# cgmb/euler

Measured on AMD Instinct MI355X. Metric: cells*steps/sec of sim_step() (frames incl. the PCG pressure projection) + pressure-solve HBM GB/s vs roofline, higher is better.
Workload: dtype f64

## Files before the change

euler_amd/__init__.py:

```python
import ctypes as C
import os

import numpy as np

_HERE = os.path.dirname(os.path.abspath(__file__))
LIB_PATH = os.path.join(_HERE, "lib", "libeuler_hip.so")

DOT_AUTO, DOT_SEQUENTIAL, DOT_TREE = 0, 1, 2
PRECOND_IC0, PRECOND_JACOBI, PRECOND_IC0_TILE, PRECOND_IC0_TILE2, PRECOND_IC0_TILE_MG = 0, 1, 2, 3, 4
(OPT_P_STEPS, OPT_TILE_STORE_AS, OPT_TILE_REVERSE, OPT_RESIDENT_CAP, OPT_GRID4_MIN_CELLS, OPT_SLAB_FUSION, OPT_RCCL_SMALL, OPT_RCCL_NO_EXCHANGE, OPT_MARKERS_ROWMAJOR,
 OPT_SA_RUN, OPT_NO_INTERIOR, OPT_BUILD_GATHER, OPT_RESIDENT_FORCE_TIMEOUT, OPT_MG_SPLIT_LEVEL, OPT_MG_SPLIT_ACTIVE, OPT_MARKERS_TWO_PASS, OPT_BUILD_TWO_PASS,
 OPT_VELOCITY_TWO_PASS, OPT_NO_TILE_MAP, OPT_PROFILE_STRIDE, OPT_TILE_STORE_Z, OPT_ADVECT_RK2, OPT_ADVECT_MACCORMACK) = range(1, 24)
SWEEP_AUTO, SWEEP_BAND, SWEEP_SIMPLE = 0, 1, 2
PCG_F64, PCG_F32 = 0, 1
RESIDENT_AUTO, RESIDENT_OFF = 0, 1
IMAGE_COVERAGE, IMAGE_DYE, IMAGE_SPEED = 0, 1, 2
EDIT_SOLID, EDIT_CLEAR, EDIT_SINK, EDIT_SOURCE, EDIT_FILL, EDIT_DRAIN = range(6)
OVERVIEW_DTYPE = np.dtype({"names": ["cells", "solid", "sink", "water", "marks", "max_speed2", "dye"],
                           "formats": [np.uint32, np.uint32, np.uint32, np.uint32, np.uint32, np.float32, (np.uint64, 3)],
                           "offsets": [0, 4, 8, 12, 16, 20, 24], "itemsize": 48})
DIAG_CROWDED = 8
DIAG_DTYPE = np.dtype({"names": ["cells", "fluid", "markers", "crowded", "mass_x", "mass_y", "div_l1", "ke_hi", "ke_lo", "count_max", "nonfinite", "max_div", "max_speed2"],
                       "formats": [np.uint64] * 9 + [np.uint32, np.uint32, np.float32, np.float32],
                       "offsets": [0, 8, 16, 24, 32, 40, 48, 56, 64, 72, 76, 80, 84], "itemsize": 88})
FLOW_PRESSURE = 1
PAINT_VORTICITY, PAINT_PRESSURE, PAINT_SPEED = 0, 1, 2
FLOW_DTYPE = np.dtype({"names": ["cells", "water", "nodes", "nonfinite", "u_pos", "u_neg", "v_pos", "v_neg", "w_pos", "w_neg", "p_sum", "max_speed2", "max_abs_w", "max_p", "reserved"],
                       "formats": [np.uint32] * 4 + [np.uint64] * 7 + [np.float32] * 3 + [np.uint32],
                       "offsets": [0, 4, 8, 12, 16, 24, 32, 40, 48, 56, 64, 72, 76, 80, 84], "itemsize": 88})
DIAG_VALUES = ("mean_abs_div", "kinetic_energy", "com_x", "com_y", "markers_per_cell", "crowded_fraction")
(F_U, F_V, F_UTMP, F_VTMP, F_SOLID, F_SOURCE, F_SINK, F_COUNT, F_PREV_COUNT, F_MARKERS, F_PRECON,
 F_PRESSURE, F_PCG_B, F_PCG_R, F_PCG_Z, F_PCG_S, F_PCG_Q, F_CELLMASK,
 F_DYE_R, F_DYE_G, F_DYE_B, F_DYE_RTMP, F_DYE_GTMP, F_DYE_BTMP, F_MARKER_KEYS) = range(25)
(STAGE_ADVECT_MARKERS, STAGE_REFRESH_COUNTS, STAGE_SOURCES, STAGE_EXTRAPOLATE, STAGE_ADVECT_VELOCITY,
 STAGE_PROJECT) = range(6)
(OP_BUILD_SYSTEM, OP_PRECON_FACTOR, OP_FORWARD_SOLVE, OP_BACKWARD_SOLVE, OP_APPLY_A, OP_DOT_ZR, OP_DOT_ZS,
 OP_INF_NORM_R, OP_UPDATE_PR, OP_UPDATE_SEARCH) = range(10)

_FIELD_DTYPE = {
    F_U: np.float32, F_V: np.float32, F_UTMP: np.float32, F_VTMP: np.float32,
    F_SOLID: np.uint8, F_SOURCE: np.uint8, F_SINK: np.uint8, F_COUNT: np.uint8, F_PREV_COUNT: np.uint8,
    F_MARKERS: np.float32, F_PRECON: np.float64, F_PRESSURE: np.float64, F_PCG_B: np.float64,
    F_PCG_R: np.float64, F_PCG_Z: np.float64, F_PCG_S: np.float64, F_PCG_Q: np.float64, F_CELLMASK: np.uint8,
    F_DYE_R: np.float32, F_DYE_G: np.float32, F_DYE_B: np.float32,
    F_DYE_RTMP: np.float32, F_DYE_GTMP: np.float32, F_DYE_BTMP: np.float32, F_MARKER_KEYS: np.uint32,
}


class EulerError(RuntimeError):
    def __init__(self, code, msg):
        super().__init__("libeuler_hip error %d: %s" % (code, msg))
        self.code = code


class Config(C.Structure):
    _fields_ = [
        ("abi_version", C.c_int32), ("X", C.c_int32), ("Y", C.c_int32), ("device", C.c_int32),
        ("max_iterations", C.c_int32), ("tol", C.c_double), ("dot_mode", C.c_int32), ("precond", C.c_int32),
        ("sweep_mode", C.c_int32), ("max_substeps", C.c_int32), ("frame_time", C.c_float),
        ("viscosity", C.c_float), ("pcg_poll_interval", C.c_int32), ("rainbow", C.c_int32),
        ("precond_tile_records", C.c_int32), ("slab_rank", C.c_int32), ("slab_nranks", C.c_int32),
        ("slab_band_lo", C.c_int32), ("slab_band_hi", C.c_int32), ("pcg_precision", C.c_int32), ("resident", C.c_int32),
    ]


class Stats(C.Structure):
    _fields_ = [
        ("frames", C.c_uint64), ("total_substeps", C.c_uint64), ("total_pcg_iterations", C.c_uint64),
        ("last_substeps", C.c_int32), ("last_pcg_iterations", C.c_int32), ("last_residual", C.c_double),
        ("last_dt", C.c_float), ("n_markers", C.c_uint64), ("source_exhausted", C.c_int32),
        ("rng_state", C.c_uint64), ("marker_dt_events", C.c_uint64), ("marker_multi_events", C.c_uint64),
        ("fluid_cells", C.c_uint64),
    ]


_lib = None

EXPORTS = [
    "euler_config_default", "euler_create", "euler_destroy", "euler_last_error", "euler_abi_version",
    "euler_load_scenario_mem", "euler_load_scenario_file", "euler_load_half_tank", "euler_load_half_tanks", "euler_parse_scenario",
    "euler_seed_markers", "euler_step", "euler_timestep", "euler_substep", "euler_stage", "euler_pcg_op", "euler_set_precond", "euler_set_solver",
    "euler_get_field", "euler_set_field", "euler_set_markers", "euler_set_rng", "euler_get_stats",
    "euler_field_bytes", "euler_render", "euler_render_grids", "euler_render_grids_rgb", "euler_colorize", "euler_profile_enable",
    "euler_profile_class_count", "euler_profile_class_name", "euler_profile_get", "euler_profile_reset",
    "euler_measure_copy_bandwidth", "euler_measure_exchange", "euler_device_name", "euler_hbm_bytes", "euler_sweep_timeline", "euler_save_state", "euler_load_state", "euler_set_comm", "euler_set_stream", "euler_slab_info",
    "euler_rccl_unique_id", "euler_rccl_version", "euler_set_comm_rccl", "euler_comm_calls",
    "euler_p2p_export", "euler_p2p_connect", "euler_p2p_disconnect", "euler_p2p_calls", "euler_resident_info",
    "euler_set_option", "euler_get_option",
    "euler_overview", "euler_overview_text", "euler_overview_rgb", "euler_render_fit",
    "euler_diagnostics", "euler_diag_derive",
    "euler_overview_box", "euler_marker_raster", "euler_view_text", "euler_render_view",
    "euler_edit_box",
    "euler_flow_raster", "euler_flow_paint",
]

# ... 511 lines not shown
```

euler_amd/csrc/driver.hip:

```cpp
#include "euler_dev.h"
#include "k_mg.h"

#include <math.h>
#include <stdarg.h>
#include <stdlib.h>
#include <string.h>

#include <vector>

int eu_launch_build_system(euler_sim* S, float dt);
int eu_launch_velocity_update(euler_sim* S, float dt, int finish);
int eu_pressure_current(euler_sim* S);
int eu_unskew(euler_sim* S, const void* skew, void* rowmajor, int elem_bytes);
int eu_unskew_fluid(euler_sim* S, const double* skew, double* rowmajor);
double* eu_current_search_direction(euler_sim* S);
int eu_launch_tile_table(euler_sim* S);
int eu_skew(euler_sim* S, const void* rowmajor, void* skew, int elem_bytes);

static thread_local char g_err[512] = "";

void eu_set_error(const char* fmt, ...) {
  va_list ap;
  va_start(ap, fmt);
  vsnprintf(g_err, sizeof(g_err), fmt, ap);
// ... 40 lines not shown
    const int e = k / 2, cls = S->ev_cls[e];
    bool active = true;
    if (S->ev_iter[e] > -2) {
      const int q = S->ev_solve[e];
      const int iters = q == S->solve_seq ? cur_iters : (S->solve_seq - q < 256 ? S->solve_iters[q & 255] : 0);
      active = iters >= 0 && S->ev_iter[e] < iters;
      if (S->ev_iter[e] == -1) active = iters >= 0;
    }
    float ms = 0.f;
    if (hipEventElapsedTime(&ms, S->ev_pool[k], S->ev_pool[k + 1]) != hipSuccess) continue;
    if (active) { S->prof_ms[cls] += ms; S->prof_launches[cls] += 1; }
    else S->prof_idle[cls] += 1;
  }
  S->ev_used = 0;
  return EULER_OK;
}

extern "C" int euler_profile_class_count(void) { return KC__COUNT; }
extern "C" const char* euler_profile_class_name(int32_t c) { return (c >= 0 && c < KC__COUNT) ? k_class_names[c] : ""; }
extern "C" int euler_profile_enable(euler_sim* S, uint64_t mask) {
  if (!S) return EULER_EINVAL;
  int rc = eu_prof_flush(S);
  S->prof_mask = mask;
  S->prof_open = 0;
  return rc;
}
extern "C" int euler_profile_get(euler_sim* S, int32_t cls, double* ms, uint64_t* launches) {
  if (!S || cls < 0 || cls >= KC__COUNT) return EULER_EINVAL;
  int rc = eu_prof_flush(S);
  if (ms) *ms = S->prof_ms[cls];
  if (launches) *launches = S->prof_launches[cls];
  return rc;
}
extern "C" int euler_profile_reset(euler_sim* S) {
  if (!S) return EULER_EINVAL;
  int rc = eu_prof_flush(S);
  memset(S->prof_ms, 0, sizeof(S->prof_ms));
  memset(S->prof_launches, 0, sizeof(S->prof_launches));
  memset(S->prof_idle, 0, sizeof(S->prof_idle));
  return rc;
}

extern "C" int euler_config_default(euler_config* c) {
  if (!c) return EULER_EINVAL;
  memset(c, 0, sizeof(*c));
  c->abi_version = EULER_ABI_VERSION;
  c->X = 100; c->Y = 40;
  c->device = 0;
  c->max_iterations = 100;
  c->tol = (double)1e-6f;
  c->dot_mode = EULER_DOT_AUTO;
  c->precond = EULER_PRECOND_IC0;
  c->sweep_mode = EULER_SWEEP_AUTO;
  c->max_substeps = 8;
  c->frame_time = 0.1f;
  c->viscosity = 0.f;
  c->pcg_poll_interval = 8;
  return EULER_OK;
}

static int eu_set_tiles(euler_sim* S, int w) {
  if (w <= 0) w = 16;
  if (w != 8 && w != 16 && w != 32) { eu_set_error("precond_tile_records = %d: 8, 16 or 32 (0 = 16)", w); return EULER_EINVAL; }
  S->cfg.precond_tile_records = w;
  S->tile_w = w;
  return EULER_OK;
}

bool eu_resident_eligible(const euler_sim* S) {
  if (S->res_disabled || S->cfg.resident == EULER_RESIDENT_OFF) return false;
  if (S->cfg.precond != EULER_PRECOND_IC0_TILE || S->tile_w != 16 || S->cfg.sweep_mode == EULER_SWEEP_SIMPLE || S->cfg.dot_mode != EULER_DOT_TREE) return false;
  if (S->has_comm || S->slab_on || S->p2p_on) return false;
  const int cap = eu_resident_capacity(const_cast<euler_sim*>(S), S->cfg.pcg_precision == EULER_PCG_F32);
  if (S->cfg.pcg_precision == EULER_PCG_F32) return cap > 0 && S->geom.nbands * (S->geom.T / 16) <= 4 * cap;
  return cap > 0;
}
extern "C" int euler_resident_info(euler_sim* S, uint64_t out[3]) {
  if (!S || !out) return EULER_EINVAL;
  out[0] = eu_resident_eligible(S) ? 1 : 0; out[1] = S->res_solves; out[2] = S->res_fallbacks;
  return EULER_OK;
}

extern "C" int euler_set_option(euler_sim* S, int32_t key, int64_t value) {
  if (!S || key <= 0 || key >= EULER_OPT__COUNT) { eu_set_error("euler_set_option: unknown key %d", (int)key); return EULER_EINVAL; }
  bool ok = true;
  const char* when = nullptr;
  switch (key) {
    case EULER_OPT_P_STEPS: ok = value == 2 || value == 4 || value == 8; break;
    case EULER_OPT_SA_RUN: ok = value == 8 || value == 16 || value == 32;
      if (ok && value != 8 && (S->has_comm || eu_is_two_level(S))) when = "on a handle without a communicator, in the parity or the plain tile-local mode (the others run runs of 8)";
      break;
    case EULER_OPT_RCCL_SMALL: ok = value >= 0 && value <= 2; if (S->rccl) when = "before euler_set_comm_rccl"; break;
    case EULER_OPT_RCCL_NO_EXCHANGE: ok = value == 0 || value == 1; if (S->rccl) when = "before euler_set_comm_rccl"; break;
    case EULER_OPT_SLAB_FUSION: ok = value == 0 || value == 1; if (S->p2p_on) when = "before euler_p2p_connect"; break;
    case EULER_OPT_RESIDENT_CAP: case EULER_OPT_GRID4_MIN_CELLS: case EULER_OPT_RESIDENT_FORCE_TIMEOUT: ok = value >= 0; break;
    case EULER_OPT_MG_SPLIT_LEVEL: ok = value >= -1 && value < 12; break;
    case EULER_OPT_PROFILE_STRIDE: ok = value >= 1 && value <= 1024; break;
    case EULER_OPT_MG_SPLIT_ACTIVE: ok = false; break;
    case EULER_OPT_ADVECT_RK2: ok = value == 0 || value == 1;
      if (ok && value == 1 && S->slab_on) when = "on a whole-grid handle (row slabs: the midpoint samples reach one row beyond the ghost rows)";
      break;
    case EULER_OPT_ADVECT_MACCORMACK: ok = value == 0 || value == 1;
      if (ok && value == 1 && S->slab_on) when = "on a whole-grid handle (row slabs: the correction reads the forward result one row beyond the own rows)";
      break;
    default: ok = value == 0 || value == 1; break;
  }
  if (!ok) { eu_set_error("euler_set_option: key %d does not take the value %lld", (int)key, (long long)value); return EULER_EINVAL; }
  if (when) { eu_set_error("euler_set_option: key %d must be set %s", (int)key, when); return EULER_ESTATE; }
  HIPCHK(hipStreamSynchronize(S->stream));
  if (key == EULER_OPT_ADVECT_MACCORMACK && value == 1 && !S->mc_u) {
    float *a = nullptr, *b = nullptr;
    const size_t bytes = S->C * sizeof(float);
    if (hipMalloc((void**)&a, bytes) != hipSuccess || hipMalloc((void**)&b, bytes) != hipSuccess || hipMemset(a, 0, bytes) != hipSuccess ||
        hipMemset(b, 0, bytes) != hipSuccess) {
      if (a) (void)hipFree(a);
      if (b) (void)hipFree(b);
      (void)hipGetLastError();
      eu_set_error("euler_set_option: EULER_OPT_ADVECT_MACCORMACK needs %zu bytes of scratch", 2 * bytes);
      return EULER_ENOMEM;
    }
    S->mc_u = a; S->mc_v = b;
    S->hbm_bytes += 2 * bytes;
  }
  if (key == EULER_OPT_P_STEPS || key == EULER_OPT_SA_RUN) {
    int rcp = eu_pressure_current(S);
    if (rcp) return rcp;
  }
  S->opt[key] = value;
  if (key == EULER_OPT_P_STEPS || key == EULER_OPT_SA_RUN) S->s_ring_n = 0;
  if (key == EULER_OPT_MG_SPLIT_LEVEL) { eu_mg_split_release(S); S->opt[EULER_OPT_MG_SPLIT_ACTIVE] = 0; }
  return EULER_OK;
}
extern "C" int euler_get_option(euler_sim* S, int32_t key, int64_t* value) {
  if (!S || !value || key <= 0 || key >= EULER_OPT__COUNT) { eu_set_error("euler_get_option: unknown key %d", (int)key); return EULER_EINVAL; }
  *value = S->opt[key];
  return EULER_OK;
}

static const char* eu_precond_combination(const euler_sim* S, int precond, int tile_w, int has_comm, int slab_on, int p2p_on) {
  const bool coarse = precond == EULER_PRECOND_IC0_TILE2 || precond == EULER_PRECOND_IC0_TILE_MG;
  if (!coarse) return nullptr;
  if (tile_w != 16 || S->cfg.sweep_mode == EULER_SWEEP_SIMPLE) return "the coarse-correction preconditioners run on tiles of 16 records with the band schedule";
  if (precond == EULER_PRECOND_IC0_TILE2 && (has_comm || slab_on)) return "EULER_PRECOND_IC0_TILE2 runs on one GPU (row slabs: EULER_PRECOND_IC0_TILE_MG)";
  if (precond == EULER_PRECOND_IC0_TILE_MG && has_comm && (!slab_on || p2p_on)) return "EULER_PRECOND_IC0_TILE_MG with several ranks: row-slab handles without mailboxes only";
  return nullptr;
}

extern "C" int euler_set_precond(euler_sim* S, int32_t precond, int32_t tile_records) {
  if (!S || precond < EULER_PRECOND_IC0 || precond > EULER_PRECOND_IC0_TILE_MG) { eu_set_error("euler_set_precond: bad argument"); return EULER_EINVAL; }
  const int w = tile_records <= 0 ? 16 : tile_records;
  if (w != 8 && w != 16 && w != 32) { eu_set_error("precond_tile_records = %d: 8, 16 or 32 (0 = 16)", tile_records); return EULER_EINVAL; }
  if (const char* why = eu_precond_combination(S, precond, w, S->has_comm, S->slab_on, S->p2p_on)) { eu_set_error("euler_set_precond: %s", why); return EULER_EINVAL; }
  if (S->cfg.pcg_precision == EULER_PCG_F32 && (precond != EULER_PRECOND_IC0_TILE || w != 16)) { eu_set_error("euler_set_precond: an EULER_PCG_F32 handle runs EULER_PRECOND_IC0_TILE with tiles of 16 records only"); return EULER_EINVAL; }
  HIPCHK(hipStreamSynchronize(S->stream));
  const bool coarse = precond == EULER_PRECOND_IC0_TILE2 || precond == EULER_PRECOND_IC0_TILE_MG;
  if (coarse) { int rc = eu_coarse_alloc(S, precond == EULER_PRECOND_IC0_TILE_MG); if (rc) return rc; }
  (void)eu_set_tiles(S, w);
  S->cfg.dot_mode = coarse ? EULER_DOT_TREE : S->dot_mode_user;
  if (S->has_comm && S->cfg.dot_mode == EULER_DOT_SEQUENTIAL) S->cfg.dot_mode = EULER_DOT_TREE;
  S->cfg.precond = precond;
  S->lean_ok = 0;
  return EULER_OK;
}

extern "C" int euler_set_solver(euler_sim* S, int32_t max_iterations, double tol) {
  if (!S) return EULER_EINVAL;
  HIPCHK(hipStreamSynchronize(S->stream));
  if (max_iterations > 0) S->cfg.max_iterations = max_iterations;
  if (tol >= 0.0) S->cfg.tol = tol;
  return EULER_OK;
}

static thread_local size_t g_alloc_bytes = 0;
template <typename T>
static int dalloc(T** p, size_t n) {
  HIPCHK(hipMalloc((void**)p, n * sizeof(T)));
  g_alloc_bytes += n * sizeof(T);
  HIPCHK(hipMemset(*p, 0, n * sizeof(T)));
  return EULER_OK;
}
#define DALLOC(p, n) do { int _rc = dalloc(&(p), (n)); if (_rc) { euler_destroy(S); return _rc; } } while (0)

extern "C" void euler_destroy(euler_sim* S) {
  if (!S) return;
  if (S->stream) (void)hipStreamSynchronize(S->stream);
  eu_p2p_release(S);
  eu_rccl_release(S);
  eu_slab_release(S);
  eu_coarse_release(S);
  for (eu_devbuf* b : {&S->ov_buf, &S->diag_buf, &S->vr_buf, &S->flow_buf}) eu_devbuf_release(S, b);
  const size_t wo = S->shifted ? S->win_off : 0;
  for (float* f : {S->u, S->v, S->utmp, S->vtmp}) if (f) (void)hipFree(f + wo);
  for (uint8_t* g : {S->solid, S->source, S->sink, S->count, S->prev_count}) if (g) (void)hipFree(g + wo);
  if (S->count32) (void)hipFree(S->count32);
  if (S->blockedT) (void)hipFree(S->blockedT);
  if (S->tmap) (void)hipFree(S->tmap);
  if (S->uT) (void)hipFree(S->uT);
  if (S->vT) (void)hipFree(S->vT);
  if (S->countT) (void)hipFree(S->countT);
  if (S->solidT) (void)hipFree(S->solidT);
  if (S->sys_m) (void)hipFree(S->sys_m);
  if (S->sys_div) (void)hipFree(S->sys_div);
  void* dev[] = {S->markers[0], S->markers[1], S->keys[0], S->keys[1], S->ms, S->evmask, S->delmask, S->ev_theta, S->ev_delta, S->sel_idx, S->act_idx,
                 S->act_dt, S->cellmask64, S->draws, S->sel.block_sums, S->sc, S->partial, S->red_counter, S->granules, S->ticket, S->sweep_timeline, S->halo_buf, S->band_ranges, S->partial2, S->pair_buf, S->xrows, S->alpha_buf, S->rng_jump, S->chunk_flag, S->chunk_prev, S->chunk_part, S->tile_table, S->chunk_bits, S->chunk_list, S->zhalo, S->zrows,
                 S->rowmajor_tmp, S->mc_u, S->mc_v};
  for (void* p : dev) if (p) (void)hipFree(p);
  for (float* d : S->dye) if (d) (void)hipFree(d + wo);
  const size_t so = S->shifted ? S->skew_off : 0, sl = S->shifted ? (size_t)EU_SKEW_SLACK : 0;
  (void)so; (void)sl;
  for (void* d : S->s_ring_alloc) if (d) (void)hipFree(d);
  for (void* d : S->skew_alloc) if (d) (void)hipFree(d);
  const size_t fb_off = S->shifted ? (size_t)S->ab_lo * S->fb_stride * 64 : 0;
  if (S->fbits_fwd) (void)hipFree(S->fbits_fwd + fb_off);
  if (S->fbits_bwd) (void)hipFree(S->fbits_bwd + fb_off);
  if (S->ms_host) (void)hipHostFree(S->ms_host);
  if (S->sc_host) (void)hipHostFree(S->sc_host);
  if (S->poll_host) (void)hipHostFree(S->poll_host);
  if (S->res_err) (void)hipHostFree(S->res_err);
  if (S->res_gran) (void)hipFree(S->res_gran);
  for (hipEvent_t e : S->poll_event) if (e) (void)hipEventDestroy(e);
  if (S->ev_pool) { for (int k = 0; k < S->ev_cap; ++k) if (S->ev_pool[k]) (void)hipEventDestroy(S->ev_pool[k]); free(S->ev_pool); }
  free(S->ev_cls); free(S->ev_solve); free(S->ev_iter);
  if (S->stream && S->own_stream) (void)hipStreamDestroy(S->stream);
  free(S);
}

extern "C" int euler_create(const euler_config* cfg, euler_sim** out) {
  if (!cfg || !out) { eu_set_error("euler_create: null argument"); return EULER_EINVAL; }
  if (cfg->abi_version != EULER_ABI_VERSION) { eu_set_error("euler_create: ABI version %d != %d", cfg->abi_version, EULER_ABI_VERSION); return EULER_EINVAL; }
  if (cfg->X < 8 || cfg->Y < 8 || (size_t)cfg->X * cfg->Y > (size_t)1 << 30) { eu_set_error("euler_create: grid %dx%d out of range", cfg->X, cfg->Y); return EULER_EINVAL; }
  int ndev = 0;
  hipError_t e = hipGetDeviceCount(&ndev);
  if (e != hipSuccess || ndev == 0) {
    eu_set_error("euler_create: no HIP device (%s); libeuler_hip has no CPU path", e == hipSuccess ? "device count 0" : hipGetErrorString(e));
    return EULER_EHIP;
  }
  if (cfg->device < 0 || cfg->device >= ndev) { eu_set_error("euler_create: device %d of %d", cfg->device, ndev); return EULER_EINVAL; }
  HIPCHK(hipSetDevice(cfg->device));
  hipDeviceProp_t prop;
  HIPCHK(hipGetDeviceProperties(&prop, cfg->device));
  if (strncmp(prop.gcnArchName, "gfx950", 6) != 0) {
    eu_set_error("euler_create: device is %s; this library carries gfx950 code only", prop.gcnArchName);
    return EULER_EHIP;
  }

  euler_sim* S = (euler_sim*)calloc(1, sizeof(euler_sim));
  if (S) { S->opt[EULER_OPT_P_STEPS] = 8; S->opt[EULER_OPT_TILE_REVERSE] = 1; S->opt[EULER_OPT_GRID4_MIN_CELLS] = 1ll << 22; S->opt[EULER_OPT_SA_RUN] = 8; S->opt[EULER_OPT_PROFILE_STRIDE] = 1; }
  if (!S) return EULER_ENOMEM;
  g_alloc_bytes = 0;
  S->cfg = *cfg;
  if (S->cfg.max_iterations <= 0) S->cfg.max_iterations = 100;
  if (S->cfg.max_substeps <= 0) S->cfg.max_substeps = 8;
  if (S->cfg.frame_time <= 0.f) S->cfg.frame_time = 0.1f;
  S->X = cfg->X; S->Y = cfg->Y;
  const size_t C = S->C = (size_t)cfg->X * cfg->Y;
  if (S->cfg.dot_mode == EULER_DOT_AUTO) S->cfg.dot_mode = C <= 65536 ? EULER_DOT_SEQUENTIAL : EULER_DOT_TREE;
  S->dot_mode_user = S->cfg.dot_mode;
  if (S->cfg.sweep_mode == EULER_SWEEP_AUTO) S->cfg.sweep_mode = EULER_SWEEP_BAND;
  S->geom.X = S->X; S->geom.Y = S->Y;
  S->geom.nbands = (S->Y + 63) / 64;
  S->geom.T = (S->X + 63 + 95) / 96 * 96;
  S->geom.TS = (S->geom.T + 31) / 32 * 32 + 64;
  S->geom.S = (size_t)S->geom.nbands * S->geom.TS * 64;
  const int nbands = S->geom.nbands;
  S->slab_on = cfg->slab_nranks >= 1;
  if (S->slab_on) {
    if (cfg->slab_rank < 0 || cfg->slab_rank >= cfg->slab_nranks || cfg->slab_nranks > nbands) {
      eu_set_error("euler_create: slab rank %d of %d for %d bands of 64 rows", cfg->slab_rank, cfg->slab_nranks, nbands);
      free(S); return EULER_EINVAL;
    }
    if (S->cfg.sweep_mode == EULER_SWEEP_SIMPLE) {
      eu_set_error("euler_create: row slabs do not run EULER_SWEEP_SIMPLE");
      free(S); return EULER_EINVAL;
    }
    S->band_lo = (int)((int64_t)nbands * cfg->slab_rank / cfg->slab_nranks);
    S->band_hi = (int)((int64_t)nbands * (cfg->slab_rank + 1) / cfg->slab_nranks);
    if (cfg->slab_band_hi > cfg->slab_band_lo || cfg->slab_band_lo != 0) {
      const int lo = cfg->slab_band_lo, hi = cfg->slab_band_hi;
      const bool first = cfg->slab_rank == 0, last = cfg->slab_rank + 1 == cfg->slab_nranks;
      if (lo < 0 || hi <= lo || hi > nbands || (first && lo != 0) || (last && hi != nbands) || (!first && lo < cfg->slab_rank) ||
          (!last && nbands - hi < cfg->slab_nranks - 1 - cfg->slab_rank)) {
        eu_set_error("euler_create: slab rank %d of %d cannot own bands [%d, %d) of %d (every rank needs a band; the ranges tile the grid in rank order)",
                     cfg->slab_rank, cfg->slab_nranks, lo, hi, nbands);
        free(S); return EULER_EINVAL;
      }
      S->band_lo = lo; S->band_hi = hi;
    }
    if (S->cfg.dot_mode == EULER_DOT_SEQUENTIAL) S->cfg.dot_mode = EULER_DOT_TREE;
  } else { S->band_lo = 0; S->band_hi = nbands; }
  S->row_lo = 64 * S->band_lo; S->row_hi = 64 * S->band_hi < S->Y ? 64 * S->band_hi : S->Y;
  S->win_lo = S->row_lo - EU_GHOST_LO > 0 ? S->row_lo - EU_GHOST_LO : 0;
  S->win_hi = S->row_hi + EU_GHOST_HI < S->Y ? S->row_hi + EU_GHOST_HI : S->Y;
  S->win_off = (size_t)S->win_lo * S->X;
  S->Cw = (size_t)(S->win_hi - S->win_lo) * S->X;
  S->ab_lo = S->band_lo > 0 ? S->band_lo - 1 : 0; S->ab_hi = S->band_hi < nbands ? S->band_hi + 1 : nbands;
  S->skew_off = (size_t)S->ab_lo * S->geom.TS * 64;
  S->Sw = (size_t)(S->ab_hi - S->ab_lo) * S->geom.TS * 64;
  S->e_lo = (size_t)S->band_lo * S->geom.TS * 64; S->e_cnt = (size_t)(S->band_hi - S->band_lo) * S->geom.TS * 64;
  const size_t SS = S->Sw;
  const size_t Cw = S->Cw;
  if (C > ((size_t)1 << 29) || Cw > ((size_t)1 << 28) || (SS + EU_SKEW_SLACK) * 8 >= ((size_t)1 << 32)) {
    eu_set_error("grid %d x %d is larger than the supported maximum (2^28 cells per GPU, 2^29 in all)", cfg->X, cfg->Y);
    free(S);
    return EULER_EINVAL;
  }
#define CREATECHK(call) do { hipError_t _e = (call); if (_e != hipSuccess) { int _rc = eu_hip_fail(_e, #call, __FILE__, __LINE__); euler_destroy(S); return _rc; } } while (0)
  CREATECHK(hipStreamCreateWithFlags(&S->stream, hipStreamNonBlocking));
  S->own_stream = 1;

  DALLOC(S->u, Cw); DALLOC(S->v, Cw); DALLOC(S->utmp, Cw); DALLOC(S->vtmp, Cw);
  DALLOC(S->solid, Cw); DALLOC(S->source, Cw); DALLOC(S->sink, Cw); DALLOC(S->count, Cw); DALLOC(S->prev_count, Cw);
  DALLOC(S->count32, Cw);
  if (!S->slab_on) { DALLOC(S->blockedT, Cw); DALLOC(S->uT, Cw); DALLOC(S->vT, Cw); DALLOC(S->countT, Cw); DALLOC(S->solidT, Cw); }
  eu_state_replaced(S);
  DALLOC(S->sys_m, Cw); DALLOC(S->sys_div, Cw);
  if (S->cfg.rainbow) for (float*& d : S->dye) DALLOC(d, Cw);
  S->max_markers = 4 * C;
  if (S->slab_on) { const size_t cap = 6 * (size_t)(S->row_hi - S->row_lo) * S->X + 65536; if (cap < S->max_markers) S->max_markers = cap; }
  DALLOC(S->markers[0], S->max_markers); DALLOC(S->markers[1], S->max_markers);
  if (S->slab_on) { DALLOC(S->keys[0], S->max_markers); DALLOC(S->keys[1], S->max_markers); }
  DALLOC(S->ms, 1);
  const size_t mwords = (S->max_markers + 63) / 64;
  DALLOC(S->evmask, mwords);
  if (!S->slab_on) DALLOC(S->delmask, mwords);
  if (!S->slab_on) {
    S->tmap_nx = (S->X + 63) / 64 + 1; S->tmap_n = S->tmap_nx * ((S->Y + 63) / 64 + 2);
    DALLOC(S->tmap, 3 * (size_t)S->tmap_n);
  }
  DALLOC(S->ev_theta, S->max_markers); DALLOC(S->ev_delta, S->max_markers);
  S->sel_cap = S->max_markers;
  DALLOC(S->sel_idx, S->sel_cap);
  DALLOC(S->act_idx, S->max_markers); DALLOC(S->act_dt, S->max_markers);
  DALLOC(S->cellmask64, (Cw + 63) / 64 + 1);
  S->sel.capacity_blocks = (mwords + 2047) / 2048 + 1;
  DALLOC(S->sel.block_sums, S->sel.capacity_blocks);
  {
    const size_t stagger = (size_t)EU_ARRAY_STAGGER / 8 * 8;
    int k = 0;
    for (double** d : {&S->b, &S->p, &S->r, &S->z, &S->s, &S->s2, &S->q, &S->precon}) {
      DALLOC(*d, SS + EU_SKEW_SLACK + 8 * stagger / 8);
      S->skew_alloc[k] = *d;
      *d += (size_t)k * stagger / 8;
      ++k;
    }
    DALLOC(S->cellmask, SS + EU_SKEW_SLACK);
    S->skew_alloc[8] = S->cellmask;
  }
  S->fb_stride = 12 * (((S->geom.T + 7) / 8 + 11) / 12) + 4;
  DALLOC(S->fbits_fwd, (size_t)(S->ab_hi - S->ab_lo) * S->fb_stride * 64);
  DALLOC(S->fbits_bwd, (size_t)(S->ab_hi - S->ab_lo) * S->fb_stride * 64);
  DALLOC(S->sc, 1);
  DALLOC(S->band_ranges, (size_t)S->geom.nbands);
  { int rc = eu_set_tiles(S, S->cfg.precond_tile_records); if (rc) { euler_destroy(S); return rc; } }
  S->red_blocks = (int)eu_blocks(S->e_cnt, EU_RED_ELEMS, 2048);
  DALLOC(S->partial, (size_t)S->red_blocks > 2048 ? (size_t)S->red_blocks : 2048);
  DALLOC(S->partial2, 2048);
  DALLOC(S->pair_buf, 2 * 64);
  DALLOC(S->alpha_buf, 64);
  S->xrow_len = ((size_t)S->X + 15) / 16 * 16 + 64;
  DALLOC(S->xrows, 8 * S->xrow_len);
  S->chunk_cap = (size_t)(S->band_hi - S->band_lo) * (S->geom.T / 16);
  S->chunk_words = (S->chunk_cap + 63) / 64;
  DALLOC(S->chunk_flag, S->chunk_cap + 64);
  DALLOC(S->chunk_prev, S->chunk_cap + 64);
  DALLOC(S->chunk_part, S->chunk_cap + 64);
  DALLOC(S->tile_table, 8 * 64 * 2);
  DALLOC(S->chunk_bits, S->chunk_words + 1);
  DALLOC(S->chunk_list, S->chunk_cap + 64);
  {
    RngJump* J = (RngJump*)malloc(sizeof(RngJump));
    if (!J) { euler_destroy(S); return EULER_ENOMEM; }
    auto step = [](unsigned long long st) { st ^= st >> 12; st ^= st << 25; st ^= st >> 27; return st; };
    for (int b = 0; b < 64; ++b) J->col[0][b] = step(1ull << b);
    for (int i = 1; i < EU_RNG_JUMPS; ++i)
      for (int b = 0; b < 64; ++b) {
        unsigned long long x = J->col[i - 1][b], y = 0;
        for (int k = 0; k < 64; ++k) if ((x >> k) & 1) y ^= J->col[i - 1][k];
        J->col[i][b] = y;
      }
    int rc = dalloc(&S->rng_jump, 1);
    if (!rc && hipMemcpy(S->rng_jump, J, sizeof(RngJump), hipMemcpyHostToDevice) != hipSuccess) rc = EULER_EHIP;
    free(J);
    if (rc) { euler_destroy(S); return rc; }
  }
  DALLOC(S->red_counter, 1);
  DALLOC(S->halo_buf, (size_t)8 * S->X);
  S->gran_stride = (S->geom.T - 63 + 7) / 8 * 8;
  DALLOC(S->granules, (size_t)S->geom.nbands * S->gran_stride * 2);
  DALLOC(S->ticket, 1);
  DALLOC(S->sweep_timeline, (size_t)S->geom.nbands * 8);
  S->ticket_base = 0; S->epoch = 0;
  for (float** f : {&S->u, &S->v, &S->utmp, &S->vtmp}) *f -= S->win_off;
  for (float*& d : S->dye) if (d) d -= S->win_off;
  for (uint8_t** g : {&S->solid, &S->source, &S->sink, &S->count, &S->prev_count}) *g -= S->win_off;
  for (double** d : {&S->b, &S->p, &S->r, &S->z, &S->s, &S->s2, &S->q, &S->precon}) *d += EU_SKEW_SLACK - S->skew_off;
  S->cellmask += EU_SKEW_SLACK - S->skew_off;
  S->fbits_fwd -= (size_t)S->ab_lo * S->fb_stride * 64; S->fbits_bwd -= (size_t)S->ab_lo * S->fb_stride * 64;
  S->shifted = 1;
  CREATECHK(hipHostMalloc((void**)&S->ms_host, sizeof(MarkerState), hipHostMallocDefault));
  CREATECHK(hipHostMalloc((void**)&S->sc_host, sizeof(PcgScalars), hipHostMallocDefault));
  CREATECHK(hipHostMalloc((void**)&S->poll_host, 2 * sizeof(PcgScalars), hipHostMallocDefault));
  CREATECHK(hipHostMalloc((void**)&S->res_err, sizeof(int), hipHostMallocDefault));
  *S->res_err = 0;
  DALLOC(S->res_gran, 2 * 2 * (2 * 768) * 2);
  S->res_tag = 1;
  memset(S->poll_host, 0, 2 * sizeof(PcgScalars));
  for (hipEvent_t& e : S->poll_event) CREATECHK(hipEventCreateWithFlags(&e, hipEventDisableTiming));
  memset(S->ms_host, 0, sizeof(MarkerState)); memset(S->sc_host, 0, sizeof(PcgScalars));

  S->interp_lim[0] = nextafterf((float)(S->X - 2), 0.f);
  S->interp_lim[1] = nextafterf((float)(S->Y - 1), 0.f);
  S->interp_lim[2] = nextafterf((float)(S->X - 1), 0.f);
  S->interp_lim[3] = nextafterf((float)(S->Y - 2), 0.f);

  S->ev_cap = 16384;
  S->ev_pool = (hipEvent_t*)calloc((size_t)S->ev_cap, sizeof(hipEvent_t));
  S->ev_cls = (int*)calloc((size_t)S->ev_cap / 2, sizeof(int));
  S->ev_solve = (int*)calloc((size_t)S->ev_cap / 2, sizeof(int));
  S->ev_iter = (int*)calloc((size_t)S->ev_cap / 2, sizeof(int));
  S->prof_iter = -2;
  if (!S->ev_pool || !S->ev_cls || !S->ev_solve || !S->ev_iter) { euler_destroy(S); return EULER_ENOMEM; }
  for (int k = 0; k < S->ev_cap; ++k) CREATECHK(hipEventCreate(&S->ev_pool[k]));
  if (S->slab_on) { int rc = eu_slab_alloc(S); if (rc) { euler_destroy(S); return rc; } }
  if (S->cfg.precond == EULER_PRECOND_IC0_TILE2 || S->cfg.precond == EULER_PRECOND_IC0_TILE_MG) {
    if ((S->slab_on && S->cfg.precond != EULER_PRECOND_IC0_TILE_MG) || S->tile_w != 16 || S->cfg.sweep_mode == EULER_SWEEP_SIMPLE) {
      eu_set_error("EULER_PRECOND_IC0_TILE2: one GPU; _MG: one GPU or row slabs; both: tiles of 16 records, the band schedule"); euler_destroy(S); return EULER_EINVAL;
    }
    S->cfg.dot_mode = EULER_DOT_TREE;
    int rc = eu_coarse_alloc(S, S->cfg.precond == EULER_PRECOND_IC0_TILE_MG);
    if (rc) { euler_destroy(S); return rc; }
  }
  S->hbm_bytes = g_alloc_bytes + (S->slab_on ? eu_slab_bytes(S) : 0);
  eu_launch_tile_table(S);
  if (S->cfg.pcg_precision != EULER_PCG_F64 && S->cfg.pcg_precision != EULER_PCG_F32) { eu_set_error("euler_create: pcg_precision %d", S->cfg.pcg_precision); euler_destroy(S); return EULER_EINVAL; }
  if (S->cfg.pcg_precision == EULER_PCG_F32 && !eu_resident_eligible(S)) {
    eu_set_error("euler_create: EULER_PCG_F32 runs in the resident solver: one GPU, EULER_PRECOND_IC0_TILE with tiles of 16 records, EULER_DOT_TREE, "
                 "EULER_RESIDENT_AUTO, and a grid of at most %d 16-record chunks (this one: %d)", 4 * eu_resident_capacity(S, 1), S->geom.nbands * (S->geom.T / 16));
    euler_destroy(S); return EULER_EINVAL;
  }
  CREATECHK(hipStreamSynchronize(S->stream));
#undef CREATECHK
  *out = S;
  return EULER_OK;
}

static int upload_scenario(euler_sim* S, const uint8_t* solid, const uint8_t* source, const uint8_t* sink,
                           const uint8_t* fluid) {
  const size_t C = S->C;
  if (S->slab_on && !S->has_comm) { eu_set_error("row-slab handle: install the communicator (euler_set_comm / euler_set_comm_rccl) before loading a scenario"); return EULER_ESTATE; }
  std::vector<float> mk;
  std::vector<unsigned int> keys;
  uint64_t rng = EULER_RNG_SEED, n = 0, n_loc = 0;
  int rc;
  if (S->slab_on) {
    uint64_t cells = 0;
    for (int y = S->row_lo > 0 ? S->row_lo - 1 : 0; y < S->row_hi; ++y)
      for (int x = 0; x < S->X; ++x) cells += fluid[(size_t)y * S->X + x] != 0;
    const uint64_t room = 4 * cells;
    if (room > S->max_markers) { eu_set_error("row slab %d holds up to %llu markers, more than its capacity %zu", S->cfg.slab_rank, (unsigned long long)room, S->max_markers); return EULER_ENOMEM; }
    try { mk.resize(2 * (size_t)room + 2); keys.resize((size_t)room + 1); } catch (...) { return EULER_ENOMEM; }
    rc = euler_seed_markers_rows(fluid, S->X, S->Y, S->row_lo, S->row_hi, &rng, mk.data(), keys.data(), room, &n, &n_loc);
  } else {
    try { mk.resize(2 * 4 * C); } catch (...) { return EULER_ENOMEM; }
    rc = euler_seed_markers(fluid, S->X, S->Y, &rng, mk.data(), &n);
    n_loc = n;
  }
  if (rc) return rc;
  size_t nsrc = 0;
  for (size_t i = (size_t)S->row_lo * S->X; i < (size_t)S->row_hi * S->X; ++i) nsrc += source[i] != 0;
  S->n_source_cells = nsrc;
  if (S->draws) { (void)hipFree(S->draws); S->draws = nullptr; }
  if (nsrc) HIPCHK(hipMalloc((void**)&S->draws, 2 * nsrc * sizeof(float)));

  hipStream_t st = S->stream;
  const size_t wo = S->win_off, Cw = S->Cw;
  HIPCHK(hipMemcpyAsync(S->solid + wo, solid + wo, Cw, hipMemcpyHostToDevice, st));
  HIPCHK(hipMemcpyAsync(S->source + wo, source + wo, Cw, hipMemcpyHostToDevice, st));
  HIPCHK(hipMemcpyAsync(S->sink + wo, sink + wo, Cw, hipMemcpyHostToDevice, st));
  eu_state_replaced(S);
  for (float* f : {S->u, S->v, S->utmp, S->vtmp}) HIPCHK(hipMemsetAsync(f + wo, 0, Cw * sizeof(float), st));
  for (double* d : {S->b, S->p, S->r, S->z, S->s, S->s2, S->q, S->precon}) HIPCHK(hipMemsetAsync(d + S->skew_off, 0, S->Sw * sizeof(double), st));
  for (float* d : S->dye) if (d) HIPCHK(hipMemsetAsync(d + wo, 0, Cw * sizeof(float), st));
  HIPCHK(hipMemsetAsync(S->count + wo, 0, Cw, st));
  HIPCHK(hipMemsetAsync(S->prev_count + wo, 0, Cw, st));
// ... 114 lines not shown
  if (!ops->allreduce || !ops->halo || !ops->chain || !ops->allgather || ops->rank < 0 || ops->rank >= ops->nranks) {
    eu_set_error("euler_set_comm: incomplete communicator"); return EULER_EINVAL;
  }
  const int nb = S->geom.nbands;
  if (ops->nranks > nb) { eu_set_error("euler_set_comm: %d ranks for %d bands (64 rows each)", ops->nranks, nb); return EULER_EINVAL; }
  if (S->cfg.sweep_mode == EULER_SWEEP_SIMPLE) { eu_set_error("euler_set_comm: EULER_SWEEP_SIMPLE is single-rank only"); return EULER_EINVAL; }
  S->comm = *ops; S->bulk = *ops;
  S->has_comm = 1;
  S->couple = coupling == EULER_SLAB_EXACT;
  S->band_lo = (int)((int64_t)nb * ops->rank / ops->nranks);
  S->band_hi = (int)((int64_t)nb * (ops->rank + 1) / ops->nranks);
  S->e_lo = (size_t)S->band_lo * S->geom.TS * 64;
  S->e_cnt = (size_t)(S->band_hi - S->band_lo) * S->geom.TS * 64;
  if (S->cfg.dot_mode == EULER_DOT_SEQUENTIAL) S->cfg.dot_mode = EULER_DOT_TREE;
  return eu_set_comm_slot(S);
}

extern "C" int euler_set_comm(euler_sim* S, const euler_comm_ops* ops, int32_t coupling) {
  if (!S) return EULER_EINVAL;
  HIPCHK(hipStreamSynchronize(S->stream));
  eu_p2p_release(S);
  eu_rccl_release(S);
  return eu_install_comm(S, ops, coupling, 0);
}

extern "C" int euler_slab_info(euler_sim* S, int32_t* lo, int32_t* hi, int32_t* nb) {
  if (!S) return EULER_EINVAL;
  if (lo) *lo = S->band_lo;
  if (hi) *hi = S->band_hi;
  if (nb) *nb = S->geom.nbands;
  return EULER_OK;
}

int eu_sync_marker_state(euler_sim* S) {
  HIPCHK(hipMemcpyAsync(S->ms_host, S->ms, sizeof(MarkerState), hipMemcpyDeviceToHost, S->stream));
  HIPCHK(hipStreamSynchronize(S->stream));
  S->n_markers_host = S->slab_on ? S->ms_host->n_loc : S->ms_host->n;
  if (S->ms_host->error) {
    if (S->ms_host->error >= 16) { eu_set_error("row slabs (seen on rank %d): exchange buffer overflow on some rank (code %d: 16 dt-chain candidates, 17 migration, 18 deletions, 19 marker capacity)", S->cfg.slab_rank, S->ms_host->error); return EULER_ESTATE; }
    eu_set_error("device-side bounded wait expired (band pipeline), error=%d", S->ms_host->error);
    return EULER_ETIMEOUT;
  }
  return EULER_OK;
}

extern "C" int euler_timestep(euler_sim* S, float frame_time_left, float* dt) {
  if (!S || !S->loaded) { eu_set_error("euler_timestep: no scenario loaded"); return EULER_ESTATE; }
  int rc = eu_launch_timestep(S, frame_time_left);
  if (rc) return rc;
  rc = eu_sync_marker_state(S);
  if (rc) return rc;
  if (dt) *dt = S->ms_host->dt;
  return EULER_OK;
}

static int run_stage(euler_sim* S, int stage, float dt) {
  if (stage != EULER_STAGE_REFRESH_COUNTS) S->prebin_valid = 0;
  if (stage == EULER_STAGE_EXTRAPOLATE && S->maxsq_state == 2) S->maxsq_state = 1;
  if (stage == EULER_STAGE_REFRESH_COUNTS) { S->uv_clean = S->uv_clean == 1 ? 2 : 0; S->uv_zb = 0; }
  if (stage == EULER_STAGE_REFRESH_COUNTS) { S->utmp_clean = S->utmp_clean == 1 ? 2 : 0; S->countT_clean = S->countT_clean == 1 ? 2 : 0; }
  if (stage == EULER_STAGE_SOURCES) S->uv_zb = 0;
  switch (stage) {
    case EULER_STAGE_ADVECT_MARKERS: return eu_launch_advect_markers(S, dt);
    case EULER_STAGE_REFRESH_COUNTS: return eu_launch_refresh_counts(S);
    case EULER_STAGE_SOURCES: {
      int rc = eu_launch_dye_extrapolate(S);
      if (!rc) rc = eu_launch_sources(S);
      if (!rc) rc = eu_launch_dye_sources(S);
      return rc;
    }
    case EULER_STAGE_EXTRAPOLATE: return eu_launch_extrapolate(S);
    case EULER_STAGE_ADVECT_VELOCITY: {
      int rc = eu_launch_dye_advect(S, dt);
      if (!rc) rc = eu_launch_advect_velocity(S, dt);
      return rc;
    }
    case EULER_STAGE_PROJECT: return eu_launch_project(S, dt);
    default: eu_set_error("unknown stage %d", stage); return EULER_EINVAL;
  }
}

extern "C" int euler_stage(euler_sim* S, int32_t stage, float dt) {
  if (!S || !S->loaded) { eu_set_error("euler_stage: no scenario loaded"); return EULER_ESTATE; }
  int rc = S->slab_on ? eu_slab_stage(S, stage, dt) : run_stage(S, stage, dt);
  if (rc) return rc;
  if (S->slab_on && (rc = eu_slab_error_sync(S))) return rc;
  rc = eu_sync_marker_state(S);
  if (!rc && stage == EULER_STAGE_PROJECT) {
    S->stats.last_pcg_iterations = S->sc_host->nonzero ? S->sc_host->iters : 0;
    S->stats.last_residual = S->sc_host->rnorm;
  }
  return rc;
}

static int substep_async(euler_sim* S, float dt) {
  if (S->slab_on) return eu_slab_substep(S, dt);
  for (int st = 0; st < EULER_STAGE__COUNT; ++st) {
    int rc = run_stage(S, st, dt);
    if (rc) return rc;
  }
  return EULER_OK;
}

static void account_substep(euler_sim* S, float dt) {
  S->stats.total_substeps += 1;
  S->stats.last_dt = dt;
}

extern "C" int euler_substep(euler_sim* S, float dt) {
  if (!S || !S->loaded) { eu_set_error("euler_substep: no scenario loaded"); return EULER_ESTATE; }
  int rc = substep_async(S, dt);
  if (rc) return rc;
  if (S->slab_on && (rc = eu_slab_error_sync(S))) return rc;
  rc = eu_sync_marker_state(S);
  if (rc) return rc;
  account_substep(S, dt);
  S->stats.total_pcg_iterations += (uint64_t)S->sc_host->iters;
  S->stats.last_pcg_iterations = S->sc_host->iters;
  S->stats.last_residual = S->sc_host->rnorm;
  return EULER_OK;
}

extern "C" int euler_step(euler_sim* S) {
  if (!S || !S->loaded) { eu_set_error("euler_step: no scenario loaded"); return EULER_ESTATE; }
  float frame_time = S->cfg.frame_time;
  int nsub = 0, iters = 0;
  for (int step = 0; frame_time > 0.f && step < S->cfg.max_substeps; ++step) {
    float dt = 0.f;
    int rc = euler_timestep(S, frame_time, &dt);
    if (rc) return rc;
    if (step > 0) { iters += S->sc_host->iters; S->stats.last_residual = S->sc_host->rnorm; }
    frame_time -= dt;
    rc = substep_async(S, dt);
    if (rc) return rc;
    account_substep(S, dt);
    ++nsub;
  }
  int rc = S->slab_on ? eu_slab_error_sync(S) : EULER_OK;
  if (rc) return rc;
  rc = eu_sync_marker_state(S);
  if (rc) return rc;
  if (nsub) { iters += S->sc_host->iters; S->stats.last_residual = S->sc_host->rnorm; }
  S->stats.total_pcg_iterations += (uint64_t)iters;
  S->stats.last_pcg_iterations = iters;
  S->stats.last_substeps = nsub;
  S->stats.frames += 1;
  return EULER_OK;
}

extern "C" int euler_pcg_op(euler_sim* S, int32_t op, float dt, double a, double* out) {
  if (!S || !S->loaded) { eu_set_error("euler_pcg_op: no scenario loaded"); return EULER_ESTATE; }
  if (S->slab_on) { eu_set_error("euler_pcg_op: single PCG operations are not exposed on a row-slab handle"); return EULER_ESTATE; }
  S->pcg_fields_resident = 0;
  int rcp = eu_pressure_current(S);
  if (rcp) return rcp;
  return eu_launch_pcg_op(S, op, dt, a, out);
}

static int field_ptr(euler_sim* S, int f, void** p, size_t* bytes) {
  const size_t C = (size_t)(S->row_hi - S->row_lo) * S->X, o = (size_t)S->row_lo * S->X;
  switch (f) {
    case EULER_F_U: *p = S->u + o; *bytes = C * 4; break;
    case EULER_F_V: *p = S->v + o; *bytes = C * 4; break;
    case EULER_F_UTMP: *p = S->utmp + o; *bytes = C * 4; break;
    case EULER_F_VTMP: *p = S->vtmp + o; *bytes = C * 4; break;
    case EULER_F_SOLID: *p = S->solid + o; *bytes = C; break;
    case EULER_F_SOURCE: *p = S->source + o; *bytes = C; break;
    case EULER_F_SINK: *p = S->sink + o; *bytes = C; break;
    case EULER_F_COUNT: *p = S->count + o; *bytes = C; break;
    case EULER_F_PREV_COUNT: *p = S->prev_count + o; *bytes = C; break;
    case EULER_F_MARKERS: *p = S->markers[S->cur]; *bytes = (size_t)S->n_markers_host * 8; break;
    case EULER_F_MARKER_KEYS:
      if (!S->slab_on) { eu_set_error("EULER_F_MARKER_KEYS: row-slab handles only (elsewhere a marker's key is its index)"); return EULER_ESTATE; }
      *p = S->keys[S->cur]; *bytes = (size_t)S->n_markers_host * 4; break;
    case EULER_F_PRECON: *p = S->precon; *bytes = C * 8; break;
    case EULER_F_PRESSURE: *p = S->p; *bytes = C * 8; break;
    case EULER_F_PCG_B: *p = S->b; *bytes = C * 8; break;
    case EULER_F_PCG_R: *p = S->r; *bytes = C * 8; break;
    case EULER_F_PCG_Z: *p = S->z; *bytes = C * 8; break;
    case EULER_F_PCG_S: *p = eu_current_search_direction(S); *bytes = C * 8; break;
    case EULER_F_PCG_Q: *p = S->q; *bytes = C * 8; break;
    case EULER_F_CELLMASK: *p = S->cellmask; *bytes = C; break;
    case EULER_F_DYE_R: case EULER_F_DYE_G: case EULER_F_DYE_B: case EULER_F_DYE_RTMP: case EULER_F_DYE_GTMP: case EULER_F_DYE_BTMP:
      if (!S->dye[0]) { eu_set_error("field %d needs euler_config.rainbow", f); return EULER_ESTATE; }
      *p = S->dye[f - EULER_F_DYE_R] + o; *bytes = C * 4; break;
    default: eu_set_error("unknown field %d", f); return EULER_EINVAL;
  }
  return EULER_OK;
}

extern "C" size_t euler_field_bytes(const euler_sim* S, int32_t f) {
  void* p; size_t b = 0;
  if (!S || field_ptr((euler_sim*)S, f, &p, &b)) return 0;
  return b;
}

static bool field_is_skewed(int f) {
  return f == EULER_F_PRECON || f == EULER_F_PRESSURE || (f >= EULER_F_PCG_B && f <= EULER_F_PCG_Q) || f == EULER_F_CELLMASK;
}
static int ensure_rowmajor_tmp(euler_sim* S) {
  if (!S->rowmajor_tmp) HIPCHK(hipMalloc((void**)&S->rowmajor_tmp, (size_t)(S->row_hi - S->row_lo) * S->X * sizeof(double)));
  return EULER_OK;
}

extern "C" int euler_get_field(euler_sim* S, int32_t f, void* dst, size_t dst_bytes) {
  if (!S || !dst) return EULER_EINVAL;
  void* p; size_t b;
  int rc = field_ptr(S, f, &p, &b);
  if (rc) return rc;
  if (dst_bytes < b) { eu_set_error("euler_get_field(%d): buffer %zu < %zu bytes", f, dst_bytes, b); return EULER_EINVAL; }
  if (b == 0) return EULER_OK;
  if ((f == EULER_F_PCG_Z || f == EULER_F_PCG_S || f == EULER_F_PCG_Q) && S->pcg_fields_resident) {
    eu_set_error("euler_get_field(%d): the last solve ran in the resident kernel, which keeps z, s and A s in registers (euler_config.resident = EULER_RESIDENT_OFF shows them)", f);
    return EULER_ESTATE;
  }
  if (f == EULER_F_PRESSURE && (rc = eu_pressure_current(S))) return rc;
  if (field_is_skewed(f)) {
    rc = ensure_rowmajor_tmp(S);
    if (rc) return rc;
    if (f == EULER_F_PCG_S && S->s_none) HIPCHK(hipMemsetAsync(S->rowmajor_tmp, 0, b, S->stream));
    else if (f == EULER_F_PCG_S && S->s_stale) eu_unskew_fluid(S, (const double*)p, (double*)S->rowmajor_tmp);
    else eu_unskew(S, p, S->rowmajor_tmp, f == EULER_F_CELLMASK ? 1 : 8);
    p = S->rowmajor_tmp;
  }
  HIPCHK(hipMemcpyAsync(dst, p, b, hipMemcpyDeviceToHost, S->stream));
  HIPCHK(hipStreamSynchronize(S->stream));
  return EULER_OK;
}

int eu_set_source_count(euler_sim* S, size_t nsrc) {
  S->n_source_cells = nsrc;
  if (S->draws) { (void)hipFree(S->draws); S->draws = nullptr; }
  if (nsrc) HIPCHK(hipMalloc((void**)&S->draws, 2 * nsrc * sizeof(float)));
  return EULER_OK;
}

extern "C" int euler_set_field(euler_sim* S, int32_t f, const void* src, size_t src_bytes) {
  if (!S || !src) return EULER_EINVAL;
  if (field_is_skewed(f)) { int rcp = eu_pressure_current(S); if (rcp) return rcp; }
  eu_state_edited(S);
  if (S->slab_on && (f == EULER_F_MARKERS || f == EULER_F_MARKER_KEYS || f == EULER_F_COUNT || f == EULER_F_PREV_COUNT ||
                     f == EULER_F_SOLID || f == EULER_F_SOURCE)) {
    eu_set_error("euler_set_field(%d): a row-slab handle takes its markers, counts, solid and source cells from euler_load_scenario_* / euler_load_state only", f); return EULER_ESTATE;
  }
  if (f == EULER_F_MARKERS) return euler_set_markers(S, (const float*)src, src_bytes / 8);
  void* p; size_t b;
  int rc = field_ptr(S, f, &p, &b);
  if (rc) return rc;
  if (src_bytes != b) { eu_set_error("euler_set_field(%d): %zu bytes given, %zu expected", f, src_bytes, b); return EULER_EINVAL; }
  if (field_is_skewed(f)) {
    S->lean_ok = 0;
    if (f == EULER_F_PCG_S) { S->s_stale = 0; S->s_launched = 0; S->s_none = 0; }
    rc = ensure_rowmajor_tmp(S);
    if (rc) return rc;
    HIPCHK(hipMemcpyAsync(S->rowmajor_tmp, src, b, hipMemcpyHostToDevice, S->stream));
    eu_skew(S, S->rowmajor_tmp, p, f == EULER_F_CELLMASK ? 1 : 8);
  } else {
    HIPCHK(hipMemcpyAsync(p, src, b, hipMemcpyHostToDevice, S->stream));
  }
  HIPCHK(hipStreamSynchronize(S->stream));
  if (S->slab_on && (f == EULER_F_U || f == EULER_F_V)) {
    rc = eu_slab_exchange_uv(S);
    if (rc) return rc;
    HIPCHK(hipStreamSynchronize(S->stream));
  }
  if (f == EULER_F_SOLID || f == EULER_F_SINK) { S->blocked_dirty = 1; S->solidT_dirty = 1; }
  if (f == EULER_F_SOURCE) {
    const uint8_t* s = (const uint8_t*)src;
    size_t nsrc = 0;
    for (size_t i = 0; i < (size_t)(S->row_hi - S->row_lo) * S->X; ++i) nsrc += s[i] != 0;
    if ((rc = eu_set_source_count(S, nsrc))) return rc;
  }
  S->loaded = 1;
  return EULER_OK;
}

__global__ void k_set_marker_state(MarkerState* ms, unsigned long long n, unsigned long long maxm, int set_n,
                                   unsigned long long rng, int exhausted, int set_rng) {
  if (set_n) { ms->n = n; ms->max_markers = maxm; }
  if (set_rng) { ms->rng_state = rng; ms->exhausted = exhausted; }
}

extern "C" int euler_set_markers(euler_sim* S, const float* xy, uint64_t n) {
  if (!S || (!xy && n) || n > S->max_markers) return EULER_EINVAL;
  if (S->slab_on) { eu_set_error("euler_set_markers: not on a row-slab handle"); return EULER_ESTATE; }
  eu_state_edited(S);
  if (n) HIPCHK(hipMemcpyAsync(S->markers[S->cur], xy, n * 8, hipMemcpyHostToDevice, S->stream));
  hipLaunchKernelGGL(k_set_marker_state, dim3(1), dim3(1), 0, S->stream, S->ms, (unsigned long long)n,
                     (unsigned long long)S->max_markers, 1, 0ull, 0, 0);
  S->loaded = 1;
  return eu_sync_marker_state(S);
}

extern "C" int euler_set_rng(euler_sim* S, uint64_t rng, int32_t exhausted) {
  if (!S) return EULER_EINVAL;
  hipLaunchKernelGGL(k_set_marker_state, dim3(1), dim3(1), 0, S->stream, S->ms, 0ull, 0ull, 0, (unsigned long long)rng,
                     (int)exhausted, 1);
  return eu_sync_marker_state(S);
}

__global__ __launch_bounds__(256) void k_count_fluid(const uint8_t* __restrict__ count, size_t C, unsigned long long* out) {
  unsigned int c = 0;
  for (size_t i = (size_t)blockIdx.x * blockDim.x + threadIdx.x; i < C; i += (size_t)gridDim.x * blockDim.x) c += count[i] != 0;
  c = (unsigned int)eu_wave_sum((double)c);
  if ((threadIdx.x & 63) == 0 && c) atomicAdd(out, (unsigned long long)c);
}

extern "C" int euler_get_stats(euler_sim* S, euler_stats* out) {
  if (!S || !out) return EULER_EINVAL;
  int rc = eu_sync_marker_state(S);
  if (rc) return rc;
  unsigned long long* scratch = (unsigned long long*)S->partial;
  HIPCHK(hipMemsetAsync(scratch, 0, 8, S->stream));
  hipLaunchKernelGGL(k_count_fluid, dim3(eu_blocks((size_t)(S->row_hi - S->row_lo) * S->X, 256 * 8, 1024)), dim3(256), 0, S->stream,
                     S->count + (size_t)S->row_lo * S->X, (size_t)(S->row_hi - S->row_lo) * S->X, scratch);
  unsigned long long nf = 0;
  HIPCHK(hipMemcpyAsync(&nf, scratch, 8, hipMemcpyDeviceToHost, S->stream));
  HIPCHK(hipStreamSynchronize(S->stream));
  S->stats.n_markers = S->ms_host->n;
  S->stats.source_exhausted = S->ms_host->exhausted;
  S->stats.rng_state = S->ms_host->rng_state;
  S->stats.marker_dt_events = S->ms_host->total_dt_events;
// ... 136 lines not shown
```

euler_amd/csrc/euler_dev.h:

```cpp
#pragma once

#include <hip/hip_runtime.h>
#include <stdint.h>
#include <stdio.h>

#include "euler.h"
#include "euler_host.h"

#define EU_H 1.0f
#define EU_RHO 1.0f
#define EU_G (-10.0f)

#define CM_FLUID 0x01
#define CM_RIGHT 0x02
#define CM_UP    0x04
#define CM_LEFT  0x08
#define CM_DOWN  0x10
#define CM_DIAG_SHIFT 5
#define CM_INTERIOR 0x9F
#define EU_CHUNK_INTERIOR 0x80000000u

enum {
  KC_TIMESTEP = 0, KC_MARKER_ADVECT, KC_MARKER_EVENTS, KC_MARKER_BIN, KC_MARKER_COMPACT, KC_SOURCES,
  KC_SELECT, KC_EXTRAPOLATE, KC_ADVECT_VELOCITY, KC_BUILD_SYSTEM, KC_PRECON_FACTOR,
// ... 97 lines not shown
  unsigned long long* delmask;
  uint8_t* tmap;
  int tmap_nx, tmap_n;
  int tmap_valid;
  int utmp_clean;
  int countT_clean;
  uint8_t* blockedT;
  int blocked_dirty;
  float *uT, *vT; uint8_t *countT, *solidT;
  int solidT_dirty;
  float* dye[6];
  eu_devbuf ov_buf, diag_buf, vr_buf, flow_buf;
  float *mc_u, *mc_v;
  float2* markers[2];
  int cur;
  size_t max_markers;
  unsigned long long n_markers_host;
  size_t n_source_cells;
  MarkerState* ms;
  MarkerState* ms_host;
  unsigned long long* evmask;
  float* ev_theta;
  float* ev_delta;
  unsigned int* sel_idx;
  size_t sel_cap;
  unsigned int* act_idx; float* act_dt;
  unsigned long long* cellmask64;
  float* draws;
  SelectScratch sel;

  SkewGeom geom;
  double *b, *p, *r, *z, *s, *q, *precon;
  double* s2;
  void* skew_alloc[9];
  uint8_t* cellmask;
  uint8_t* sys_m; float* sys_div;
  unsigned int* fbits_fwd; unsigned int* fbits_bwd;
  int fb_stride;
  int4* band_ranges;
  int coarse_m, coarse_shift, coarse_nx, coarse_ny, coarse_n;
  int *cc_diag, *cc_right, *cc_up;
  int* cc_pinned;
  double* cc_sten;
  int cc_n;
  double* cc_fac;
  double* cc_inv;
  double* cc_part;
  double* cc_y;
  double* cc_null;
  int mg_levels, mg_nx[12], mg_ny[12];
  size_t mg_off[12], mg_cells;
  double* mg_a;
  unsigned long long* mg_a0i;
  double *mg_rhs, *mg_x;
  double* mg_wd;
  uint8_t* mg_inner0; double mg_ic[9];
  double* mg_part;
  double* mg_dot;
  double* mg_null0;
  double* mg_m0;
  void* mg_split;
  double* mg_xbuf; int mg_xslot;
  unsigned long long* res_gran;
  unsigned long long res_tag;
  int* res_err;
  int res_disabled;
  unsigned int res_last_chunks;
  int res_have_last, res_skip_once;
  unsigned long long res_solves, res_fallbacks;
  int pcg_fields_resident;
  int tile_w;
  double* s_ring[8];
  void* s_ring_alloc[8];
  double* s_base[2];
  int s_ring_n;
  int s_launched;
  int s_none;
  int s_stale;
  const double* tile_as_override;
  double* partial2;
  struct RngJump* rng_jump;
  uint8_t* chunk_flag;
  uint8_t* chunk_prev;
  uint8_t* chunk_part;
  size_t hbm_bytes;
  int lean_ok;
  double* zhalo;
  double* zrows;
  int z_halo_last;
  double* tile_table;
  unsigned long long* chunk_bits;
  unsigned int* chunk_list;
  size_t chunk_words, chunk_cap;
  double* xrows;
  size_t xrow_len;
  int gs_cur;
  double* alpha_buf;
  double* pair_buf;
  double* rowmajor_tmp;
  PcgScalars* sc;
  PcgScalars* sc_host;
  PcgScalars* poll_host;
  hipEvent_t poll_event[2];
  double* partial;
  unsigned int* red_counter;
  int red_blocks;
  unsigned long long* granules;
  int gran_stride;
  unsigned int* ticket;
  unsigned int ticket_base;
  unsigned int epoch;
  unsigned long long* sweep_timeline;

  float interp_lim[4];

  euler_stats stats;

  euler_comm_ops comm;
  int has_comm, couple;
  int band_lo, band_hi;
  size_t e_lo, e_cnt;
  double* halo_buf;
  int own_stream;
  int slab_on, shifted;
  int row_lo, row_hi, win_lo, win_hi;
  size_t win_off, Cw, skew_off, Sw;
  int ab_lo, ab_hi;
  unsigned int* keys[2];
  euler_comm_ops bulk;
  struct SlabScratch* slab;
  int part_lo[64], part_hi[64];
  void* rccl;
  void* p2p;
  int p2p_on;

  uint64_t prof_mask;
  uint64_t prof_open;
  unsigned int prof_seq[32];
  double prof_ms[KC__COUNT];
  uint64_t prof_launches[KC__COUNT];
  uint64_t prof_idle[KC__COUNT];
  hipEvent_t* ev_pool; int* ev_cls; int* ev_solve; int* ev_iter; int ev_used, ev_cap;
  int solve_seq;
  int prof_iter;
  int solve_iters[256];
};

void eu_set_error(const char* fmt, ...);
int eu_hip_fail(hipError_t e, const char* what, const char* file, int line);
#define HIPCHK(call) do { hipError_t _e = (call); if (_e != hipSuccess) return eu_hip_fail(_e, #call, __FILE__, __LINE__); } while (0)

void eu_prof_begin(euler_sim* S, int cls);
void eu_prof_end(euler_sim* S, int cls);
int  eu_prof_flush(euler_sim* S);

#define LAUNCH(S, CLS, KERNEL, GRID, BLOCK, ...)                                   \
  do {                                                                             \
    eu_prof_begin((S), (CLS));                                                     \
    hipLaunchKernelGGL(KERNEL, GRID, BLOCK, 0, (S)->stream, __VA_ARGS__);          \
    eu_prof_end((S), (CLS));                                                       \
  } while (0)

static inline unsigned eu_blocks(size_t n, unsigned per_block, unsigned cap = 0x7fffffffu) {
  size_t b = (n + per_block - 1) / per_block;
  if (b < 1) b = 1;
  if (b > cap) b = cap;
  return (unsigned)b;
}

__device__ __forceinline__ size_t eu_xcd_block() {
  const unsigned int b = blockIdx.x, full = gridDim.x & ~7u;
  return b < full ? (size_t)(b & 7) * (full >> 3) + (b >> 3) : (size_t)b;
}

#define EU_GHOST_LO 1
#define EU_GHOST_HI 2
int  eu_slab_alloc(euler_sim* S);
size_t eu_slab_bytes(const euler_sim* S);
void eu_slab_release(euler_sim* S);
int  eu_slab_substep(euler_sim* S, float dt);
int  eu_slab_stage(euler_sim* S, int stage, float dt);
int  eu_slab_timestep(euler_sim* S, float frame_time_left);
int  eu_slab_after_load(euler_sim* S);
int  eu_slab_check_partition(euler_sim* S);
int  eu_slab_exchange_uv(euler_sim* S);
int  eu_slab_exchange_dye(euler_sim* S);
int  eu_slab_render(euler_sim* S, int wx, int wy, char* out, int cap, int* len);
int  eu_slab_after_restore(euler_sim* S);
int  eu_slab_error_sync(euler_sim* S);
int  eu_slab_same_everywhere(euler_sim* S, const double* vals, int n, int* same);
int  eu_slab_status_sync(euler_sim* S, int local_rc, int* worst);
static inline void eu_state_replaced(euler_sim* S) {
  S->blocked_dirty = 1; S->solidT_dirty = 1;
  S->prebin_valid = 0;
  if (S->maxsq_state == 2) S->maxsq_state = 1;
  S->p_pending = 0;
  S->uv_clean = 0; S->uv_zb = 0;
  S->tmap_valid = 0; S->utmp_clean = 0; S->countT_clean = 0;
}
static inline void eu_state_edited(euler_sim* S) {
  S->prebin_valid = 0;
  if (S->maxsq_state == 2) S->maxsq_state = 1;
  S->uv_clean = 0; S->uv_zb = 0; S->tmap_valid = 0; S->utmp_clean = 0; S->countT_clean = 0;
}
static inline bool eu_tile_map_on(const euler_sim* S) { return S->tmap && S->tmap_valid && !S->slab_on && S->opt[EULER_OPT_NO_TILE_MAP] == 0; }
int eu_launch_timestep(euler_sim* S, float frame_time_left);
int eu_launch_advect_markers(euler_sim* S, float dt);
int eu_launch_refresh_counts(euler_sim* S);
int eu_launch_sources(euler_sim* S);
int eu_launch_extrapolate(euler_sim* S);
int eu_launch_advect_velocity(euler_sim* S, float dt);
int eu_launch_diffuse(euler_sim* S, float dt);
int eu_launch_project(euler_sim* S, float dt);
int eu_resident_capacity(euler_sim* S, int f32);
int eu_launch_resident(euler_sim* S, unsigned int n_chunks);
bool eu_resident_eligible(const euler_sim* S);
int eu_launch_colorize(euler_sim* S);
int eu_launch_dye_extrapolate(euler_sim* S);
int eu_launch_dye_sources(euler_sim* S);
int eu_launch_dye_advect(euler_sim* S, float dt);
int eu_launch_pcg_op(euler_sim* S, int op, float dt, double a, double* out);
int eu_ordered_select(euler_sim* S, const unsigned long long* mask, size_t nwords, unsigned int* out_idx,
                      unsigned int* out_total);
int eu_sync_marker_state(euler_sim* S);
int eu_marker_compact(euler_sim* S, const unsigned long long* delmask);
int eu_observe_enter(const euler_sim* S, const char* who, const char* slab_reason, const void* out, int x0, int y0, int x1, int y1);
int eu_devbuf_reserve(euler_sim* S, const char* who, const char* what, eu_devbuf* b, size_t bytes);
void eu_devbuf_release(euler_sim* S, eu_devbuf* b);
int eu_observe_readback(euler_sim* S, void* out, const eu_devbuf* b, size_t bytes);
int eu_overview_entered(euler_sim* S, const char* who, int x0, int y0, int x1, int y1, int W, int H, euler_overview_px* out, size_t out_bytes);
void eu_rccl_release(euler_sim* S);
void eu_p2p_release(euler_sim* S);
int eu_p2p_halo_skewed(euler_sim* S, double* s_skewed);
void eu_p2p_xgran(euler_sim* S, int backward, const unsigned long long** in, unsigned long long** out);
int  eu_p2p_has_neighbour_arrays(const euler_sim* S);
void eu_p2p_neighbour_arrays(euler_sim* S, const double** z_dn, const double** s_dn, const double** z_up, const double** s_up);
int eu_install_comm(euler_sim* S, const euler_comm_ops* ops, int32_t coupling, int allow_single);
static inline bool eu_is_tile(const euler_sim* S) { return S->cfg.precond == EULER_PRECOND_IC0_TILE || S->cfg.precond == EULER_PRECOND_IC0_TILE2 || S->cfg.precond == EULER_PRECOND_IC0_TILE_MG; }
static inline bool eu_is_two_level(const euler_sim* S) { return S->cfg.precond == EULER_PRECOND_IC0_TILE2 || S->cfg.precond == EULER_PRECOND_IC0_TILE_MG; }
static inline bool eu_is_mg(const euler_sim* S) { return S->cfg.precond == EULER_PRECOND_IC0_TILE_MG; }
int  eu_coarse_alloc(euler_sim* S, bool mg);
void eu_coarse_release(euler_sim* S);
int  eu_launch_coarse_setup(euler_sim* S);
int  eu_launch_coarse_consistent(euler_sim* S);
int  eu_launch_coarse_solve(euler_sim* S, int fin_op, int force);
int  eu_launch_coarse_search_init(euler_sim* S);
int  eu_coarse_comm_slots(euler_sim* S);
int  eu_launch_coarse_pre(euler_sim* S, int force);
int  eu_launch_coarse_scatter(euler_sim* S);
int  eu_launch_coarse_add_row(euler_sim* S, double* row, int yrow);

#ifdef __HIPCC__

#define EU_WAVE 64

struct GridRef {
  int X, Y;
  const uint8_t* count;
  float ux_lim, uy_lim, vx_lim, vy_lim;
};

__device__ __forceinline__ bool eu_prop_p(const uint8_t* g, size_t i) { return g[i] != 0; }
__device__ __forceinline__ bool eu_tiles_idle(const uint8_t* __restrict__ tmap, int tnx, int tn, int ty, int tx0, int ntx) {
  unsigned int a = 0;
  for (int k = 0; k <= ntx; ++k) {
    const int tx = tx0 + k < tnx ? tx0 + k : tnx - 1;
    const int t = ty * tnx + tx;
    a |= (unsigned int)tmap[t] | tmap[t + tnx] | tmap[tn + t] | tmap[tn + t + tnx];
  }
  return a == 0;
}
__device__ __forceinline__ bool eu_tiles_idle_cur(const uint8_t* __restrict__ tmap, int tnx, int ty, int tx0, int tx1, bool up) {
  unsigned int a = 0;
  for (int tx = tx0; tx <= tx1 + 1; ++tx) {
    const int t = ty * tnx + (tx < tnx ? tx : tnx - 1);
    a |= (unsigned int)tmap[t] | (up ? (unsigned int)tmap[t + tnx] : 0u);
  }
  return a == 0;
}
__device__ __forceinline__ bool eu_prop_u(const uint8_t* g, size_t i) { return (g[i] != 0) | (g[i + 1] != 0); }
__device__ __forceinline__ bool eu_prop_v(const uint8_t* g, size_t i, int X) { return (g[i] != 0) | (g[i + X] != 0); }

__device__ __forceinline__ float eu_lerp(float x0, float x1, float f) { return (1.f - f) * x0 + f * x1; }
__device__ __forceinline__ float eu_frac(float f, bool start_ok, bool end_ok) {
  return !start_ok ? 1.f : (!end_ok ? 0.f : f);
}
__device__ __forceinline__ float eu_clampf(float lo, float x, float hi) { return x < lo ? lo : (x > hi ? hi : x); }

template <int TYPE, bool TR = false, bool PROPS = TR>
__device__ __forceinline__ float eu_interp(const GridRef& g, const float* __restrict__ q, float ix, float iy) {
  ix = eu_clampf(0.f, ix, TYPE == 1 ? g.ux_lim : g.vx_lim);
  iy = eu_clampf(0.f, iy, TYPE == 2 ? g.vy_lim : g.uy_lim);
  float wx, wy;
  const float fx = modff(ix, &wx), fy = modff(iy, &wy);
  const int bx = (int)wx, by = (int)wy;
  const size_t sx = TR ? (size_t)g.Y : (size_t)1, sy = TR ? (size_t)1 : (size_t)g.X;
  const size_t i00 = (size_t)by * sy + (size_t)bx * sx;
  const float r00 = q[i00], r01 = q[i00 + sx], r10 = q[i00 + sy], r11 = q[i00 + sy + sx];
// ... 207 lines not shown
```

euler_amd/csrc/k_pcg.h:

```cpp
#pragma once

#include "euler_dev.h"
#include "k_mg.h"

#define COMM_CALL(expr) do { if ((expr) != 0) { eu_set_error("communicator callback failed: %s", #expr); return EULER_ECOMM; } } while (0)
#define LOC(ptr) ((ptr) + S->e_lo)
enum { SW_FACTOR = 0, SW_FORWARD = 1, SW_BACKWARD = 2 };

int eu_launch_build_system(euler_sim* S, float dt);
int eu_launch_velocity_update(euler_sim* S, float dt, int finish);
int eu_launch_band_ranges(euler_sim* S);
int eu_launch_sweep(euler_sim* S, int op, int cls, int force, int fin_qq = -1);
int eu_launch_factor_tile(euler_sim* S, int force);
int eu_launch_precond_tile(euler_sim* S, int rupd, int sweeps, int fin_dot, int force, double alpha, bool r_only = false, int zform = -1);
int eu_launch_search_apply(euler_sim* S, int it);
int eu_launch_finish_p(euler_sim* S);
int eu_launch_dot(euler_sim* S, const double* a, const double* b, int fin_op, int force);
int eu_comm_exchange(euler_sim* S, double* send_lo, double* send_hi, double* recv_lo, double* recv_hi, int count, double* small, int nsmall);
int eu_comm_finish(euler_sim* S, int fin_op, int is_max, int force);
int eu_comm_halo_two(euler_sim* S, double* a, double* b);
bool tile_recompute(const euler_sim* S);
int p_steps(const euler_sim* S);

enum { FIN_SIGMA_INIT = 0, FIN_ALPHA, FIN_RNORM, FIN_BETA, FIN_STORE_ONLY, FIN_TO_COMM };
#define FIN_VIA_P2P 0x100

static inline bool tile_fused(const euler_sim* S) { return eu_is_tile(S) && S->cfg.sweep_mode != EULER_SWEEP_SIMPLE; }
static inline bool ghost_mode(const euler_sim* S) { return S->has_comm && !S->p2p_on && tile_fused(S); }
enum { XR_ZSEND_LO = 0, XR_ZSEND_HI, XR_ZRECV_LO, XR_ZRECV_HI, XR_GS_LO0, XR_GS_LO1, XR_GS_HI0, XR_GS_HI1 };
static inline double* xrow(const euler_sim* S, int k) { return S->xrows + (size_t)k * S->xrow_len; }
static inline int sa_run(const euler_sim* S) {
  if (S->opt[EULER_OPT_SA_RUN] != 8 && !S->has_comm && !eu_is_two_level(S)) return (int)S->opt[EULER_OPT_SA_RUN];
  return 8;
}
static inline bool tile_z_recompute(const euler_sim* S) {
  return tile_recompute(S) && tile_fused(S) && !eu_is_two_level(S) && S->tile_w == 16 && !S->has_comm && !S->slab_on && S->band_lo == 0 &&
         S->opt[EULER_OPT_TILE_STORE_Z] == 0 && S->chunk_list && S->tile_table;
}
static inline int fin_or_comm(const euler_sim* S, int fin_op) {
  return S->has_comm ? (S->p2p_on ? (fin_op | FIN_VIA_P2P) : (int)FIN_TO_COMM) : fin_op;
}

#ifdef __HIPCC__
#define RED_THREADS 1024
typedef double sw_d2 __attribute__((ext_vector_type(2)));

__device__ __forceinline__ bool pcg_idle(const PcgScalars* sc) { return sc->done || !sc->nonzero; }

#define DPP_WAVE_SHL1 0x130
#define DPP_WAVE_SHR1 0x138

template <int CTRL>
__device__ __forceinline__ double wave_shift_inject(double v, double edge) {
  const int lo = __builtin_amdgcn_update_dpp(__double2loint(edge), __double2loint(v), CTRL, 0xf, 0xf, false);
  const int hi = __builtin_amdgcn_update_dpp(__double2hiint(edge), __double2hiint(v), CTRL, 0xf, 0xf, false);
  return __hiloint2double(hi, lo);
}


__device__ __forceinline__ void pcg_scalar_step(PcgScalars* sc, int op, double v) {
  switch (op) {
    case FIN_SIGMA_INIT: sc->sigma = v; break;
    case FIN_ALPHA: sc->zs = v; sc->alpha_prev = sc->alpha; sc->alpha = sc->sigma / v; sc->alpha_hist[sc->iters & 7] = sc->alpha; sc->iters += 1; break;
    case FIN_RNORM: sc->rnorm = v; if (v <= sc->tol) sc->done = 1; break;
    case FIN_BETA: sc->sigma_new = v; sc->beta = v / sc->sigma; sc->sigma = v; break;
    case FIN_TO_COMM: sc->comm_val = v; if (sc->comm_slot) *sc->comm_slot = v; break;
    default: sc->sigma_new = v; break;
  }
}

template <int NT = RED_THREADS>
__device__ __forceinline__ double block_sum(double v) {
  __shared__ double sw[NT / 64];
  v = eu_wave_sum(v);
  __syncthreads();
  if ((threadIdx.x & 63) == 0) sw[threadIdx.x >> 6] = v;
  __syncthreads();
  double t = 0.0;
  if (threadIdx.x == 0) for (int k = 0; k < NT / 64; ++k) t += sw[k];
  return t;
}
template <int NT = RED_THREADS>
__device__ __forceinline__ double block_max(double v) {
  __shared__ double sm[NT / 64];
  v = eu_wave_max(v);
  __syncthreads();
  if ((threadIdx.x & 63) == 0) sm[threadIdx.x >> 6] = v;
  __syncthreads();
  double t = 0.0;
  if (threadIdx.x == 0) for (int k = 0; k < NT / 64; ++k) t = sm[k] > t ? sm[k] : t;
  return t;
}

template <bool IS_MAX, int NT = RED_THREADS>
__device__ __forceinline__ void block_finish(double v_block, double* partial, unsigned int* counter, PcgScalars* sc, int op) {
  __shared__ int am_last;
  if (threadIdx.x == 0) {
    __hip_atomic_store(reinterpret_cast<unsigned long long*>(&partial[blockIdx.x]),
                       (unsigned long long)__double_as_longlong(v_block), __ATOMIC_RELAXED, __HIP_MEMORY_SCOPE_AGENT);
    asm volatile("s_waitcnt vmcnt(0)" ::: "memory");
    const unsigned int t = __hip_atomic_fetch_add(counter, 1u, __ATOMIC_RELAXED, __HIP_MEMORY_SCOPE_AGENT);
    am_last = t == gridDim.x - 1;
  }
  __syncthreads();
  if (!am_last) return;
  double v = 0.0;
  for (unsigned int i = threadIdx.x; i < gridDim.x; i += NT) {
    const double w = __longlong_as_double((long long)__hip_atomic_load(
        reinterpret_cast<unsigned long long*>(&partial[i]), __ATOMIC_RELAXED, __HIP_MEMORY_SCOPE_AGENT));
    if (IS_MAX) v = w > v ? w : v; else v += w;
  }
  v = IS_MAX ? block_max<NT>(v) : block_sum<NT>(v);
  if (op & FIN_VIA_P2P) { v = p2p_allreduce_block<IS_MAX>(sc, v); op &= 0xff; }
  if (threadIdx.x == 0) {
    pcg_scalar_step(sc, op, v);
    __hip_atomic_store(counter, 0u, __ATOMIC_RELAXED, __HIP_MEMORY_SCOPE_AGENT);
  }
}

__device__ __forceinline__ void st_system(const double* p, double v) {
  asm volatile("global_store_dwordx2 %0, %1, off sc0 sc1" :: "v"(p), "v"(v) : "memory");
// ... 29 lines not shown
    const double res = (cm & CM_FLUID) ? qv : 0.0;
    const double carry = -1.0 * cpre * res;
    own = carry; out = carry;
    if (j & 1) zz[j >> 1].y = res; else zz[j >> 1].x = res;
  }
  own = 0.0; out = 0.0;
#pragma unroll
  for (int j = W - 1; j >= 0; --j) {
    const int cm = (int)((mm[j >> 1] >> ((j & 1) * 8)) & 0xff);
    const double cin = (j & 1) ? zz[j >> 1].y : zz[j >> 1].x, cpre = (j & 1) ? pp[j >> 1].y : pp[j >> 1].x;
    const double nbv = wave_shift_inject<DPP_WAVE_SHL1>(out, 0.0);
    const double kr = ((cm & CM_RIGHT) ? -1.0 : 0.0) * cpre, ku = ((cm & CM_UP) ? -1.0 : 0.0) * cpre;
    const double t = cin - kr * own - ku * nbv;
    const double zv = t * cpre;
    const double res = (cm & CM_FLUID) ? zv : 0.0;
    own = res; out = res;
    if (DOT && (cm & CM_FLUID)) dsum += res * ((j & 1) ? rr[j >> 1].y : rr[j >> 1].x);
    if (j & 1) zz[j >> 1].y = res; else zz[j >> 1].x = res;
  }
}
struct ZrArgs { const double* r; const double* pre; const double* table; const double* halo; const double* rows; int X; };
struct CoarseRef { const double* y; int shift, nx, ny, band0; };
struct SaHist { const double* s[6]; };

struct SweepArgs {
  SkewGeom g;
  const uint8_t* mask;
  const unsigned int* fbits_fwd;
  const unsigned int* fbits_bwd;
  int fb_stride;
  double* pre;
  const double* in;
  double* out;
  unsigned long long* granules;
  int gran_stride;
  const unsigned long long* xg_in;
  unsigned long long* xg_out;
  const int4* ranges;
  int band_lo, nb_local;
  int couple;
  unsigned int* ticket;
  unsigned int ticket_base;
  unsigned int epoch;
  const PcgScalars* sc;
  int force;
  int* error;
  unsigned long long* timeline;
  int tile_w;
  int fin_qq;
  double* qq_partial;
  unsigned int* qq_counter;
  PcgScalars* sc_w;
};

struct TileArgs {
  SkewGeom g;
  const uint8_t* mask;
  double* pre;
  double* r;
  const double* as;
  double* z;
  int band_lo, nb_local;
  int rupd;
  int sweeps;
  int fin_dot;
  int via;
  double* part_max; double* part_dot;
  unsigned int* counter;
  const unsigned int* list;
  const double* table;
  PcgScalars* sc;
  int force;
  double alpha_arg;
  double* pair_slot;
  double *zsend_lo, *zsend_hi;
  int edge_lo, edge_hi;
  int reverse;
  double* cpart;
  int cshift;
  int cmode, cnx, cny;
  const double *gs_lo, *gs_hi;
  int zform;
  double *zhalo, *zrows;
};

__device__ __forceinline__ double factor_step(double aa, double own, double nbv) {
  const double cl = -1.0 * own, cb = -1.0 * nbv;
  double e = aa - cl * cl - cb * cb;
  if (e < 0.25 * aa) e = (aa != 0.0) ? aa : 1.0;
  return 1.0 / sqrt(e);
}

template <int CTRL>
__device__ __forceinline__ double dpp_move(double v) {
  const int lo = __builtin_amdgcn_update_dpp(0, __double2loint(v), CTRL, 0xf, 0xf, true);
  const int hi = __builtin_amdgcn_update_dpp(0, __double2hiint(v), CTRL, 0xf, 0xf, true);
  return __hiloint2double(hi, lo);
}
__device__ __forceinline__ double group_sum(double v) {
  v = v + dpp_move<0xB1>(v);
  v = v + dpp_move<0x4E>(v);
  if (MG_LG == 8) v = v + dpp_move<0x141>(v);
  return v;
}
#endif
```

euler_amd/csrc/k_pcg.hip:

```cpp
#include "k_pcg.h"

#include <cmath>
#include <vector>

template <bool IS_MAX>
__global__ __launch_bounds__(RED_THREADS) void k_reduce_final(const double* __restrict__ partial, int n, PcgScalars* sc,
                                                              int op, int force) {
  if (!force && pcg_idle(sc)) return;
  double v = 0.0;
  for (int i = threadIdx.x; i < n; i += RED_THREADS) {
    const double w = partial[i];
    if (IS_MAX) v = w > v ? w : v; else v += w;
  }
  v = IS_MAX ? block_max(v) : block_sum(v);
  if (threadIdx.x == 0) pcg_scalar_step(sc, op, v);
}

template <bool EDGES>
__global__ __launch_bounds__(RED_THREADS) void k_dot_partial(const double* __restrict__ a, const double* __restrict__ b,
                                                             const uint8_t* __restrict__ mask, size_t S,
                                                             double* __restrict__ partial, PcgScalars* sc, int force,
                                                             unsigned int* counter, int fin_op, int TS, int nb_local, int edges) {
  if (!force && pcg_idle(sc)) return;
  const size_t chunk = (((S + gridDim.x - 1) / gridDim.x) + 1) & ~(size_t)1;
  const size_t lo = (size_t)blockIdx.x * chunk, hi = lo + chunk < S ? lo + chunk : S;
  double t = 0.0;
  for (size_t i = lo + 2 * (size_t)threadIdx.x; i < hi; i += 2 * RED_THREADS) {
    const unsigned int mm = *reinterpret_cast<const unsigned short*>(mask + i);
    if (!((mm | (mm >> 8)) & CM_FLUID)) continue;
    const sw_d2 av = *reinterpret_cast<const sw_d2*>(a + i), bv = *reinterpret_cast<const sw_d2*>(b + i);
    if (mm & CM_FLUID) t += av.x * bv.x;
    if ((mm >> 8) & CM_FLUID) t += av.y * bv.y;
    if (EDGES && slab_edge_row(i, (int)((i & 127) >> 1), TS, nb_local, edges)) {
      if (mm & CM_FLUID) st_system(a + i, av.x);
      if ((mm >> 8) & CM_FLUID) st_system(a + i + 1, av.y);
    }
  }
  if (EDGES) asm volatile("s_waitcnt vmcnt(0)" ::: "memory");
  t = block_sum(t);
  block_finish<false>(t, partial, counter, sc, fin_op);
}

#define SEQ_TILE 4096
__global__ __launch_bounds__(256) void k_dot_sequential(const double* __restrict__ a, const double* __restrict__ b,
                                                        const uint8_t* __restrict__ mask, SkewGeom g, PcgScalars* sc,
                                                        int op, int force) {
  if (!force && pcg_idle(sc)) return;
  __shared__ double prod[2][SEQ_TILE];
  __shared__ unsigned long long any[2][SEQ_TILE / 64];
  const size_t C = (size_t)g.X * g.Y;
  const int ntiles = (int)((C + SEQ_TILE - 1) / SEQ_TILE);
  const int wave = threadIdx.x >> 6, lane = threadIdx.x & 63;
  double total = 0.0;
  for (int tile = -1; tile < ntiles; ++tile) {
    if (wave > 0 && tile + 1 < ntiles) {
      const int buf = (tile + 1) & 1;
      const size_t base = (size_t)(tile + 1) * SEQ_TILE;
      for (int grp = wave - 1; grp < SEQ_TILE / 64; grp += 3) {
        const size_t c = base + (size_t)grp * 64 + lane;
        bool f = false;
        double pr = 0.0;
        if (c < C) {
          const size_t i = skew_index(g, (int)(c % g.X), (int)(c / g.X));
          f = (mask[i] & CM_FLUID) != 0;
          if (f) pr = a[i] * b[i];
        }
        prod[buf][grp * 64 + lane] = pr;
        const unsigned long long bal = __ballot(f);
        if (lane == 0) any[buf][grp] = bal;
      }
    }
    if (threadIdx.x == 0 && tile >= 0) {
      const int buf = tile & 1;
      for (int grp = 0; grp < SEQ_TILE / 64; ++grp) {
        if (any[buf][grp] == 0ull) continue;
        const double* pp = &prod[buf][grp * 64];
        double v[64];
#pragma unroll
        for (int k = 0; k < 64; ++k) v[k] = pp[k];
#pragma unroll
        for (int k = 0; k < 64; ++k) total += v[k];
      }
    }
    __syncthreads();
  }
  if (threadIdx.x == 0) pcg_scalar_step(sc, op, total);
}

__global__ __launch_bounds__(RED_THREADS) void k_apply_a(const double* __restrict__ s, double* __restrict__ z,
                                                         const uint8_t* __restrict__ mask, SkewGeom g,
                                                         double* __restrict__ partial, PcgScalars* sc, int force,
                                                         unsigned int* counter, int fin_op) {
  if (!force && pcg_idle(sc)) return;
  const size_t S = g.S;
  const size_t chunk = (((S + gridDim.x - 1) / gridDim.x) + 127) & ~(size_t)127;
  const size_t lo = (size_t)blockIdx.x * chunk, hi = lo + chunk < S ? lo + chunk : S;
  double t = 0.0;
  for (size_t i = lo + 2 * (size_t)threadIdx.x; i < hi; i += 2 * RED_THREADS) {
    const unsigned int mm = *reinterpret_cast<const unsigned short*>(mask + i);
    const unsigned int m0 = mm & 0xff, m1 = mm >> 8;
    if (!((m0 | m1) & CM_FLUID)) continue;
    const sw_d2 c = *reinterpret_cast<const sw_d2*>(s + i);
    const int l = (int)((i & 127) >> 1);
    sw_d2 o = {0.0, 0.0};
    if (m0 & CM_FLUID) {
      double v = (double)(int)(m0 >> CM_DIAG_SHIFT) * c.x;
      v = v - ((m0 & CM_RIGHT) ? c.y : 0.0);
      if (m0 & CM_UP) {
        size_t up = i + 3;
        if (l == 63) { int band, tt, ll; skew_decode(g, i, band, tt, ll); up = skew_index(g, tt - 63, 64 * (band + 1)); }
        v = v - s[up];
      } else {
        v = v - 0.0;
      }
      v = v - ((m0 & CM_LEFT) ? s[i - 127] : 0.0);
      if (m0 & CM_DOWN) {
        size_t dn = i - 129;
        if (l == 0) { int band, tt, ll; skew_decode(g, i, band, tt, ll); dn = skew_index(g, tt, 64 * band - 1); }
        v = v - s[dn];
      } else {
        v = v - 0.0;
      }
      o.x = v;
      t += v * c.x;
    }
    if (m1 & CM_FLUID) {
      double v = (double)(int)(m1 >> CM_DIAG_SHIFT) * c.y;
      v = v - ((m1 & CM_RIGHT) ? s[i + 128] : 0.0);
      if (m1 & CM_UP) {
        size_t up = i + 130;
        if (l == 63) { int band, tt, ll; skew_decode(g, i + 1, band, tt, ll); up = skew_index(g, tt - 63, 64 * (band + 1)); }
        v = v - s[up];
      } else {
        v = v - 0.0;
      }
      v = v - ((m1 & CM_LEFT) ? c.x : 0.0);
      if (m1 & CM_DOWN) {
        size_t dn = i - 2;
        if (l == 0) { int band, tt, ll; skew_decode(g, i + 1, band, tt, ll); dn = skew_index(g, tt, 64 * band - 1); }
        v = v - s[dn];
      } else {
        v = v - 0.0;
      }
      o.y = v;
      t += v * c.y;
    }
    if ((m0 & m1) & CM_FLUID) *reinterpret_cast<sw_d2*>(z + i) = o;
    else if (m0 & CM_FLUID) z[i] = o.x;
    else z[i + 1] = o.y;
  }
  t = block_sum(t);
  if (fin_op >= 0) block_finish<false>(t, partial, counter, sc, fin_op);
}

__global__ __launch_bounds__(RED_THREADS) void k_update_pr(double* __restrict__ p, double* __restrict__ r,
                                                           const double* __restrict__ s, const double* __restrict__ z,
                                                           const uint8_t* __restrict__ mask, size_t S,
                                                           double* __restrict__ partial, PcgScalars* sc, int force,
                                                           double alpha_arg, unsigned int* counter, int fin_op) {
  if (!force && pcg_idle(sc)) return;
  const double alpha = force ? alpha_arg : sc->alpha;
  const double nalpha = -alpha;
  const size_t chunk = (((S + gridDim.x - 1) / gridDim.x) + 1) & ~(size_t)1;
  const size_t lo = (size_t)blockIdx.x * chunk, hi = lo + chunk < S ? lo + chunk : S;
  double mx = 0.0;
  for (size_t i = lo + 2 * (size_t)threadIdx.x; i < hi; i += 2 * RED_THREADS) {
    const unsigned int mm = *reinterpret_cast<const unsigned short*>(mask + i);
    const bool f0 = (mm & CM_FLUID) != 0, f1 = ((mm >> 8) & CM_FLUID) != 0;
    if (!(f0 | f1)) continue;
    const sw_d2 sv = *reinterpret_cast<const sw_d2*>(s + i), zv = *reinterpret_cast<const sw_d2*>(z + i);
    sw_d2 pv = *reinterpret_cast<const sw_d2*>(p + i), rv = *reinterpret_cast<const sw_d2*>(r + i);
    if (f0) { pv.x = pv.x + sv.x * alpha; rv.x = rv.x + zv.x * nalpha; const double a = fabs(rv.x); if (a > mx) mx = a; }
    if (f1) { pv.y = pv.y + sv.y * alpha; rv.y = rv.y + zv.y * nalpha; const double a = fabs(rv.y); if (a > mx) mx = a; }
    *reinterpret_cast<sw_d2*>(p + i) = pv;
    *reinterpret_cast<sw_d2*>(r + i) = rv;
  }
  mx = block_max(mx);
  if (fin_op >= 0) block_finish<true>(mx, partial, counter, sc, fin_op);
}

__global__ __launch_bounds__(RED_THREADS) void k_inf_norm(const double* __restrict__ r, const uint8_t* __restrict__ mask,
                                                          size_t S, double* __restrict__ partial) {
  const size_t chunk = (S + gridDim.x - 1) / gridDim.x;
  const size_t lo = (size_t)blockIdx.x * chunk, hi = lo + chunk < S ? lo + chunk : S;
  double mx = 0.0;
  for (size_t i = lo + threadIdx.x; i < hi; i += RED_THREADS)
    if (mask[i] & CM_FLUID) { const double a = fabs(r[i]); if (a > mx) mx = a; }
  mx = block_max(mx);
  if (threadIdx.x == 0) partial[blockIdx.x] = mx;
}

template <bool COPY>
__global__ __launch_bounds__(256) void k_update_search(double* __restrict__ s, const double* __restrict__ z,
                                                       const uint8_t* __restrict__ mask, size_t S, const PcgScalars* sc,
                                                       int force, double beta_arg) {
  if (!force && pcg_idle(sc)) return;
  const double beta = force ? beta_arg : sc->beta;
  for (size_t i = 2 * ((size_t)blockIdx.x * blockDim.x + threadIdx.x); i < S; i += 2 * (size_t)gridDim.x * blockDim.x) {
    const sw_d2 zv = *reinterpret_cast<const sw_d2*>(z + i);
    if (COPY) { *reinterpret_cast<sw_d2*>(s + i) = zv; continue; }
    const unsigned int mm = *reinterpret_cast<const unsigned short*>(mask + i);
    const bool f0 = (mm & CM_FLUID) != 0, f1 = ((mm >> 8) & CM_FLUID) != 0;
    if (!(f0 | f1)) continue;
    sw_d2 sv = *reinterpret_cast<const sw_d2*>(s + i);
    if (f0) sv.x = zv.x + beta * sv.x;
    if (f1) sv.y = zv.y + beta * sv.y;
    *reinterpret_cast<sw_d2*>(s + i) = sv;
  }
}

__global__ __launch_bounds__(256) void k_publish_edge_rows(double* arr, SkewGeom g, int y0, int y1, const PcgScalars* sc) {
  if (pcg_idle(sc)) return;
  const int x = blockIdx.x * 256 + threadIdx.x;
  if (x >= g.X) return;
  const int y = blockIdx.y == 0 ? y0 : y1;
  if (y < 0) return;
  double* p = arr + skew_index(g, x, y);
  st_system(p, *p);
}

__global__ __launch_bounds__(256) void k_jacobi(const double* __restrict__ r, double* __restrict__ z,
                                                const uint8_t* __restrict__ mask, size_t S, const PcgScalars* sc, int force) {
  if (!force && pcg_idle(sc)) return;
  for (size_t i = (size_t)blockIdx.x * blockDim.x + threadIdx.x; i < S; i += (size_t)gridDim.x * blockDim.x) {
    const uint8_t m = mask[i];
    const int d = m >> CM_DIAG_SHIFT;
// ... 207 lines not shown
  const int n = p_steps(S);
  if (!S->s_base[0]) { S->s_base[0] = S->s; S->s_base[1] = S->s2; }
  if (n > 2) { S->s = S->s_base[0]; S->s2 = S->s_base[1]; }
  else if (S->s != S->s_base[0] && S->s != S->s_base[1]) { S->s = S->s_base[0]; S->s2 = S->s_base[1]; }
  else if (S->s2 != S->s_base[0] && S->s2 != S->s_base[1]) S->s2 = S->s == S->s_base[0] ? S->s_base[1] : S->s_base[0];
  S->s_ring[0] = S->s; S->s_ring[1] = S->s2;
  for (int k = 2; k < n; ++k) {
    if (!S->s_ring_alloc[k]) {
      const size_t elems = S->Sw + EU_SKEW_SLACK;
      if (hipMalloc(&S->s_ring_alloc[k], elems * sizeof(double)) != hipSuccess) {
        (void)hipGetLastError();
        S->s_ring_alloc[k] = nullptr;
        for (int j = 2; j < k; ++j) if (S->s_ring_alloc[j]) { (void)hipFree(S->s_ring_alloc[j]); S->s_ring_alloc[j] = nullptr; S->hbm_bytes -= elems * sizeof(double); }
        S->opt[EULER_OPT_P_STEPS] = 2;
        return ring_begin(S);
      }
      S->hbm_bytes += elems * sizeof(double);
      HIPCHK(hipMemsetAsync(S->s_ring_alloc[k], 0, elems * sizeof(double), S->stream));
    }
    S->s_ring[k] = static_cast<double*>(S->s_ring_alloc[k]) + EU_SKEW_SLACK - S->skew_off;
  }
  S->s_ring_n = n;
  S->s_launched = 0;
  return EULER_OK;
}
double* eu_current_search_direction(euler_sim* S) {
  if (S->s_ring_n < 2 || S->s_launched <= 0) return S->s;
  (void)hipStreamSynchronize(S->stream);
  const int ran = S->sc_host->nonzero ? S->sc_host->iters : 0;
  if (ran <= 0 || ran > S->s_launched) return S->s;
  return S->s_ring[(ran - 1) % S->s_ring_n];
}

__global__ void k_pcg_reset(PcgScalars* sc, double tol, int max_iters) {
  sc->sigma = sc->zs = sc->sigma_new = sc->alpha = sc->alpha_prev = sc->beta = sc->rnorm = 0.0;
  sc->tol = tol; sc->nonzero = 0; sc->done = 0; sc->iters = 0; sc->max_iters = max_iters; sc->zfix = 0;
}

static inline bool first_direction_folded(const euler_sim* S) { return tile_fused(S) && eu_is_mg(S) && !S->has_comm && S->cfg.dot_mode != EULER_DOT_SEQUENTIAL && sa_run(S) == 8; }
struct Solve {
  PcgScalars prev;
  int pred_iters;
  bool drain_poll;
  bool zr, zr_ran;
  bool solved;
};

static int project_begin(euler_sim* S, float dt, Solve& v) {
  S->s_launched = 0;
  S->z_halo_last = 0;
  S->p_pending = 0;
  S->pcg_fields_resident = 0;
  v.prev = *S->sc_host;
  S->solve_iters[S->solve_seq & 255] = S->sc_host->nonzero ? S->sc_host->iters : -1;
  if (S->solve_seq > 0) { S->res_last_chunks = S->sc_host->n_chunks; S->res_have_last = 1; }
  S->solve_seq += 1;
  v.pred_iters = (S->sc_host->nonzero && S->sc_host->done && S->sc_host->iters < S->cfg.max_iterations) ? S->sc_host->iters : 0;
  v.drain_poll = S->p2p_on && !(S->sc_host->nonzero && !S->sc_host->done && S->sc_host->iters >= S->cfg.max_iterations);
  S->prof_iter = -1;
  LAUNCH(S, KC_MISC, k_pcg_reset, dim3(1), dim3(1), S->sc, S->cfg.tol, S->cfg.max_iterations);
  eu_launch_build_system(S, dt);
  if (S->has_comm) {
    hipLaunchKernelGGL(k_nonzero_to_comm, dim3(1), dim3(1), 0, S->stream, S->sc);
    COMM_CALL(S->comm.allreduce(S->comm.ctx, &S->sc->comm_val, 1, 1));
    hipLaunchKernelGGL(k_nonzero_from_comm, dim3(1), dim3(1), 0, S->stream, S->sc);
  }
  return EULER_OK;
}

static int project_resident(euler_sim* S, float dt, Solve& v) {
  const bool res_skip = S->res_skip_once != 0;
  S->res_skip_once = 0;
  if (!res_skip && eu_resident_eligible(S)) {
    const unsigned int cap_chunks = 4u * (unsigned int)eu_resident_capacity(S, S->cfg.pcg_precision == EULER_PCG_F32);
    unsigned int guess = S->res_last_chunks;
    if (!S->res_have_last) {
      HIPCHK(hipMemcpyAsync(S->sc_host, S->sc, sizeof(PcgScalars), hipMemcpyDeviceToHost, S->stream));
      HIPCHK(hipStreamSynchronize(S->stream));
      guess = S->sc_host->n_chunks;
    }
    if (guess + guess / 16 + 8 <= cap_chunks || S->cfg.pcg_precision == EULER_PCG_F32) {
      v.solved = true;
      S->prof_iter = -2;
      if (int rc = eu_launch_resident(S, cap_chunks)) return rc;
      HIPCHK(hipMemcpyAsync(S->sc_host, S->sc, sizeof(PcgScalars), hipMemcpyDeviceToHost, S->stream));
      HIPCHK(hipStreamSynchronize(S->stream));
      S->res_last_chunks = S->sc_host->n_chunks; S->res_have_last = 1;
      const int err = *S->res_err;
      if (err == 0) {
        if (S->sc_host->nonzero) { S->res_solves += 1; S->pcg_fields_resident = 1; }
        return eu_launch_velocity_update(S, dt, 0);
      }
      *S->res_err = 0;
      if (S->cfg.pcg_precision == EULER_PCG_F32 && err == 2) { eu_set_error("EULER_PCG_F32: the solve's active chunks do not fit the resident solver"); return EULER_EHIP; }
      if (err != 2) { S->res_fallbacks += 1; S->res_disabled = 1; }
      S->solve_seq -= 1;
      S->lean_ok = 0;
      S->res_skip_once = 1;
      *S->sc_host = v.prev;
      return eu_launch_project(S, dt);
    }
  }
  return EULER_OK;
}

static int project_first_direction(euler_sim* S, Solve& v) {
  int rc;
  const bool tile = tile_fused(S), two_level = tile && eu_is_two_level(S);
  if (two_level && S->has_comm && !(eu_is_mg(S) && ghost_mode(S) && S->slab_on)) {
    eu_set_error("coarse-correction preconditioners with several ranks: EULER_PRECOND_IC0_TILE_MG on row slabs without mailboxes only");
    return EULER_EINVAL;
  }
  if (two_level && (rc = eu_launch_coarse_setup(S))) return rc;
  if (two_level && (rc = eu_launch_coarse_consistent(S))) return rc;
  v.zr = tile && tile_z_begin(S);
  if (tile) {
    if ((rc = eu_launch_factor_tile(S, 0))) return rc;
    if ((rc = eu_launch_precond_tile(S, 0, 1, FIN_SIGMA_INIT, 0, 0.0))) return rc;
  } else {
  if (S->cfg.precond != EULER_PRECOND_JACOBI && (rc = eu_launch_sweep(S, SW_FACTOR, KC_PRECON_FACTOR, 0))) return rc;
  if ((rc = launch_precondition(S, 0, FIN_SIGMA_INIT))) return rc;
  }
  if ((rc = ring_begin(S))) return rc;
  if (first_direction_folded(S)) {
    const PcgScalars& ps = v.prev;
    if (ps.nonzero && !(std::isfinite(ps.alpha) && std::isfinite(ps.beta) && std::isfinite(ps.rnorm) && std::isfinite(ps.sigma) && std::isfinite(ps.zs)))
      for (int k = 0; k < S->s_ring_n; ++k) HIPCHK(hipMemsetAsync(S->s_ring[k] + S->skew_off, 0, S->Sw * sizeof(double), S->stream));
  }
  else if (two_level) { if ((rc = eu_launch_coarse_search_init(S))) return rc; }
  else
  LAUNCH(S, KC_UPDATE_SEARCH, k_update_search<true>, dim3(eu_blocks(S->e_cnt, 256 * 4, 4096)), dim3(256), LOC(S->s), LOC(S->z),
         LOC(S->cellmask), S->e_cnt, S->sc, 0, 0.0);
  if (S->has_comm && eu_p2p_has_neighbour_arrays(S)) {
    const int y0 = S->band_lo > 0 ? 64 * S->band_lo : -1, y1 = S->band_hi < S->geom.nbands ? 64 * S->band_hi - 1 : -1;
    LAUNCH(S, KC_UPDATE_SEARCH, k_publish_edge_rows, dim3((S->X + 255) / 256, 2), dim3(256), S->s, S->geom, y0, y1, S->sc);
  }
  if (S->s_ring_n == 2) HIPCHK(hipMemsetAsync(LOC(S->s2), 0, S->e_cnt * sizeof(double), S->stream));
  S->s_stale = 1;
  return EULER_OK;
}

static int project_iterate(euler_sim* S, Solve& v) {
  int rc;
  HIPCHK(hipMemcpyAsync(S->sc_host, S->sc, sizeof(PcgScalars), hipMemcpyDeviceToHost, S->stream));
  HIPCHK(hipStreamSynchronize(S->stream));
  const int poll = S->cfg.pcg_poll_interval > 0 ? S->cfg.pcg_poll_interval : 8;
  const int max_it = S->cfg.max_iterations;
  const bool tile = tile_fused(S), fold0 = first_direction_folded(S);
  int it = 0, chunk = 0;
  bool stop = !S->sc_host->nonzero;
  S->s_none = stop ? 1 : 0;
  while (it < max_it && !stop) {
    int chunk_end = it + poll;
    if (!v.drain_poll && v.pred_iters > 0 && it < v.pred_iters + poll && chunk_end > v.pred_iters - 2) {
      const int lo = v.pred_iters - 2 < chunk_end ? v.pred_iters - 2 : chunk_end;
      chunk_end = lo > it + 2 ? lo : it + 2;
    }
    if (chunk_end > max_it) chunk_end = max_it;
    for (; it < chunk_end; ++it) {
      S->prof_iter = it;
      const bool fused = it > 0 || fold0;
      if (it == 0 && fold0) { S->s = S->s_ring[S->s_ring_n - 1]; S->s2 = S->s_ring[0]; }
      if ((rc = fused ? eu_launch_search_apply(S, it) : launch_apply_a_and_alpha(S, 0))) return rc;
      if (tile) {
        S->prof_iter = it;
        const int nx = it + 1, steps = S->s_ring_n;
        const bool next_odd = !(nx >= steps && nx % steps == 0);
        const int zform = v.zr && it + 1 < max_it ? (it + 2 < max_it && next_odd ? 1 : 0) : -1;
        if ((rc = eu_launch_precond_tile(S, 1, it + 1 < max_it, FIN_BETA, 0, 0.0, false, zform))) return rc;
        S->z_halo_last = zform == 1;
        v.zr_ran = v.zr_ran || zform == 1;
        continue;
      }
      S->tile_as_override = fused ? S->q : S->z;
      rc = eu_launch_precond_tile(S, 1, 0, -1, 0, 0.0, true);
      S->tile_as_override = nullptr;
      if (rc) return rc;
      if (it + 1 < max_it) {
        S->prof_iter = it + 1;
        if ((rc = launch_precondition(S, 0, FIN_BETA))) return rc;
      }
    }
    if (it < max_it && v.drain_poll) {
      HIPCHK(hipMemcpyAsync(S->sc_host, S->sc, sizeof(PcgScalars), hipMemcpyDeviceToHost, S->stream));
      HIPCHK(hipStreamSynchronize(S->stream));
      stop = S->sc_host->done != 0;
    } else
    if (it < max_it) {
      const int slot = chunk & 1;
      if (chunk > 0) {
        HIPCHK(hipEventSynchronize(S->poll_event[slot ^ 1]));
        stop = S->poll_host[slot ^ 1].done != 0;
      }
      HIPCHK(hipMemcpyAsync(&S->poll_host[slot], S->sc, sizeof(PcgScalars), hipMemcpyDeviceToHost, S->stream));
      HIPCHK(hipEventRecord(S->poll_event[slot], S->stream));
      ++chunk;
    }
  }
  return EULER_OK;
}

static int project_finish(euler_sim* S, float dt, const Solve& v) {
  int rc;
  S->prof_iter = -2;
  S->z_halo_last = 0;
  if (v.zr_ran && (rc = eu_launch_precond_tile(S, 0, 1, -1, 0, 0.0, false, 2))) return rc;
  const bool finish_in_update = !S->has_comm && !S->slab_on && S->opt[EULER_OPT_VELOCITY_TWO_PASS] == 0;
  if (!finish_in_update) { if ((rc = eu_launch_finish_p(S))) return rc; }
  if (S->s_ring_n > 2) { S->s = S->s_base[0]; S->s2 = S->s_base[1]; }
  if (S->has_comm && S->slab_on) {
    const int X = S->X, nbk = (X + 255) / 256;
    double *send_lo = S->halo_buf, *send_hi = S->halo_buf + X, *recv_lo = S->halo_buf + 2 * X, *recv_hi = S->halo_buf + 3 * X;
    if (S->band_lo > 0) hipLaunchKernelGGL(k_pack_row, dim3(nbk), dim3(256), 0, S->stream, S->p, send_lo, S->geom, S->band_lo, 0);
    COMM_CALL(S->bulk.halo(S->bulk.ctx, send_lo, send_hi, recv_lo, recv_hi, X));
    if (S->band_hi < S->geom.nbands) hipLaunchKernelGGL(k_unpack_row, dim3(nbk), dim3(256), 0, S->stream, S->p, recv_hi, S->geom, S->band_hi, 0);
  } else if (S->has_comm) {
    const int n = S->comm.nranks, nb = S->geom.nbands;
    std::vector<int64_t> off(n), cnt(n);
    for (int k = 0; k < n; ++k) {
      const int64_t lo = (int64_t)nb * k / n, hi = (int64_t)nb * (k + 1) / n;
      off[k] = lo * S->geom.TS * 64 * 8;
      cnt[k] = (hi - lo) * S->geom.TS * 64 * 8;
    }
    COMM_CALL(S->comm.allgather(S->comm.ctx, S->p, off.data(), cnt.data()));
  }
  if ((rc = eu_launch_velocity_update(S, dt, finish_in_update ? 1 : 0))) return rc;
  HIPCHK(hipMemcpyAsync(S->sc_host, S->sc, sizeof(PcgScalars), hipMemcpyDeviceToHost, S->stream));
  return EULER_OK;
}

int eu_launch_project(euler_sim* S, float dt) {
  Solve v = {};
  int rc;
  if ((rc = project_begin(S, dt, v))) return rc;
  if ((rc = project_resident(S, dt, v)) || v.solved) return rc;
  if ((rc = project_first_direction(S, v))) return rc;
  if ((rc = project_iterate(S, v))) return rc;
  return project_finish(S, dt, v);
}

int eu_launch_pcg_op(euler_sim* S, int op, float dt, double a, double* out) {
  S->s_none = 0;
  S->s_launched = 0;
  const bool want_scalar = op == EULER_OP_DOT_ZR || op == EULER_OP_DOT_ZS || op == EULER_OP_INF_NORM_R;
  const size_t SS = S->geom.S;
  if (eu_is_two_level(S) && (op == EULER_OP_PRECON_FACTOR || op == EULER_OP_FORWARD_SOLVE || op == EULER_OP_BACKWARD_SOLVE)) {
    eu_set_error("euler_pcg_op: the preconditioner of EULER_PRECOND_IC0_TILE2 / _MG is not available as a single operation (select EULER_PRECOND_IC0_TILE for its tile level)");
    return EULER_EINVAL;
  }
  switch (op) {
    case EULER_OP_BUILD_SYSTEM:
      LAUNCH(S, KC_MISC, k_pcg_reset, dim3(1), dim3(1), S->sc, S->cfg.tol, S->cfg.max_iterations);
      eu_launch_build_system(S, dt);
      break;
    case EULER_OP_PRECON_FACTOR: if (tile_fused(S)) eu_launch_factor_tile(S, 1); else eu_launch_sweep(S, SW_FACTOR, KC_PRECON_FACTOR, 1); break;
    case EULER_OP_FORWARD_SOLVE: if (!tile_fused(S)) eu_launch_sweep(S, SW_FORWARD, KC_FORWARD_SOLVE, 1); break;
    case EULER_OP_BACKWARD_SOLVE:
      if (tile_fused(S)) eu_launch_precond_tile(S, 0, 1, FIN_STORE_ONLY, 1, 0.0); else eu_launch_sweep(S, SW_BACKWARD, KC_BACKWARD_SOLVE, 1);
      break;
    case EULER_OP_APPLY_A:
      LAUNCH(S, KC_APPLY_A, k_apply_a, dim3(S->red_blocks), dim3(RED_THREADS), S->s, S->z, S->cellmask, S->geom,
             S->partial, S->sc, 1, S->red_counter, -1);
      break;
    case EULER_OP_DOT_ZR: eu_launch_dot(S, S->z, S->r, FIN_STORE_ONLY, 1); break;
    case EULER_OP_DOT_ZS: eu_launch_dot(S, S->z, S->s, FIN_STORE_ONLY, 1); break;
    case EULER_OP_INF_NORM_R:
      LAUNCH(S, KC_UPDATE_PR, k_inf_norm, dim3(S->red_blocks), dim3(RED_THREADS), S->r, S->cellmask, SS, S->partial);
      LAUNCH(S, KC_REDUCE_FINAL, k_reduce_final<true>, dim3(1), dim3(RED_THREADS), S->partial, S->red_blocks, S->sc,
             (int)FIN_STORE_ONLY, 1);
      break;
    case EULER_OP_UPDATE_PR:
      LAUNCH(S, KC_UPDATE_PR, k_update_pr, dim3(S->red_blocks), dim3(RED_THREADS), S->p, S->r, S->s, S->z, S->cellmask,
             SS, S->partial, S->sc, 1, a, S->red_counter, -1);
      break;
    case EULER_OP_UPDATE_SEARCH:
      LAUNCH(S, KC_UPDATE_SEARCH, k_update_search<false>, dim3(eu_blocks(SS, 256 * 4, 4096)), dim3(256), S->s, S->z,
             S->cellmask, SS, S->sc, 1, a);
// ... 9 lines not shown
```

euler_amd/csrc/k_sweep.hip:

```cpp
#include "k_pcg.h"

#include <type_traits>


__device__ __forceinline__ void sweep_qq_arrive(const SweepArgs& a, int ord, double lane_sum) {
  const int lane = threadIdx.x & 63;
  const double v = eu_wave_sum(lane_sum);
  int last = 0;
  if (lane == 0) {
    __hip_atomic_store(reinterpret_cast<unsigned long long*>(&a.qq_partial[ord]), (unsigned long long)__double_as_longlong(v), __ATOMIC_RELAXED, __HIP_MEMORY_SCOPE_AGENT);
    asm volatile("s_waitcnt vmcnt(0)" ::: "memory");
    last = __hip_atomic_fetch_add(a.qq_counter, 1u, __ATOMIC_RELAXED, __HIP_MEMORY_SCOPE_AGENT) == (unsigned int)a.nb_local - 1;
  }
  last = __builtin_amdgcn_readfirstlane(last);
  if (!last) return;
  double t = 0.0;
  for (int k = lane; k < a.nb_local; k += 64)
    t += __longlong_as_double((long long)__hip_atomic_load(reinterpret_cast<unsigned long long*>(&a.qq_partial[k]), __ATOMIC_RELAXED, __HIP_MEMORY_SCOPE_AGENT));
  t = eu_wave_sum(t);
  if (lane == 0) {
    pcg_scalar_step(a.sc_w, a.fin_qq, t);
    __hip_atomic_store(a.qq_counter, 0u, __ATOMIC_RELAXED, __HIP_MEMORY_SCOPE_AGENT);
  }
}
// ... 387 lines not shown
  a.mask = S->cellmask; a.fbits_fwd = S->fbits_fwd; a.fbits_bwd = S->fbits_bwd; a.fb_stride = S->fb_stride; a.pre = S->precon;
  a.in = op == SW_FORWARD ? S->r : S->q;
  a.out = op == SW_FORWARD ? S->q : S->z;
  a.granules = S->granules; a.gran_stride = S->gran_stride; a.ticket = S->ticket;
  a.xg_in = nullptr; a.xg_out = nullptr;
  a.ranges = S->band_ranges;
  a.band_lo = S->band_lo; a.nb_local = S->band_hi - S->band_lo; a.couple = S->has_comm && S->couple;
  a.ticket_base = S->ticket_base; a.epoch = S->epoch;
  a.sc = S->sc; a.force = force; a.error = &S->ms->error;
  a.timeline = S->sweep_timeline;
  a.tile_w = eu_is_tile(S) ? S->tile_w : 0;
  a.fin_qq = -1; a.qq_partial = S->partial; a.qq_counter = S->red_counter; a.sc_w = S->sc;
  return a;
}

__global__ __launch_bounds__(1024) void k_band_ranges(const uint8_t* __restrict__ count, int X, int Y, int T, int4* __restrict__ ranges, int band0) {
  __shared__ int s_lo, s_hi;
  const int band = band0 + blockIdx.x;
  if (threadIdx.x == 0) { s_lo = 0x7fffffff; s_hi = -1; }
  __syncthreads();
  int lo = 0x7fffffff, hi = -1;
  const int rows = Y - band * 64 < 64 ? Y - band * 64 : 64;
  for (int x = threadIdx.x; x < X; x += 1024) {
    for (int l0 = 0; l0 < rows; l0 += 8) {
      uint8_t c[8];
#pragma unroll
      for (int k = 0; k < 8; ++k) c[k] = l0 + k < rows ? count[(size_t)(band * 64 + l0 + k) * X + x] : (uint8_t)0;
#pragma unroll
      for (int k = 0; k < 8; ++k)
        if (c[k]) { const int t = x + l0 + k; lo = t < lo ? t : lo; hi = t > hi ? t : hi; }
    }
  }
  if (hi >= 0) { atomicMin(&s_lo, lo); atomicMax(&s_hi, hi); }
  __syncthreads();
  if (threadIdx.x == 0) {
    int4 r = make_int4(0, 0, 0, 0);
    if (s_hi >= 0) {
      const int f0 = s_lo / 32 * 32, f1 = (s_hi + 2 + 31) / 32 * 32;
      const int b0 = (T - 1 - s_hi) / 32 * 32, b1 = (T - 1 - s_lo + 2 + 31) / 32 * 32;
      r = make_int4(f0 / 8, f1 / 8, b0 / 8, b1 / 8);
    }
    ranges[band] = r;
  }
}
__global__ __launch_bounds__(256) void k_pack_fbits(const uint8_t* __restrict__ cellmask, SkewGeom g, unsigned int* __restrict__ fwd,
                                                    unsigned int* __restrict__ bwd, int fb_stride, int band_lo, int nb_local) {
  const size_t i = (size_t)blockIdx.x * 256 + threadIdx.x;
  if (i >= (size_t)nb_local * fb_stride * 64) return;
  const int lane = (int)(i & 63);
  const int gi = (int)((i >> 6) % fb_stride), band = band_lo + (int)((i >> 6) / fb_stride);
  const uint8_t* base = cellmask + (size_t)band * g.TS * 64 + 2 * lane;
  unsigned int wf = 0, wb = 0;
#pragma unroll
  for (int j = 0; j < 8; ++j) {
    const int tf = 8 * gi + j, tb = g.T - 1 - 8 * gi - j;
    if (tf < g.T && (base[(size_t)(tf & ~1) * 64 + (tf & 1)] & CM_FLUID)) wf |= 1u << j;
    if (tb >= 0) {
      const unsigned int m = base[(size_t)(tb & ~1) * 64 + (tb & 1)];
      if (m & CM_FLUID) wb |= 1u << j;
      if (m & CM_RIGHT) wb |= 1u << (8 + j);
      if (m & CM_UP) wb |= 1u << (16 + j);
    }
  }
  const size_t o = ((size_t)band * fb_stride + gi) * 64 + lane;
  fwd[o] = wf; bwd[o] = wb;
}
int eu_launch_band_ranges(euler_sim* S) {
  if (eu_is_tile(S)) return EULER_OK;
  const bool nbrs = S->has_comm && S->couple && !S->slab_on;
  const int b0 = nbrs && S->band_lo > 0 ? S->band_lo - 1 : S->band_lo, b1 = nbrs && S->band_hi < S->geom.nbands ? S->band_hi + 1 : S->band_hi;
  LAUNCH(S, KC_BUILD_SYSTEM, k_band_ranges, dim3(b1 - b0), dim3(1024), S->count, S->X, S->Y, S->geom.T, S->band_ranges, b0);
  const int nbl = S->band_hi - S->band_lo;
  const size_t n = (size_t)nbl * S->fb_stride * 64;
  LAUNCH(S, KC_BUILD_SYSTEM, k_pack_fbits, dim3((unsigned)((n + 255) / 256)), dim3(256), S->cellmask, S->geom, S->fbits_fwd, S->fbits_bwd,
         S->fb_stride, S->band_lo, nbl);
  return EULER_OK;
}

int eu_launch_sweep(euler_sim* S, int op, int cls, int force, int fin_qq) {
  typedef void (*Kernel)(SweepArgs);
  static const Kernel simple[3] = {k_sweep_simple<SW_FACTOR>, k_sweep_simple<SW_FORWARD>, k_sweep_simple<SW_BACKWARD>};
  static const Kernel skew[3] = {k_sweep_skew<SW_FACTOR>, k_sweep_skew<SW_FORWARD>, k_sweep_skew<SW_BACKWARD>};
  static const Kernel skew_xg[3] = {k_sweep_skew<SW_FACTOR, true>, k_sweep_skew<SW_FORWARD, true>, k_sweep_skew<SW_BACKWARD, true>};
  if (S->cfg.sweep_mode == EULER_SWEEP_SIMPLE) {
    LAUNCH(S, cls, simple[op], dim3(1), dim3(1024), make_sweep_args(S, op, force));
    return EULER_OK;
  }
  const bool BWD = op == SW_BACKWARD;
  const int nb = S->geom.nbands, nbl = S->band_hi - S->band_lo;
  const bool chain = S->has_comm && S->couple;
  const int64_t row_bytes = (int64_t)S->gran_stride * 2 * 8;
  const int g_first = BWD ? nb - S->band_hi : S->band_lo, g_last = g_first + nbl - 1;
  const int r = S->comm.rank, prev_rank = BWD ? r + 1 : r - 1, next_rank = BWD ? r - 1 : r + 1;
  S->epoch += 1;
  if (chain && S->p2p_on) {
    SweepArgs a = make_sweep_args(S, op, force);
    eu_p2p_xgran(S, BWD ? 1 : 0, &a.xg_in, &a.xg_out);
    LAUNCH(S, cls, skew_xg[op], dim3(nbl), dim3(192), a);
    S->ticket_base += (unsigned)nbl;
    return EULER_OK;
  }
  if (chain && g_first > 0)
    COMM_CALL(S->comm.chain(S->comm.ctx, S->granules + (size_t)(g_first - 1) * S->gran_stride * 2, row_bytes, prev_rank, r));
  SweepArgs a = make_sweep_args(S, op, force);
  a.fin_qq = fin_qq;
  LAUNCH(S, cls, skew[op], dim3(nbl), dim3(192), a);
  S->ticket_base += (unsigned)nbl;
  if (chain && g_last + 1 < nb)
    COMM_CALL(S->comm.chain(S->comm.ctx, S->granules + (size_t)g_last * S->gran_stride * 2, row_bytes, r, next_rank));
  return EULER_OK;
}
```

euler_amd/csrc/k_tile.hip:

```cpp
#include "k_pcg.h"

#include <type_traits>

#define PT_THREADS 256
__device__ __forceinline__ void tile_block_reduce(double& mx, double& sm) {
  __shared__ double s_mx[PT_THREADS / 64], s_sm[PT_THREADS / 64];
  mx = eu_wave_max(mx);
  sm = eu_wave_sum(sm);
  __syncthreads();
  if ((threadIdx.x & 63) == 0) { s_mx[threadIdx.x >> 6] = mx; s_sm[threadIdx.x >> 6] = sm; }
  __syncthreads();
  if (threadIdx.x == 0) {
    mx = s_mx[0]; sm = s_sm[0];
    for (int k = 1; k < PT_THREADS / 64; ++k) { mx = s_mx[k] > mx ? s_mx[k] : mx; sm += s_sm[k]; }
  }
}

__global__ __launch_bounds__(64) void k_tile_table(double* __restrict__ tab) {
  const int lane = threadIdx.x & 63;
  double own = 0.0, out = 0.0;
  sw_d2 pp[8];
#pragma unroll
  for (int j = 0; j < 16; ++j) {
    const double nbv = wave_shift_inject<DPP_WAVE_SHR1>(out, 0.0);
    const double res = factor_step(4.0, own, nbv);
    own = res; out = res;
    if (j & 1) pp[j >> 1].y = res; else pp[j >> 1].x = res;
  }
#pragma unroll
  for (int P = 0; P < 8; ++P) reinterpret_cast<sw_d2*>(tab)[P * 64 + lane] = pp[P];
}
int eu_launch_tile_table(euler_sim* S) {
  hipLaunchKernelGGL(k_tile_table, dim3(1), dim3(64), 0, S->stream, S->tile_table);
  return EULER_OK;
}

template <int W>
__global__ __launch_bounds__(PT_THREADS) void k_factor_tile(TileArgs a) {
  if (!a.force && pcg_idle(a.sc)) return;
  const int lane = threadIdx.x & 63;
  const int ntb = a.g.T / W, total = a.nb_local * ntb;
  const int n_waves = gridDim.x * (PT_THREADS / 64);
  for (int tile = blockIdx.x * (PT_THREADS / 64) + (threadIdx.x >> 6); tile < total; tile += n_waves) {
    const int band = a.band_lo + tile / ntb, k = tile % ntb;
    const size_t base = ((size_t)band * a.g.TS + (size_t)k * W) * 64 + 2 * lane;
    unsigned int mm[W / 2];
    unsigned int any = 0;
#pragma unroll
    for (int P = 0; P < W / 2; ++P) { mm[P] = *reinterpret_cast<const unsigned short*>(a.mask + base + P * 128); any |= mm[P]; }
    if (!__ballot(((any | (any >> 8)) & CM_FLUID) != 0)) continue;
    sw_d2 pp[W / 2];
#pragma unroll
    for (int P = 0; P < W / 2; ++P) pp[P] = *reinterpret_cast<const sw_d2*>(a.pre + base + P * 128);
    double own = 0.0, out = 0.0;
#pragma unroll
    for (int j = 0; j < W; ++j) {
      const int cm = (int)((mm[j >> 1] >> ((j & 1) * 8)) & 0xff);
      const double cpre = (j & 1) ? pp[j >> 1].y : pp[j >> 1].x;
      const double nbv = wave_shift_inject<DPP_WAVE_SHR1>(out, 0.0);
      const double aa = (double)(cm >> CM_DIAG_SHIFT);
      const double res = (cm & CM_FLUID) ? factor_step(aa, own, nbv) : cpre;
      own = res; out = res;
      if (j & 1) pp[j >> 1].y = res; else pp[j >> 1].x = res;
    }
#pragma unroll
    for (int P = 0; P < W / 2; ++P) *reinterpret_cast<sw_d2*>(a.pre + base + P * 128) = pp[P];
  }
}

#ifndef PT_RECOMP_BLOCKS
#define PT_RECOMP_BLOCKS 1
#endif
template <int W, bool RECOMP = false, int CMODE = 0>
__global__ __launch_bounds__(PT_THREADS, RECOMP ? PT_RECOMP_BLOCKS : 1) void k_precond_tile(TileArgs a) {
  if (!a.force && (a.zform == 2 ? a.sc->zfix == 0 : pcg_idle(a.sc))) return;
  const int lane = threadIdx.x & 63;
  const int ntb = a.g.T / W, total = a.nb_local * ntb;
  const int n_waves = gridDim.x * (PT_THREADS / 64);
  const double nalpha = -(a.force ? a.alpha_arg : a.sc->alpha);
  double mx = 0.0, dsum = 0.0;
  const bool listed = W == 16 && a.list != nullptr;
  const int todo = listed ? (int)a.sc->n_chunks : total;
  constexpr int TABP = W == 16 ? 8 : 1;
  __shared__ sw_d2 s_tab[TABP][64];
  __shared__ double s_cpart[CMODE == 2 ? PT_THREADS / 64 : 1][CMODE == 2 ? 16 * 2 * MG_NSLOT : 1];
  (void)s_cpart;
  const bool have_tab = W == 16 && listed && a.table != nullptr;
  if (have_tab) {
    for (int k = threadIdx.x; k < TABP * 64; k += PT_THREADS) (&s_tab[0][0])[k] = reinterpret_cast<const sw_d2*>(a.table)[k];
    __syncthreads();
  }
  typedef std::integral_constant<bool, true> yes_t;
  typedef std::integral_constant<bool, false> no_t;
  for (int i = blockIdx.x * (PT_THREADS / 64) + (threadIdx.x >> 6); i < todo; i += n_waves) {
    const int ii = a.reverse ? todo - 1 - i : i;
    const unsigned int ent = listed ? a.list[ii] : (unsigned int)ii;
    const bool interior = have_tab && (ent & EU_CHUNK_INTERIOR) != 0;
    const int tile = (int)(listed ? ent & ~EU_CHUNK_INTERIOR : ent);
    const int band = a.band_lo + tile / ntb, k = tile % ntb;
    const size_t base = ((size_t)band * a.g.TS + (size_t)k * W) * 64 + 2 * lane;
    auto run = [&](auto full_tag) {
      constexpr bool FULL = decltype(full_tag)::value;
      unsigned int mm[W / 2];
      unsigned int any = 0;
#pragma unroll
      for (int P = 0; P < W / 2; ++P) {
        mm[P] = FULL ? (unsigned int)(CM_INTERIOR | (CM_INTERIOR << 8)) : (unsigned int)*reinterpret_cast<const unsigned short*>(a.mask + base + P * 128);
        any |= mm[P];
      }
      if (!FULL && !listed && !__ballot(((any | (any >> 8)) & CM_FLUID) != 0)) return;
      sw_d2 rr[W / 2], qq[W / 2], pp[W / 2];
#pragma unroll
      for (int P = 0; P < W / 2; ++P) {
        rr[P] = *reinterpret_cast<const sw_d2*>(a.r + base + P * 128);
        if (RECOMP && a.rupd) continue;
        if (!a.sweeps) pp[P] = sw_d2{0.0, 0.0};
        else if (FULL) pp[P] = s_tab[P < TABP ? P : 0][lane];
        else pp[P] = *reinterpret_cast<const sw_d2*>(a.pre + base + P * 128);
        if (!RECOMP && a.rupd) qq[P] = *reinterpret_cast<const sw_d2*>(a.as + base + P * 128);
      }
      if (RECOMP && a.rupd) {
        const int npairs = a.g.TS / 2, P0 = k * (W / 2);
        sw_d2 ss[W / 2 + 2];
#pragma unroll
        for (int P = -1; P <= W / 2; ++P)
          ss[P + 1] = (P0 + P >= 0 && P0 + P < npairs) ? *reinterpret_cast<const sw_d2*>(a.as + base + (long long)P * 128) : sw_d2{0.0, 0.0};
        double ev = 0.0;
        if (lane < 16) {
          const int x = k * W + lane;
          if (x < a.g.X) {
            if (a.gs_lo && band == a.band_lo) ev = a.gs_lo[x];
            else if (band > 0) ev = a.as[skew_index(a.g, x, 64 * band - 1)];
          }
        } else if (lane >= 48) {
          const int x = k * W + lane - 48 - 63;
          if (x >= 0 && x < a.g.X) {
            if (a.gs_hi && band == a.band_lo + a.nb_local - 1) ev = a.gs_hi[x];
            else if (band + 1 < a.g.nbands) ev = a.as[skew_index(a.g, x, 64 * (band + 1))];
          }
        }
        const int ev_lo = __double2loint(ev), ev_hi = __double2hiint(ev);
#pragma unroll
        for (int P = 0; P < W / 2; ++P) {
          const unsigned int m0 = mm[P] & 0xff, m1 = mm[P] >> 8;
          const sw_d2 cc = ss[P + 1];
          const double prev_y = ss[P].y, nxt_x = ss[P + 2].x;
          const double d0 = __hiloint2double(__builtin_amdgcn_readlane(ev_hi, 2 * P), __builtin_amdgcn_readlane(ev_lo, 2 * P));
          const double d1 = __hiloint2double(__builtin_amdgcn_readlane(ev_hi, 2 * P + 1), __builtin_amdgcn_readlane(ev_lo, 2 * P + 1));
          const double u0 = __hiloint2double(__builtin_amdgcn_readlane(ev_hi, 48 + 2 * P), __builtin_amdgcn_readlane(ev_lo, 48 + 2 * P));
// ... 37 lines not shown
        for (int m = 0; m < MG_NSEG; ++m) { sg_s[m] = 0.0; sg_t[m] = 0.0; }
#pragma unroll
        for (int j = 0; j < W; ++j) {
          const int cm = (int)((mm[j >> 1] >> ((j & 1) * 8)) & 0xff);
          const double rv = (cm & CM_FLUID) ? ((j & 1) ? rr[j >> 1].y : rr[j >> 1].x) : 0.0;
          const double jv = rv * (double)j;
#pragma unroll
          for (int m = 0; m < MG_NSEG; ++m) {
            const bool in = (m == 0 || j >= tbase + MG_G0 * m) && (m == MG_NSEG - 1 || j < tbase + MG_G0 * (m + 1));
            sg_s[m] += in ? rv : 0.0; sg_t[m] += in ? jv : 0.0;
          }
        }
        double cn[MG_NSEG + 1];
#pragma unroll
        for (int m = 0; m <= MG_NSEG; ++m) cn[m] = 0.0;
#pragma unroll
        for (int m = 0; m < MG_NSEG; ++m) {
          double u1 = sg_t[m] + (double)(-tbase - MG_G0 * m) * sg_s[m], u0 = (double)MG_G0 * sg_s[m] - u1;
          if (Jb + m < 0) { u0 = 0.0; u1 = (double)MG_G0 * sg_s[m]; }
          if (Jb + m >= a.cnx - 1) { u0 = (double)MG_G0 * sg_s[m]; u1 = 0.0; }
          cn[m] += u0; cn[m + 1] += u1;
        }
        const bool shifted = Jb != Jq;
        wy0 *= 1.0 / (MG_G0 * MG_G0); wy1 *= 1.0 / (MG_G0 * MG_G0);
        double* sp = s_cpart[threadIdx.x >> 6];
#pragma unroll
        for (int q = 0; q < MG_NSLOT; ++q) {
          const double lo = cn[q], hi = q >= 1 ? cn[q - 1] : 0.0;
          const double cs = shifted ? hi : lo;
          const double p0 = group_sum(wy0 * cs), p1 = group_sum(wy1 * cs);
          if ((lane & 3) == 0) { sp[quad * 2 * MG_NSLOT + q] = p0; sp[quad * 2 * MG_NSLOT + MG_NSLOT + q] = p1; }
        }
        __builtin_amdgcn_fence(__ATOMIC_RELEASE, "wavefront");
        __builtin_amdgcn_wave_barrier();
        {
          double* cp = a.cpart + ((size_t)(tile / ntb) * MG_NGRP * ntb + (size_t)k) * (2 * MG_NSLOT);
#pragma unroll
          for (int u = 0; u < (MG_PART + 63) / 64; ++u) {
            const int e = lane + 64 * u;
            if (e < MG_PART) {
              const int g = e / (2 * MG_NSLOT), w = e % (2 * MG_NSLOT);
              const double va = g > 0 ? sp[(2 * g - 1) * 2 * MG_NSLOT + w] : 0.0, vb = g < 8 ? sp[(2 * g) * 2 * MG_NSLOT + w] : 0.0;
              cp[((size_t)g * ntb) * (2 * MG_NSLOT) + w] = va + vb;
            }
          }
        }
        __builtin_amdgcn_fence(__ATOMIC_ACQUIRE, "wavefront");
        __builtin_amdgcn_wave_barrier();
      } else if (W == 16 && CMODE == 1) {
        const int xl = k * W - 63, J0 = (xl > 0 ? xl : 0) >> a.cshift;
        double c0 = 0.0, c1 = 0.0, c2 = 0.0;
#pragma unroll
        for (int j = 0; j < W; ++j) {
          const int cm = (int)((mm[j >> 1] >> ((j & 1) * 8)) & 0xff);
          const double rv = (cm & CM_FLUID) ? ((j & 1) ? rr[j >> 1].y : rr[j >> 1].x) : 0.0;
          const int x = k * W + j - lane;
          const int b = ((x > 0 ? x : 0) >> a.cshift) - J0;
          c0 += b == 0 ? rv : 0.0; c1 += b == 1 ? rv : 0.0; c2 += b == 2 ? rv : 0.0;
        }
        c0 = eu_wave_sum(c0); c1 = eu_wave_sum(c1); c2 = eu_wave_sum(c2);
        if (lane == 0) { double* cp = a.cpart + (size_t)tile * 3; cp[0] = c0; cp[1] = c1; cp[2] = c2; }
      }
      if (RECOMP && a.rupd) {
        asm volatile("" ::: "memory");
#pragma unroll
        for (int P = 0; P < W / 2; ++P) pp[P] = FULL ? s_tab[P < TABP ? P : 0][lane] : *reinterpret_cast<const sw_d2*>(a.pre + base + P * 128);
      }
      tile_solve<W, true>(mm, rr, pp, qq, dsum);
      if (W == 16 && a.zform == 1) {
        double* h = a.zhalo + ((size_t)band * ntb + k) * 128;
        h[lane] = qq[0].x;
        h[64 + lane] = qq[W / 2 - 1].y;
        if (lane == 0 || lane == 63) {
          double* row = a.zrows + ((size_t)band * 2 + (lane == 63 ? 1 : 0)) * a.g.X;
#pragma unroll
          for (int j = 0; j < W; ++j) {
            const int x = k * W + j - lane;
            if (x >= 0 && x < a.g.X) row[x] = (j & 1) ? qq[j >> 1].y : qq[j >> 1].x;
          }
        }
      } else {
#pragma unroll
        for (int P = 0; P < W / 2; ++P) *reinterpret_cast<sw_d2*>(a.z + base + P * 128) = qq[P];
      }
      if (band == a.edge_lo || band == a.edge_hi) {
        const bool lo = band == a.edge_lo && lane == 0, hi = band == a.edge_hi && lane == 63;
#pragma unroll
        for (int j = 0; j < W; ++j) {
          const double zv = (j & 1) ? qq[j >> 1].y : qq[j >> 1].x;
          const int x_lo = k * W + j, x_hi = k * W + j - 63;
          if (lo && x_lo < a.g.X) a.zsend_lo[x_lo] = zv;
          if (hi && x_hi >= 0 && x_hi < a.g.X) a.zsend_hi[x_hi] = zv;
        }
      }
    };
    if (W == 16 && interior) run(yes_t()); else run(no_t());
  }
  tile_block_reduce(mx, dsum);
  __shared__ int am_last;
  if (threadIdx.x == 0) {
    __hip_atomic_store(reinterpret_cast<unsigned long long*>(&a.part_max[blockIdx.x]), (unsigned long long)__double_as_longlong(mx), __ATOMIC_RELAXED, __HIP_MEMORY_SCOPE_AGENT);
    __hip_atomic_store(reinterpret_cast<unsigned long long*>(&a.part_dot[blockIdx.x]), (unsigned long long)__double_as_longlong(dsum), __ATOMIC_RELAXED, __HIP_MEMORY_SCOPE_AGENT);
    asm volatile("s_waitcnt vmcnt(0)" ::: "memory");
    const unsigned int t = __hip_atomic_fetch_add(a.counter, 1u, __ATOMIC_RELAXED, __HIP_MEMORY_SCOPE_AGENT);
    am_last = t == gridDim.x - 1;
  }
  __syncthreads();
  if (!am_last) return;
  double vmax = 0.0, vsum = 0.0;
  for (unsigned int i = threadIdx.x; i < gridDim.x; i += PT_THREADS) {
    const double m = __longlong_as_double((long long)__hip_atomic_load(reinterpret_cast<unsigned long long*>(&a.part_max[i]), __ATOMIC_RELAXED, __HIP_MEMORY_SCOPE_AGENT));
    const double d = __longlong_as_double((long long)__hip_atomic_load(reinterpret_cast<unsigned long long*>(&a.part_dot[i]), __ATOMIC_RELAXED, __HIP_MEMORY_SCOPE_AGENT));
    vmax = m > vmax ? m : vmax; vsum += d;
  }
  tile_block_reduce(vmax, vsum);
  if (a.via == FIN_VIA_P2P) {
    if (a.rupd) vmax = p2p_allreduce_block<true>(a.sc, vmax);
    if (a.fin_dot >= 0) vsum = p2p_allreduce_block<false>(a.sc, vsum);
  }
  if (threadIdx.x == 0) {
    if (a.via == FIN_TO_COMM) { a.pair_slot[0] = vmax; a.pair_slot[1] = vsum; }
    else {
      if (a.rupd) pcg_scalar_step(a.sc, FIN_RNORM, vmax);
      if (a.fin_dot >= 0 && !(a.rupd && a.sc->done)) pcg_scalar_step(a.sc, a.fin_dot, vsum);
    }
    if (a.zform >= 0) a.sc->zfix = a.zform == 1 ? 1u : 0u;
    __hip_atomic_store(a.counter, 0u, __ATOMIC_RELAXED, __HIP_MEMORY_SCOPE_AGENT);
  }
}

__global__ void k_pair_fold(PcgScalars* sc, const double* __restrict__ pairs, int stride, int R, int rupd, int fin_dot, int force) {
  if (!force && pcg_idle(sc)) return;
  double vmax = 0.0, vsum = 0.0;
  for (int r = 0; r < R; ++r) { vmax = pairs[(size_t)stride * r] > vmax ? pairs[(size_t)stride * r] : vmax; vsum += pairs[(size_t)stride * r + 1]; }
  if (rupd) pcg_scalar_step(sc, FIN_RNORM, vmax);
  if (fin_dot >= 0 && !(rupd && sc->done)) pcg_scalar_step(sc, fin_dot, vsum);
}
static TileArgs make_tile_args(euler_sim* S, int force) {
  TileArgs a;
  a.g = S->geom; a.mask = S->cellmask; a.pre = S->precon; a.r = S->r; a.as = S->tile_as_override ? S->tile_as_override : S->q; a.z = S->z;
  a.band_lo = S->band_lo; a.nb_local = S->band_hi - S->band_lo;
  a.rupd = 0; a.sweeps = 1; a.fin_dot = -1;
  a.via = S->has_comm ? (S->p2p_on ? (int)FIN_VIA_P2P : (int)FIN_TO_COMM) : 0;
  a.part_max = S->partial; a.part_dot = S->partial2; a.counter = S->red_counter; a.sc = S->sc; a.force = force; a.alpha_arg = 0.0;
  a.pair_slot = S->pair_buf + 2 * (S->has_comm ? S->comm.rank : 0);
  a.list = !force ? S->chunk_list : nullptr;
  a.table = S->tile_table;
  a.zsend_lo = a.zsend_hi = nullptr; a.edge_lo = a.edge_hi = -1;
  a.reverse = S->opt[EULER_OPT_TILE_REVERSE] != 0;
  a.cpart = nullptr; a.cshift = 0; a.cmode = 0; a.cnx = a.cny = 0;
  a.gs_lo = a.gs_hi = nullptr;
  a.zform = -1; a.zhalo = S->zhalo; a.zrows = S->zrows;
  if (ghost_mode(S)) {
    if (S->band_lo > 0) { a.zsend_lo = xrow(S, XR_ZSEND_LO); a.edge_lo = S->band_lo; }
    if (S->band_hi < S->geom.nbands) { a.zsend_hi = xrow(S, XR_ZSEND_HI); a.edge_hi = S->band_hi - 1; }
  }
  return a;
}
static inline unsigned tile_blocks(const euler_sim* S, int w) {
  return eu_blocks((size_t)(S->band_hi - S->band_lo) * (S->geom.T / w), PT_THREADS / 64, 2048);
}
typedef void (*TileKernel)(TileArgs);
int eu_launch_factor_tile(euler_sim* S, int force) {
  const TileKernel k = S->tile_w == 8 ? k_factor_tile<8> : S->tile_w == 32 ? k_factor_tile<32> : k_factor_tile<16>;
  LAUNCH(S, KC_PRECON_FACTOR, k, dim3(tile_blocks(S, S->tile_w)), dim3(PT_THREADS), make_tile_args(S, force));
  return EULER_OK;
}
int eu_launch_precond_tile(euler_sim* S, int rupd, int sweeps, int fin_dot, int force, double alpha, bool r_only, int zform) {
  const bool seq = S->cfg.dot_mode == EULER_DOT_SEQUENTIAL && !S->has_comm;
  TileArgs a = make_tile_args(S, force);
  a.rupd = rupd; a.sweeps = sweeps; a.fin_dot = (seq || !sweeps) ? -1 : fin_dot; a.alpha_arg = alpha;
  a.zform = zform;
  const bool two_level = eu_is_two_level(S) && sweeps && !r_only && !force && a.list != nullptr;
  const int fin_real = a.fin_dot;
  if (two_level) {
    const bool mg = eu_is_mg(S);
    a.cpart = mg ? S->mg_part : S->cc_part; a.cshift = mg ? 0 : S->coarse_shift;
    a.cmode = mg ? 2 : 1; a.cnx = mg ? S->mg_nx[0] : 0; a.cny = mg ? S->mg_ny[0] : 0;
    if (a.fin_dot >= 0) a.fin_dot = FIN_STORE_ONLY;
  }
  double* xsmall = S->pair_buf;
  int nsmall = 2;
  bool split = false;
  if (two_level && a.via == FIN_TO_COMM) {
    split = eu_is_mg(S) && ghost_mode(S) && eu_mg_split(S);
    nsmall = eu_coarse_comm_slots(S);
    if (nsmall < 0) return EULER_ENOMEM;
    xsmall = S->mg_xbuf;
    a.pair_slot = xsmall + (size_t)S->comm.rank * nsmall;
    if (split) {
      if (a.zsend_lo) a.zsend_lo = eu_mg_split_msg(S, 0);
      if (a.zsend_hi) a.zsend_hi = eu_mg_split_msg(S, 1);
    }
  }
  const int w = r_only ? 16 : S->tile_w, cls = r_only ? KC_UPDATE_PR : zform == 2 ? KC_MISC : KC_PRECOND_TILE;
  const bool recomp = rupd && !force && tile_recompute(S) && (r_only ? S->tile_as_override == S->q : !S->tile_as_override);
  if (recomp) {
    a.as = S->s;
    if (ghost_mode(S)) {
      if (S->band_lo > 0) a.gs_lo = xrow(S, XR_GS_LO0 + S->gs_cur);
      if (S->band_hi < S->geom.nbands) a.gs_hi = xrow(S, XR_GS_HI0 + S->gs_cur);
    }
  }
  const TileKernel k = w == 8 ? k_precond_tile<8> : w == 32 ? k_precond_tile<32>
                     : a.cmode == 2 ? (recomp ? k_precond_tile<16, true, 2> : k_precond_tile<16, false, 2>)
                     : a.cmode == 1 ? (recomp ? k_precond_tile<16, true, 1> : k_precond_tile<16, false, 1>)
                     : (recomp ? k_precond_tile<16, true> : k_precond_tile<16>);
  LAUNCH(S, cls, k, dim3(tile_blocks(S, w)), dim3(PT_THREADS), a);
  if (two_level && a.via != FIN_TO_COMM) { int rc = eu_launch_coarse_solve(S, fin_real, force); if (rc) return rc; }
  if (seq && sweeps && fin_dot >= 0) eu_launch_dot(S, S->z, S->r, fin_dot, force);
  if (a.via == FIN_TO_COMM) {
    const int R = S->comm.nranks;
    const bool rows = ghost_mode(S) && !force;
    int rc = !two_level ? EULER_OK : split ? eu_mg_split_pre(S) : eu_launch_coarse_pre(S, force);
    if (rc) return rc;
    if (split) rc = eu_comm_exchange(S, eu_mg_split_msg(S, 0), eu_mg_split_msg(S, 1), eu_mg_split_msg(S, 2), eu_mg_split_msg(S, 3), eu_mg_split_count(S), xsmall, nsmall);
    else rc = eu_comm_exchange(S, xrow(S, XR_ZSEND_LO), xrow(S, XR_ZSEND_HI), xrow(S, XR_ZRECV_LO), xrow(S, XR_ZRECV_HI), rows ? S->X : 0, xsmall, nsmall);
    if (rc) return rc;
    hipLaunchKernelGGL(k_pair_fold, dim3(1), dim3(1), 0, S->stream, S->sc, xsmall, nsmall, R, rupd, a.fin_dot, force);
    if (split) {
      if ((rc = eu_mg_split_mid(S, fin_real, force, xrow(S, XR_ZRECV_LO), xrow(S, XR_ZRECV_HI)))) return rc;
      if ((rc = eu_comm_exchange(S, nullptr, nullptr, nullptr, nullptr, 0, eu_mg_split_gc(S), 1 + MG_NULL_MAX))) return rc;
      return eu_mg_split_fold(S, fin_real, force);
    }
    if (two_level) { rc = eu_launch_coarse_scatter(S); if (rc) return rc; rc = eu_launch_coarse_solve(S, fin_real, force); if (rc) return rc; }
  }
  return EULER_OK;
}
```

euler_amd/csrc/snapshot.hip:

```cpp
#include "euler_dev.h"

#include <math.h>
#include <stdlib.h>
#include <string.h>

#include <string>
#include <vector>

int eu_set_source_count(euler_sim* S, size_t nsrc);

static uint64_t snap_fnv(uint64_t h, const void* p, size_t n) {
  const unsigned char* b = (const unsigned char*)p;
  for (size_t i = 0; i < n; ++i) { h ^= b[i]; h *= 1099511628211ull; }
  return h;
}
struct SnapHeader {
  char magic[8]; uint32_t version; int32_t X, Y; uint32_t reserved;
  uint64_t n_markers, rng_state; int32_t source_exhausted; int32_t reserved2;
  uint64_t frames, total_substeps, total_pcg_iterations;
};
struct SlabHeader {
  int32_t nranks, rank, band_lo, band_hi, row_lo, row_hi;
  uint64_t n_loc;
};
struct ManifestHeader { char magic[8]; uint32_t version; int32_t X, Y, nranks; };
static const int SNAP_F32[] = {EULER_F_U, EULER_F_V, EULER_F_UTMP, EULER_F_VTMP};
static const int SNAP_U8[] = {EULER_F_SOLID, EULER_F_SOURCE, EULER_F_SINK, EULER_F_COUNT, EULER_F_PREV_COUNT};
static const int SNAP_DYE[] = {EULER_F_DYE_R, EULER_F_DYE_G, EULER_F_DYE_B, EULER_F_DYE_RTMP, EULER_F_DYE_GTMP, EULER_F_DYE_BTMP};

static std::string part_name(const char* path, int rank, int nranks) {
  char suffix[64];
  snprintf(suffix, sizeof suffix, ".%dof%d", rank, nranks);
  return std::string(path) + suffix;
}

static int write_part_file(euler_sim* S, const euler_stats& st, const std::string& tmp, bool slab, int nranks, int rank) {
  FILE* f = fopen(tmp.c_str(), "wb");
  if (!f) { eu_set_error("cannot open %s for writing", tmp.c_str()); return EULER_EIO; }
  int rc = EULER_OK;
  SnapHeader h;
  memset(&h, 0, sizeof h);
  memcpy(h.magic, "EULERSNP", 8);
  h.version = slab ? 3 : (S->dye[0] ? 2 : 1); h.reserved = (slab && S->dye[0]) ? 1 : 0;
  h.X = S->X; h.Y = S->Y; h.n_markers = st.n_markers; h.rng_state = st.rng_state;
  h.source_exhausted = st.source_exhausted; h.frames = st.frames; h.total_substeps = st.total_substeps;
  h.total_pcg_iterations = st.total_pcg_iterations;
  uint64_t sum = snap_fnv(14695981039346656037ull, &h, sizeof h);
  bool ok = fwrite(&h, sizeof h, 1, f) == 1;
  const uint64_t n_loc = S->n_markers_host;
  if (slab) {
    SlabHeader sh;
    memset(&sh, 0, sizeof sh);
    sh.nranks = nranks; sh.rank = rank; sh.band_lo = S->band_lo; sh.band_hi = S->band_hi; sh.row_lo = S->row_lo; sh.row_hi = S->row_hi; sh.n_loc = n_loc;
    sum = snap_fnv(sum, &sh, sizeof sh);
    ok = ok && fwrite(&sh, sizeof sh, 1, f) == 1;
  }
  const size_t Cr = (size_t)(S->row_hi - S->row_lo) * S->X;
  std::vector<unsigned char> buf;
  try { buf.resize(Cr * 8 > n_loc * 8 ? Cr * 8 : (size_t)n_loc * 8); } catch (...) { fclose(f); return EULER_ENOMEM; }
  auto put = [&](int field, size_t bytes) {
    if (!ok || !bytes) return;
    rc = euler_get_field(S, field, buf.data(), bytes);
    if (rc) { ok = false; return; }
    sum = snap_fnv(sum, buf.data(), bytes);
    ok = fwrite(buf.data(), 1, bytes, f) == bytes;
  };
  for (int fd : SNAP_F32) put(fd, Cr * 4);
  for (int fd : SNAP_U8) put(fd, Cr);
  put(EULER_F_PRECON, Cr * 8);
  if (S->dye[0]) for (int fd : SNAP_DYE) put(fd, Cr * 4);
  put(EULER_F_MARKERS, (size_t)n_loc * 8);
  if (slab) put(EULER_F_MARKER_KEYS, (size_t)n_loc * 4);
  ok = ok && fwrite(&sum, 8, 1, f) == 1;
  ok = (fclose(f) == 0) && ok;
  if (rc) return rc;
  if (!ok) { eu_set_error("short write to %s", tmp.c_str()); return EULER_EIO; }
  return EULER_OK;
}

extern "C" int euler_save_state(euler_sim* S, const char* path) {
  if (!S || !path) return EULER_EINVAL;
  euler_stats st;
  int rc = euler_get_stats(S, &st);
  const bool slab = S->slab_on != 0;
  if (rc && !slab) return rc;
  const int nranks = slab ? S->cfg.slab_nranks : 1, rank = slab ? S->cfg.slab_rank : 0;
  const std::string file = slab ? part_name(path, rank, nranks) : std::string(path);
  const std::string tmp = file + ".tmp";
  if (!rc) rc = write_part_file(S, st, tmp, slab, nranks, rank);
  auto agree = [&](int local, const char* what) -> int {
    if (!slab || !S->has_comm) return local;
    int worst = local;
    const int rc2 = eu_slab_status_sync(S, local, &worst);
    if (rc2) return rc2;
    if (worst && !local) eu_set_error("euler_save_state(%s): another rank failed to %s", path, what);
    return worst;
  };
  if ((rc = agree(rc, "write its part file"))) { remove(tmp.c_str()); return rc; }
  if (rename(tmp.c_str(), file.c_str()) != 0) { eu_set_error("cannot rename %s to %s", tmp.c_str(), file.c_str()); rc = EULER_EIO; }
  if ((rc = agree(rc, "put its part file in place"))) return rc;
  if (slab && rank == 0) {
    const std::string mtmp = std::string(path) + ".tmp";
    FILE* m = fopen(mtmp.c_str(), "wb");
    bool mok = m != nullptr;
    if (mok) {
      ManifestHeader mh;
      memset(&mh, 0, sizeof mh);
      memcpy(mh.magic, "EULERMAN", 8);
      mh.version = 3; mh.X = S->X; mh.Y = S->Y; mh.nranks = nranks;
      mok = fwrite(&mh, sizeof mh, 1, m) == 1;
      for (int r = 0; r < nranks && mok; ++r) { const int32_t b[2] = {S->part_lo[r], S->part_hi[r]}; mok = fwrite(b, sizeof b, 1, m) == 1; }
      mok = (fclose(m) == 0) && mok;
      mok = mok && rename(mtmp.c_str(), path) == 0;
    }
    if (!mok) { eu_set_error("cannot write the manifest %s", path); rc = EULER_EIO; }
  }
  return agree(rc, "write the manifest");
}

namespace {
struct Part {
  std::string file;
  SnapHeader h;
  int row_lo, row_hi;
  int keep_lo, keep_hi;
  uint64_t n_loc;
  bool keyed;
  std::vector<unsigned char> sec[16];
  std::vector<float> mk;
  std::vector<unsigned int> keys;
  bool has_dye() const { return h.version == 2 || (h.version == 3 && h.reserved == 1); }
  const unsigned char* rows(int k, int y) const { return sec[k].data() + (size_t)(y - keep_lo) * h.X * elem(k); }
  static size_t elem(int k) { return k <= 3 ? 4 : (k <= 8 ? 1 : (k == 9 ? 8 : 4)); }
};

int read_part(Part& p, int need_lo, int need_hi, int mark_lo, int mark_hi) {
  FILE* f = fopen(p.file.c_str(), "rb");
  if (!f) { eu_set_error("cannot open %s", p.file.c_str()); return EULER_EIO; }
  struct Closer { FILE* f; ~Closer() { fclose(f); } } closer{f};
  fseek(f, 0, SEEK_END);
  const long n = ftell(f);
  fseek(f, 0, SEEK_SET);
  if (n < (long)(sizeof(SnapHeader) + 8) || fread(&p.h, sizeof p.h, 1, f) != 1 || memcmp(p.h.magic, "EULERSNP", 8) != 0 || p.h.version < 1 || p.h.version > 3) {
    eu_set_error("%s is not an euler state snapshot (version 1, 2 or 3)", p.file.c_str()); return EULER_EINVAL;
  }
  uint64_t sum = snap_fnv(14695981039346656037ull, &p.h, sizeof p.h);
  size_t body = sizeof(SnapHeader);
  p.row_lo = 0; p.row_hi = p.h.Y; p.n_loc = p.h.n_markers; p.keyed = false;
  if (p.h.version == 3) {
    SlabHeader sh;
    if ((size_t)n < sizeof(SnapHeader) + sizeof sh + 8 || fread(&sh, sizeof sh, 1, f) != 1) { eu_set_error("%s is truncated (slab header)", p.file.c_str()); return EULER_EIO; }
    sum = snap_fnv(sum, &sh, sizeof sh);
    body += sizeof sh;
    p.row_lo = sh.row_lo; p.row_hi = sh.row_hi; p.n_loc = sh.n_loc; p.keyed = true;
  }
  if (p.h.X <= 0 || p.row_hi < p.row_lo) { eu_set_error("%s: bad header", p.file.c_str()); return EULER_EINVAL; }
  const size_t X = (size_t)p.h.X, C = (size_t)(p.row_hi - p.row_lo) * X;
  const size_t want = body + C * 29 + (p.has_dye() ? C * 24 : 0) + (size_t)p.n_loc * (p.keyed ? 12 : 8) + 8;
  if ((size_t)n != want) { eu_set_error("%s is truncated or corrupt (size)", p.file.c_str()); return EULER_EIO; }
  p.keep_lo = need_lo > p.row_lo ? need_lo : p.row_lo; p.keep_hi = need_hi < p.row_hi ? need_hi : p.row_hi;
  if (p.keep_hi < p.keep_lo) p.keep_hi = p.keep_lo;
  std::vector<unsigned char> chunk;
  try { chunk.resize((size_t)4 << 20); } catch (...) { return EULER_ENOMEM; }
  auto stream = [&](size_t bytes, auto&& sink) -> bool {
    for (size_t done = 0; done < bytes;) {
      const size_t len = bytes - done < chunk.size() ? bytes - done : chunk.size();
// ... 265 lines not shown
```

include/euler.h:

```cpp
#ifndef EULER_H
#define EULER_H

#include <stddef.h>
#include <stdint.h>

#ifdef __cplusplus
extern "C" {
#endif

#define EULER_ABI_VERSION 2

enum {
  EULER_OK = 0,
  EULER_EINVAL = -1,
  EULER_ENOMEM = -2,
  EULER_EIO = -3,
  EULER_EHIP = -4,
  EULER_ESTATE = -5,
  EULER_ETIMEOUT = -6,
  EULER_ECOMM = -7
};

enum {
  EULER_DOT_AUTO = 0,
// ... 188 lines not shown
  uint32_t count_max;
  uint32_t nonfinite;
  float    max_div;
  float    max_speed2;
} euler_diag;
typedef struct euler_diag_values {
  double mean_abs_div;
  double kinetic_energy;
  double com_x, com_y;
  double markers_per_cell;
  double crowded_fraction;
} euler_diag_values;
int euler_diagnostics(euler_sim* sim, int32_t x0, int32_t y0, int32_t x1, int32_t y1, euler_diag* out, size_t out_bytes);
int euler_diag_derive(const euler_diag* rec, euler_diag_values* out);

enum { EULER_FLOW_PRESSURE = 1 };
typedef struct euler_flow_px {
  uint32_t cells;
  uint32_t water;
  uint32_t nodes;
  uint32_t nonfinite;
  uint64_t u_pos, u_neg;
  uint64_t v_pos, v_neg;
  uint64_t w_pos, w_neg;
  uint64_t p_sum;
  float    max_speed2;
  float    max_abs_w;
  float    max_p;
  uint32_t reserved;
} euler_flow_px;
int euler_flow_raster(euler_sim* sim, int32_t x0, int32_t y0, int32_t x1, int32_t y1,
                      int32_t W, int32_t H, int32_t flags, euler_flow_px* out, size_t out_bytes);
enum { EULER_PAINT_VORTICITY = 0, EULER_PAINT_PRESSURE = 1, EULER_PAINT_SPEED = 2 };
int euler_flow_paint(const euler_flow_px* flow, euler_overview_px* px, int32_t W, int32_t H, int32_t field, double scale);

enum { EULER_EDIT_SOLID = 0, EULER_EDIT_CLEAR = 1, EULER_EDIT_SINK = 2, EULER_EDIT_SOURCE = 3, EULER_EDIT_FILL = 4, EULER_EDIT_DRAIN = 5 };
int euler_edit_box(euler_sim* sim, int32_t op, int32_t x0, int32_t y0, int32_t x1, int32_t y1);

typedef struct euler_comm_ops {
  void*   ctx;
  int32_t rank, nranks;
  int (*allreduce)(void* ctx, void* dev_f64, int32_t count, int32_t is_max);
  int (*halo)(void* ctx, void* send_lo, void* send_hi, void* recv_lo, void* recv_hi, int32_t count);
  int (*chain)(void* ctx, void* dev_ptr, int64_t nbytes, int32_t src, int32_t dst);
  int (*allgather)(void* ctx, void* dev_base, const int64_t* off, const int64_t* cnt);
  int (*exchange)(void* ctx, void* send_lo, void* send_hi, void* recv_lo, void* recv_hi, int32_t count, void* small, int32_t nsmall);
} euler_comm_ops;

enum {
  EULER_SLAB_EXACT = 1,
  EULER_SLAB_LOCAL = 0
};
int euler_set_comm(euler_sim* sim, const euler_comm_ops* ops, int32_t coupling);

#define EULER_RCCL_ID_BYTES 128
int euler_rccl_unique_id(void* id_out, int32_t cap);
int euler_rccl_version(void);
int euler_set_comm_rccl(euler_sim* sim, const void* unique_id, int32_t id_bytes, int32_t rank, int32_t nranks,
                        int32_t coupling);
enum {
  EULER_OPT_P_STEPS = 1,
  EULER_OPT_TILE_STORE_AS = 2,
  EULER_OPT_TILE_REVERSE = 3,
  EULER_OPT_RESIDENT_CAP = 4,
  EULER_OPT_GRID4_MIN_CELLS = 5,
  EULER_OPT_SLAB_FUSION = 6,
  EULER_OPT_RCCL_SMALL = 7,
  EULER_OPT_RCCL_NO_EXCHANGE = 8,
  EULER_OPT_MARKERS_ROWMAJOR = 9,
  EULER_OPT_SA_RUN = 10,
  EULER_OPT_NO_INTERIOR = 11,
  EULER_OPT_BUILD_GATHER = 12,
  EULER_OPT_RESIDENT_FORCE_TIMEOUT = 13,
  EULER_OPT_MG_SPLIT_LEVEL = 14,
  EULER_OPT_MG_SPLIT_ACTIVE = 15,
  EULER_OPT_MARKERS_TWO_PASS = 16,
  EULER_OPT_BUILD_TWO_PASS = 17,
  EULER_OPT_VELOCITY_TWO_PASS = 18,
  EULER_OPT_NO_TILE_MAP = 19,
  EULER_OPT_PROFILE_STRIDE = 20,
  EULER_OPT_TILE_STORE_Z = 21,
  EULER_OPT_ADVECT_RK2 = 22,
  EULER_OPT_ADVECT_MACCORMACK = 23,
  EULER_OPT__COUNT
};
int euler_set_option(euler_sim* sim, int32_t key, int64_t value);
int euler_get_option(euler_sim* sim, int32_t key, int64_t* value);

int euler_comm_calls(euler_sim* sim, uint64_t out[5]);

#define EULER_P2P_HANDLE_BYTES 256
int euler_p2p_export(euler_sim* sim, void* handle_out, int32_t cap);
int euler_p2p_connect(euler_sim* sim, const void* handles, int32_t nranks);
int euler_p2p_disconnect(euler_sim* sim);
int euler_p2p_calls(euler_sim* sim, uint64_t out[2]);
int euler_set_stream(euler_sim* sim, void* hip_stream);
int euler_slab_info(euler_sim* sim, int32_t* band_lo, int32_t* band_hi, int32_t* nbands);

int euler_profile_enable(euler_sim* sim, uint64_t class_mask);
int euler_profile_class_count(void);
const char* euler_profile_class_name(int32_t cls);
int euler_profile_get(euler_sim* sim, int32_t cls, double* total_ms, uint64_t* launches);
int euler_profile_reset(euler_sim* sim);
int euler_measure_copy_bandwidth(euler_sim* sim, size_t bytes, int32_t reps, double* gbps);
int euler_measure_exchange(euler_sim* sim, int32_t reps, int32_t row_doubles, int32_t nsmall, double* us_per_exchange);
int euler_device_name(euler_sim* sim, char* out, int32_t cap);
uint64_t euler_hbm_bytes(const euler_sim* sim);
int euler_sweep_timeline(euler_sim* sim, uint64_t* out, int32_t cap_bands);

#ifdef __cplusplus
}
#endif
#endif
```

Before: 184.6 million.

## Lean PCG solve prologue: lazy interior precon, fused first direction, mapped poll

Adds a lean solve prologue on the recompute-tile path. The IC0 factor skips interior tiles and marks them lazy so their preconditioner comes from a shared table, with a flush kernel run before anything reads precon. The first preconditioner pass writes z straight into the search direction, so the separate update_search launch goes away. Iteration polling reads a mapped host word written by the kernel instead of doing a per-chunk device-to-host memcpy. Separately, the stencil apply kernel takes its up/down neighbours via wave DPP shifts instead of scattered loads. Together these add state tracking (precon_pending) and flush hooks at every entry point that might read the preconditioner.

Result: no change. 185.6 million, median of 4 (+0.5%).

```diff
diff --git a/euler_amd/__init__.py b/euler_amd/__init__.py
--- a/euler_amd/__init__.py
+++ b/euler_amd/__init__.py
@@ -11,6 +11,7 @@
 (OPT_P_STEPS, OPT_TILE_STORE_AS, OPT_TILE_REVERSE, OPT_RESIDENT_CAP, OPT_GRID4_MIN_CELLS, OPT_SLAB_FUSION, OPT_RCCL_SMALL, OPT_RCCL_NO_EXCHANGE, OPT_MARKERS_ROWMAJOR,
  OPT_SA_RUN, OPT_NO_INTERIOR, OPT_BUILD_GATHER, OPT_RESIDENT_FORCE_TIMEOUT, OPT_MG_SPLIT_LEVEL, OPT_MG_SPLIT_ACTIVE, OPT_MARKERS_TWO_PASS, OPT_BUILD_TWO_PASS,
  OPT_VELOCITY_TWO_PASS, OPT_NO_TILE_MAP, OPT_PROFILE_STRIDE, OPT_TILE_STORE_Z, OPT_ADVECT_RK2, OPT_ADVECT_MACCORMACK) = range(1, 24)
+OPT_SOLVE_PROLOGUE_SPLIT = 25
 SWEEP_AUTO, SWEEP_BAND, SWEEP_SIMPLE = 0, 1, 2
 PCG_F64, PCG_F32 = 0, 1
 RESIDENT_AUTO, RESIDENT_OFF = 0, 1
diff --git a/euler_amd/csrc/driver.hip b/euler_amd/csrc/driver.hip
--- a/euler_amd/csrc/driver.hip
+++ b/euler_amd/csrc/driver.hip
@@ -146,7 +146,7 @@
 }
 
 extern "C" int euler_set_option(euler_sim* S, int32_t key, int64_t value) {
-  if (!S || key <= 0 || key >= EULER_OPT__COUNT) { eu_set_error("euler_set_option: unknown key %d", (int)key); return EULER_EINVAL; }
+  if (!S || key <= 0 || key >= EULER_OPT__COUNT || key == EULER_OPT_ADVECT_MACCORMACK + 1) { eu_set_error("euler_set_option: unknown key %d", (int)key); return EULER_EINVAL; }
   bool ok = true;
   const char* when = nullptr;
   switch (key) {
@@ -196,7 +196,7 @@
   return EULER_OK;
 }
 extern "C" int euler_get_option(euler_sim* S, int32_t key, int64_t* value) {
-  if (!S || !value || key <= 0 || key >= EULER_OPT__COUNT) { eu_set_error("euler_get_option: unknown key %d", (int)key); return EULER_EINVAL; }
+  if (!S || !value || key <= 0 || key >= EULER_OPT__COUNT || key == EULER_OPT_ADVECT_MACCORMACK + 1) { eu_set_error("euler_get_option: unknown key %d", (int)key); return EULER_EINVAL; }
   *value = S->opt[key];
   return EULER_OK;
 }
@@ -217,6 +217,7 @@
   if (const char* why = eu_precond_combination(S, precond, w, S->has_comm, S->slab_on, S->p2p_on)) { eu_set_error("euler_set_precond: %s", why); return EULER_EINVAL; }
   if (S->cfg.pcg_precision == EULER_PCG_F32 && (precond != EULER_PRECOND_IC0_TILE || w != 16)) { eu_set_error("euler_set_precond: an EULER_PCG_F32 handle runs EULER_PRECOND_IC0_TILE with tiles of 16 records only"); return EULER_EINVAL; }
   HIPCHK(hipStreamSynchronize(S->stream));
+  if (int rcp = eu_precon_current(S)) return rcp;
   const bool coarse = precond == EULER_PRECOND_IC0_TILE2 || precond == EULER_PRECOND_IC0_TILE_MG;
   if (coarse) { int rc = eu_coarse_alloc(S, precond == EULER_PRECOND_IC0_TILE_MG); if (rc) return rc; }
   (void)eu_set_tiles(S, w);
@@ -266,7 +267,7 @@
   if (S->sys_m) (void)hipFree(S->sys_m);
   if (S->sys_div) (void)hipFree(S->sys_div);
   void* dev[] = {S->markers[0], S->markers[1], S->keys[0], S->keys[1], S->ms, S->evmask, S->delmask, S->ev_theta, S->ev_delta, S->sel_idx, S->act_idx,
-                 S->act_dt, S->cellmask64, S->draws, S->sel.block_sums, S->sc, S->partial, S->red_counter, S->granules, S->ticket, S->sweep_timeline, S->halo_buf, S->band_ranges, S->partial2, S->pair_buf, S->xrows, S->alpha_buf, S->rng_jump, S->chunk_flag, S->chunk_prev, S->chunk_part, S->tile_table, S->chunk_bits, S->chunk_list, S->zhalo, S->zrows,
+                 S->act_dt, S->cellmask64, S->draws, S->sel.block_sums, S->sc, S->partial, S->red_counter, S->granules, S->ticket, S->sweep_timeline, S->halo_buf, S->band_ranges, S->partial2, S->pair_buf, S->xrows, S->alpha_buf, S->rng_jump, S->chunk_flag, S->chunk_prev, S->chunk_part, S->pre_lazy, S->tile_table, S->chunk_bits, S->chunk_list, S->zhalo, S->zrows,
                  S->rowmajor_tmp, S->mc_u, S->mc_v};
   for (void* p : dev) if (p) (void)hipFree(p);
   for (float* d : S->dye) if (d) (void)hipFree(d + wo);
@@ -280,6 +281,7 @@
   if (S->ms_host) (void)hipHostFree(S->ms_host);
   if (S->sc_host) (void)hipHostFree(S->sc_host);
   if (S->poll_host) (void)hipHostFree(S->poll_host);
+  if (S->poll_pair) (void)hipHostFree(S->poll_pair);
   if (S->res_err) (void)hipHostFree(S->res_err);
   if (S->res_gran) (void)hipFree(S->res_gran);
   for (hipEvent_t e : S->poll_event) if (e) (void)hipEventDestroy(e);
@@ -428,6 +430,7 @@
   DALLOC(S->chunk_flag, S->chunk_cap + 64);
   DALLOC(S->chunk_prev, S->chunk_cap + 64);
   DALLOC(S->chunk_part, S->chunk_cap + 64);
+  DALLOC(S->pre_lazy, S->chunk_cap + 64);
   DALLOC(S->tile_table, 8 * 64 * 2);
   DALLOC(S->chunk_bits, S->chunk_words + 1);
   DALLOC(S->chunk_list, S->chunk_cap + 64);
@@ -464,6 +467,9 @@
   CREATECHK(hipHostMalloc((void**)&S->ms_host, sizeof(MarkerState), hipHostMallocDefault));
   CREATECHK(hipHostMalloc((void**)&S->sc_host, sizeof(PcgScalars), hipHostMallocDefault));
   CREATECHK(hipHostMalloc((void**)&S->poll_host, 2 * sizeof(PcgScalars), hipHostMallocDefault));
+  CREATECHK(hipHostMalloc((void**)&S->poll_pair, sizeof(unsigned long long), hipHostMallocMapped));
+  *S->poll_pair = 0;
+  CREATECHK(hipHostGetDevicePointer((void**)&S->poll_pair_dev, S->poll_pair, 0));
   CREATECHK(hipHostMalloc((void**)&S->res_err, sizeof(int), hipHostMallocDefault));
   *S->res_err = 0;
   DALLOC(S->res_gran, 2 * 2 * (2 * 768) * 2);
@@ -744,7 +750,9 @@
 
 extern "C" int euler_stage(euler_sim* S, int32_t stage, float dt) {
   if (!S || !S->loaded) { eu_set_error("euler_stage: no scenario loaded"); return EULER_ESTATE; }
-  int rc = S->slab_on ? eu_slab_stage(S, stage, dt) : run_stage(S, stage, dt);
+  int rc = eu_precon_current(S);
+  if (rc) return rc;
+  rc = S->slab_on ? eu_slab_stage(S, stage, dt) : run_stage(S, stage, dt);
   if (rc) return rc;
   if (S->slab_on && (rc = eu_slab_error_sync(S))) return rc;
   rc = eu_sync_marker_state(S);
@@ -816,6 +824,7 @@
   S->pcg_fields_resident = 0;
   int rcp = eu_pressure_current(S);
   if (rcp) return rcp;
+  if ((rcp = eu_precon_current(S))) return rcp;
   return eu_launch_pcg_op(S, op, dt, a, out);
 }
 
@@ -876,6 +885,7 @@
     eu_set_error("euler_get_field(%d): the last solve ran in the resident kernel, which keeps z, s and A s in registers (euler_config.resident = EULER_RESIDENT_OFF shows them)", f);
     return EULER_ESTATE;
   }
+  if (f == EULER_F_PRECON && (rc = eu_precon_current(S))) return rc;
   if (f == EULER_F_PRESSURE && (rc = eu_pressure_current(S))) return rc;
   if (field_is_skewed(f)) {
     rc = ensure_rowmajor_tmp(S);
@@ -899,7 +909,7 @@
 
 extern "C" int euler_set_field(euler_sim* S, int32_t f, const void* src, size_t src_bytes) {
   if (!S || !src) return EULER_EINVAL;
-  if (field_is_skewed(f)) { int rcp = eu_pressure_current(S); if (rcp) return rcp; }
+  if (field_is_skewed(f)) { int rcp = eu_pressure_current(S); if (!rcp) rcp = eu_precon_current(S); if (rcp) return rcp; }
   eu_state_edited(S);
   if (S->slab_on && (f == EULER_F_MARKERS || f == EULER_F_MARKER_KEYS || f == EULER_F_COUNT || f == EULER_F_PREV_COUNT ||
                      f == EULER_F_SOLID || f == EULER_F_SOURCE)) {
diff --git a/euler_amd/csrc/euler_dev.h b/euler_amd/csrc/euler_dev.h
--- a/euler_amd/csrc/euler_dev.h
+++ b/euler_amd/csrc/euler_dev.h
@@ -203,6 +203,8 @@
   struct RngJump* rng_jump;
   uint8_t* chunk_flag;
   uint8_t* chunk_prev;
+  uint8_t* pre_lazy;
+  int precon_pending;
   uint8_t* chunk_part;
   size_t hbm_bytes;
   int lean_ok;
@@ -223,6 +225,8 @@
   PcgScalars* sc_host;
   PcgScalars* poll_host;
   hipEvent_t poll_event[2];
+  unsigned long long* poll_pair;
+  double* poll_pair_dev;
   double* partial;
   unsigned int* red_counter;
   int red_blocks;
@@ -316,6 +320,7 @@
   S->prebin_valid = 0;
   if (S->maxsq_state == 2) S->maxsq_state = 1;
   S->p_pending = 0;
+  S->precon_pending = 2;
   S->uv_clean = 0; S->uv_zb = 0;
   S->tmap_valid = 0; S->utmp_clean = 0; S->countT_clean = 0;
 }
@@ -335,6 +340,7 @@
 int eu_launch_project(euler_sim* S, float dt);
 int eu_resident_capacity(euler_sim* S, int f32);
 int eu_launch_resident(euler_sim* S, unsigned int n_chunks);
+int eu_precon_current(euler_sim* S);
 bool eu_resident_eligible(const euler_sim* S);
 int eu_launch_colorize(euler_sim* S);
 int eu_launch_dye_extrapolate(euler_sim* S);
diff --git a/euler_amd/csrc/k_pcg.h b/euler_amd/csrc/k_pcg.h
--- a/euler_amd/csrc/k_pcg.h
+++ b/euler_amd/csrc/k_pcg.h
@@ -12,7 +12,7 @@
 int eu_launch_band_ranges(euler_sim* S);
 int eu_launch_sweep(euler_sim* S, int op, int cls, int force, int fin_qq = -1);
 int eu_launch_factor_tile(euler_sim* S, int force);
-int eu_launch_precond_tile(euler_sim* S, int rupd, int sweeps, int fin_dot, int force, double alpha, bool r_only = false, int zform = -1);
+int eu_launch_precond_tile(euler_sim* S, int rupd, int sweeps, int fin_dot, int force, double alpha, bool r_only = false, int zform = -1, double* s0 = nullptr);
 int eu_launch_search_apply(euler_sim* S, int it);
 int eu_launch_finish_p(euler_sim* S);
 int eu_launch_dot(euler_sim* S, const double* a, const double* b, int fin_op, int force);
@@ -37,6 +37,7 @@
   return tile_recompute(S) && tile_fused(S) && !eu_is_two_level(S) && S->tile_w == 16 && !S->has_comm && !S->slab_on && S->band_lo == 0 &&
          S->opt[EULER_OPT_TILE_STORE_Z] == 0 && S->chunk_list && S->tile_table;
 }
+static inline bool solve_prologue_lean(const euler_sim* S) { return tile_z_recompute(S) && S->opt[EULER_OPT_SOLVE_PROLOGUE_SPLIT] == 0; }
 static inline int fin_or_comm(const euler_sim* S, int fin_op) {
   return S->has_comm ? (S->p2p_on ? (fin_op | FIN_VIA_P2P) : (int)FIN_TO_COMM) : fin_op;
 }
@@ -232,6 +233,10 @@
   const double *gs_lo, *gs_hi;
   int zform;
   double *zhalo, *zrows;
+  double* s0;
+  uint8_t* lazy;
+  const uint8_t* part;
+  double* poll;
 };
 
 __device__ __forceinline__ double factor_step(double aa, double own, double nbv) {
diff --git a/euler_amd/csrc/k_pcg.hip b/euler_amd/csrc/k_pcg.hip
--- a/euler_amd/csrc/k_pcg.hip
+++ b/euler_amd/csrc/k_pcg.hip
@@ -96,52 +96,45 @@
   const size_t chunk = (((S + gridDim.x - 1) / gridDim.x) + 127) & ~(size_t)127;
   const size_t lo = (size_t)blockIdx.x * chunk, hi = lo + chunk < S ? lo + chunk : S;
   double t = 0.0;
+  const int l = (int)(threadIdx.x & 63);
   for (size_t i = lo + 2 * (size_t)threadIdx.x; i < hi; i += 2 * RED_THREADS) {
     const unsigned int mm = *reinterpret_cast<const unsigned short*>(mask + i);
     const unsigned int m0 = mm & 0xff, m1 = mm >> 8;
-    if (!((m0 | m1) & CM_FLUID)) continue;
+    const bool fluid = ((m0 | m1) & CM_FLUID) != 0;
+    if (!__ballot(fluid)) continue;
     const sw_d2 c = *reinterpret_cast<const sw_d2*>(s + i);
-    const int l = (int)((i & 127) >> 1);
+    const sw_d2 nx = *reinterpret_cast<const sw_d2*>(s + i + 128);
+    const sw_d2 pv = i >= 128 ? *reinterpret_cast<const sw_d2*>(s + i - 128) : sw_d2{0.0, 0.0};
+    double up0e = 0.0, up1e = 0.0, dn0e = 0.0, dn1e = 0.0;
+    if (l == 63 && ((m0 | m1) & CM_UP)) {
+      int band, tt, ll;
+      if (m0 & CM_UP) { skew_decode(g, i, band, tt, ll); up0e = s[skew_index(g, tt - 63, 64 * (band + 1))]; }
+      if (m1 & CM_UP) { skew_decode(g, i + 1, band, tt, ll); up1e = s[skew_index(g, tt - 63, 64 * (band + 1))]; }
+    }
+    if (l == 0 && ((m0 | m1) & CM_DOWN)) {
+      int band, tt, ll;
+      if (m0 & CM_DOWN) { skew_decode(g, i, band, tt, ll); dn0e = s[skew_index(g, tt, 64 * band - 1)]; }
+      if (m1 & CM_DOWN) { skew_decode(g, i + 1, band, tt, ll); dn1e = s[skew_index(g, tt, 64 * band - 1)]; }
+    }
+    const double up0 = wave_shift_inject<DPP_WAVE_SHL1>(c.y, up0e), up1 = wave_shift_inject<DPP_WAVE_SHL1>(nx.x, up1e);
+    const double dn0 = wave_shift_inject<DPP_WAVE_SHR1>(pv.y, dn0e), dn1 = wave_shift_inject<DPP_WAVE_SHR1>(c.x, dn1e);
+    if (!fluid) continue;
     sw_d2 o = {0.0, 0.0};
     if (m0 & CM_FLUID) {
       double v = (double)(int)(m0 >> CM_DIAG_SHIFT) * c.x;
       v = v - ((m0 & CM_RIGHT) ? c.y : 0.0);
-      if (m0 & CM_UP) {
-        size_t up = i + 3;
-        if (l == 63) { int band, tt, ll; skew_decode(g, i, band, tt, ll); up = skew_index(g, tt - 63, 64 * (band + 1)); }
-        v = v - s[up];
-      } else {
-        v = v - 0.0;
-      }
-      v = v - ((m0 & CM_LEFT) ? s[i - 127] : 0.0);
-      if (m0 & CM_DOWN) {
-        size_t dn = i - 129;
-        if (l == 0) { int band, tt, ll; skew_decode(g, i, band, tt, ll); dn = skew_index(g, tt, 64 * band - 1); }
-        v = v - s[dn];
-      } else {
-        v = v - 0.0;
-      }
+      v = v - ((m0 & CM_UP) ? up0 : 0.0);
+      v = v - ((m0 & CM_LEFT) ? pv.y : 0.0);
+      v = v - ((m0 & CM_DOWN) ? dn0 : 0.0);
       o.x = v;
       t += v * c.x;
     }
     if (m1 & CM_FLUID) {
       double v = (double)(int)(m1 >> CM_DIAG_SHIFT) * c.y;
-      v = v - ((m1 & CM_RIGHT) ? s[i + 128] : 0.0);
-      if (m1 & CM_UP) {
-        size_t up = i + 130;
-        if (l == 63) { int band, tt, ll; skew_decode(g, i + 1, band, tt, ll); up = skew_index(g, tt - 63, 64 * (band + 1)); }
-        v = v - s[up];
-      } else {
-        v = v - 0.0;
-      }
+      v = v - ((m1 & CM_RIGHT) ? nx.x : 0.0);
+      v = v - ((m1 & CM_UP) ? up1 : 0.0);
       v = v - ((m1 & CM_LEFT) ? c.x : 0.0);
-      if (m1 & CM_DOWN) {
-        size_t dn = i - 2;
-        if (l == 0) { int band, tt, ll; skew_decode(g, i + 1, band, tt, ll); dn = skew_index(g, tt, 64 * band - 1); }
-        v = v - s[dn];
-      } else {
-        v = v - 0.0;
-      }
+      v = v - ((m1 & CM_DOWN) ? dn1 : 0.0);
       o.y = v;
       t += v * c.y;
     }
@@ -515,6 +508,7 @@
     if (guess + guess / 16 + 8 <= cap_chunks || S->cfg.pcg_precision == EULER_PCG_F32) {
       v.solved = true;
       S->prof_iter = -2;
+      if (int rc = eu_precon_current(S)) return rc;
       if (int rc = eu_launch_resident(S, cap_chunks)) return rc;
       HIPCHK(hipMemcpyAsync(S->sc_host, S->sc, sizeof(PcgScalars), hipMemcpyDeviceToHost, S->stream));
       HIPCHK(hipStreamSynchronize(S->stream));
@@ -547,21 +541,23 @@
   if (two_level && (rc = eu_launch_coarse_setup(S))) return rc;
   if (two_level && (rc = eu_launch_coarse_consistent(S))) return rc;
   v.zr = tile && tile_z_begin(S);
+  const bool lean = tile && solve_prologue_lean(S);
+  if (lean && (rc = ring_begin(S))) return rc;
   if (tile) {
     if ((rc = eu_launch_factor_tile(S, 0))) return rc;
-    if ((rc = eu_launch_precond_tile(S, 0, 1, FIN_SIGMA_INIT, 0, 0.0))) return rc;
+    if ((rc = eu_launch_precond_tile(S, 0, 1, FIN_SIGMA_INIT, 0, 0.0, false, -1, lean ? S->s : nullptr))) return rc;
   } else {
   if (S->cfg.precond != EULER_PRECOND_JACOBI && (rc = eu_launch_sweep(S, SW_FACTOR, KC_PRECON_FACTOR, 0))) return rc;
   if ((rc = launch_precondition(S, 0, FIN_SIGMA_INIT))) return rc;
   }
-  if ((rc = ring_begin(S))) return rc;
+  if (!lean && (rc = ring_begin(S))) return rc;
   if (first_direction_folded(S)) {
     const PcgScalars& ps = v.prev;
     if (ps.nonzero && !(std::isfinite(ps.alpha) && std::isfinite(ps.beta) && std::isfinite(ps.rnorm) && std::isfinite(ps.sigma) && std::isfinite(ps.zs)))
       for (int k = 0; k < S->s_ring_n; ++k) HIPCHK(hipMemsetAsync(S->s_ring[k] + S->skew_off, 0, S->Sw * sizeof(double), S->stream));
   }
   else if (two_level) { if ((rc = eu_launch_coarse_search_init(S))) return rc; }
-  else
+  else if (!lean)
   LAUNCH(S, KC_UPDATE_SEARCH, k_update_search<true>, dim3(eu_blocks(S->e_cnt, 256 * 4, 4096)), dim3(256), LOC(S->s), LOC(S->z),
          LOC(S->cellmask), S->e_cnt, S->sc, 0, 0.0);
   if (S->has_comm && eu_p2p_has_neighbour_arrays(S)) {
@@ -580,6 +576,8 @@
   const int poll = S->cfg.pcg_poll_interval > 0 ? S->cfg.pcg_poll_interval : 8;
   const int max_it = S->cfg.max_iterations;
   const bool tile = tile_fused(S), fold0 = first_direction_folded(S);
+  const bool pair_poll = tile && !v.drain_poll && S->poll_pair_dev && solve_prologue_lean(S);
+  if (pair_poll) *static_cast<volatile unsigned long long*>(S->poll_pair) = 0;
   int it = 0, chunk = 0;
   bool stop = !S->sc_host->nonzero;
   S->s_none = stop ? 1 : 0;
@@ -623,9 +621,9 @@
       const int slot = chunk & 1;
       if (chunk > 0) {
         HIPCHK(hipEventSynchronize(S->poll_event[slot ^ 1]));
-        stop = S->poll_host[slot ^ 1].done != 0;
+        stop = pair_poll ? (*static_cast<volatile unsigned long long*>(S->poll_pair) & 0xffffffffull) != 0 : S->poll_host[slot ^ 1].done != 0;
       }
-      HIPCHK(hipMemcpyAsync(&S->poll_host[slot], S->sc, sizeof(PcgScalars), hipMemcpyDeviceToHost, S->stream));
+      if (!pair_poll) HIPCHK(hipMemcpyAsync(&S->poll_host[slot], S->sc, sizeof(PcgScalars), hipMemcpyDeviceToHost, S->stream));
       HIPCHK(hipEventRecord(S->poll_event[slot], S->stream));
       ++chunk;
     }
diff --git a/euler_amd/csrc/k_sweep.hip b/euler_amd/csrc/k_sweep.hip
--- a/euler_amd/csrc/k_sweep.hip
+++ b/euler_amd/csrc/k_sweep.hip
@@ -493,6 +493,7 @@
   static const Kernel simple[3] = {k_sweep_simple<SW_FACTOR>, k_sweep_simple<SW_FORWARD>, k_sweep_simple<SW_BACKWARD>};
   static const Kernel skew[3] = {k_sweep_skew<SW_FACTOR>, k_sweep_skew<SW_FORWARD>, k_sweep_skew<SW_BACKWARD>};
   static const Kernel skew_xg[3] = {k_sweep_skew<SW_FACTOR, true>, k_sweep_skew<SW_FORWARD, true>, k_sweep_skew<SW_BACKWARD, true>};
+  if (int rc = eu_precon_current(S)) return rc;
   if (S->cfg.sweep_mode == EULER_SWEEP_SIMPLE) {
     LAUNCH(S, cls, simple[op], dim3(1), dim3(1024), make_sweep_args(S, op, force));
     return EULER_OK;
diff --git a/euler_amd/csrc/k_tile.hip b/euler_amd/csrc/k_tile.hip
--- a/euler_amd/csrc/k_tile.hip
+++ b/euler_amd/csrc/k_tile.hip
@@ -49,9 +49,15 @@
 #pragma unroll
     for (int P = 0; P < W / 2; ++P) { mm[P] = *reinterpret_cast<const unsigned short*>(a.mask + base + P * 128); any |= mm[P]; }
     if (!__ballot(((any | (any >> 8)) & CM_FLUID) != 0)) continue;
+    bool from_table = false;
+    if (W == 16 && a.lazy) {
+      const bool flagged = a.lazy[tile] != 0;
+      if (a.part && !a.part[tile]) { if (!flagged && lane == 0) a.lazy[tile] = 1; continue; }
+      from_table = flagged;
+    }
     sw_d2 pp[W / 2];
 #pragma unroll
-    for (int P = 0; P < W / 2; ++P) pp[P] = *reinterpret_cast<const sw_d2*>(a.pre + base + P * 128);
+    for (int P = 0; P < W / 2; ++P) pp[P] = from_table ? reinterpret_cast<const sw_d2*>(a.table)[(P < 8 ? P : 0) * 64 + lane] : *reinterpret_cast<const sw_d2*>(a.pre + base + P * 128);
     double own = 0.0, out = 0.0;
 #pragma unroll
     for (int j = 0; j < W; ++j) {
@@ -65,6 +71,19 @@
     }
 #pragma unroll
     for (int P = 0; P < W / 2; ++P) *reinterpret_cast<sw_d2*>(a.pre + base + P * 128) = pp[P];
+    if (from_table && lane == 0) a.lazy[tile] = 0;
+  }
+}
+__global__ __launch_bounds__(PT_THREADS) void k_precon_flush(double* __restrict__ pre, const double* __restrict__ tab, uint8_t* __restrict__ lazy, SkewGeom g, int nbands) {
+  const int lane = threadIdx.x & 63;
+  const int ntb = g.T / 16, total = nbands * ntb;
+  const int n_waves = gridDim.x * (PT_THREADS / 64);
+  for (int tile = blockIdx.x * (PT_THREADS / 64) + (threadIdx.x >> 6); tile < total; tile += n_waves) {
+    if (!lazy[tile]) continue;
+    const size_t base = ((size_t)(tile / ntb) * g.TS + (size_t)(tile % ntb) * 16) * 64 + 2 * lane;
+#pragma unroll
+    for (int P = 0; P < 8; ++P) *reinterpret_cast<sw_d2*>(pre + base + P * 128) = reinterpret_cast<const sw_d2*>(tab)[P * 64 + lane];
+    if (lane == 0) lazy[tile] = 0;
   }
 }
 
@@ -268,6 +287,10 @@
       } else {
 #pragma unroll
         for (int P = 0; P < W / 2; ++P) *reinterpret_cast<sw_d2*>(a.z + base + P * 128) = qq[P];
+        if (!RECOMP && a.s0) {
+#pragma unroll
+          for (int P = 0; P < W / 2; ++P) *reinterpret_cast<sw_d2*>(a.s0 + base + P * 128) = qq[P];
+        }
       }
       if (band == a.edge_lo || band == a.edge_hi) {
         const bool lo = band == a.edge_lo && lane == 0, hi = band == a.edge_hi && lane == 63;
@@ -309,6 +332,7 @@
     else {
       if (a.rupd) pcg_scalar_step(a.sc, FIN_RNORM, vmax);
       if (a.fin_dot >= 0 && !(a.rupd && a.sc->done)) pcg_scalar_step(a.sc, a.fin_dot, vsum);
+      if (a.rupd && a.poll) st_system(a.poll, __longlong_as_double((long long)(((unsigned long long)(unsigned int)a.sc->iters << 32) | (a.sc->done ? 1u : 0u))));
     }
     if (a.zform >= 0) a.sc->zfix = a.zform == 1 ? 1u : 0u;
     __hip_atomic_store(a.counter, 0u, __ATOMIC_RELAXED, __HIP_MEMORY_SCOPE_AGENT);
@@ -337,6 +361,7 @@
   a.cpart = nullptr; a.cshift = 0; a.cmode = 0; a.cnx = a.cny = 0;
   a.gs_lo = a.gs_hi = nullptr;
   a.zform = -1; a.zhalo = S->zhalo; a.zrows = S->zrows;
+  a.s0 = nullptr; a.lazy = nullptr; a.part = nullptr; a.poll = nullptr;
   if (ghost_mode(S)) {
     if (S->band_lo > 0) { a.zsend_lo = xrow(S, XR_ZSEND_LO); a.edge_lo = S->band_lo; }
     if (S->band_hi < S->geom.nbands) { a.zsend_hi = xrow(S, XR_ZSEND_HI); a.edge_hi = S->band_hi - 1; }
@@ -347,16 +372,35 @@
   return eu_blocks((size_t)(S->band_hi - S->band_lo) * (S->geom.T / w), PT_THREADS / 64, 2048);
 }
 typedef void (*TileKernel)(TileArgs);
+int eu_precon_current(euler_sim* S) {
+  if (!S->precon_pending) return EULER_OK;
+  const int mode = S->precon_pending;
+  S->precon_pending = 0;
+  if (!S->pre_lazy) return EULER_OK;
+  if (mode == 2) { HIPCHK(hipMemsetAsync(S->pre_lazy, 0, S->chunk_cap, S->stream)); return EULER_OK; }
+  LAUNCH(S, KC_PRECON_FACTOR, k_precon_flush, dim3(eu_blocks((size_t)S->geom.nbands * (S->geom.T / 16), PT_THREADS / 64, 2048)), dim3(PT_THREADS), S->precon, S->tile_table, S->pre_lazy,
+         S->geom, S->band_hi - S->band_lo);
+  return EULER_OK;
+}
 int eu_launch_factor_tile(euler_sim* S, int force) {
   const TileKernel k = S->tile_w == 8 ? k_factor_tile<8> : S->tile_w == 32 ? k_factor_tile<32> : k_factor_tile<16>;
-  LAUNCH(S, KC_PRECON_FACTOR, k, dim3(tile_blocks(S, S->tile_w)), dim3(PT_THREADS), make_tile_args(S, force));
+  TileArgs a = make_tile_args(S, force);
+  if (!force && solve_prologue_lean(S) && S->pre_lazy) {
+    if (S->precon_pending == 2) HIPCHK(hipMemsetAsync(S->pre_lazy, 0, S->chunk_cap, S->stream));
+    S->precon_pending = 1;
+    a.lazy = S->pre_lazy;
+    a.part = S->opt[EULER_OPT_NO_INTERIOR] ? nullptr : S->chunk_part;
+  } else if (int rc = eu_precon_current(S)) return rc;
+  LAUNCH(S, KC_PRECON_FACTOR, k, dim3(tile_blocks(S, S->tile_w)), dim3(PT_THREADS), a);
   return EULER_OK;
 }
-int eu_launch_precond_tile(euler_sim* S, int rupd, int sweeps, int fin_dot, int force, double alpha, bool r_only, int zform) {
+int eu_launch_precond_tile(euler_sim* S, int rupd, int sweeps, int fin_dot, int force, double alpha, bool r_only, int zform, double* s0) {
+  if (force) { int rc = eu_precon_current(S); if (rc) return rc; }
   const bool seq = S->cfg.dot_mode == EULER_DOT_SEQUENTIAL && !S->has_comm;
   TileArgs a = make_tile_args(S, force);
   a.rupd = rupd; a.sweeps = sweeps; a.fin_dot = (seq || !sweeps) ? -1 : fin_dot; a.alpha_arg = alpha;
-  a.zform = zform;
+  a.zform = zform; a.s0 = s0;
+  if (rupd && !force && !r_only && solve_prologue_lean(S)) a.poll = S->poll_pair_dev;
   const bool two_level = eu_is_two_level(S) && sweeps && !r_only && !force && a.list != nullptr;
   const int fin_real = a.fin_dot;
   if (two_level) {
diff --git a/euler_amd/csrc/snapshot.hip b/euler_amd/csrc/snapshot.hip
--- a/euler_amd/csrc/snapshot.hip
+++ b/euler_amd/csrc/snapshot.hip
@@ -82,6 +82,7 @@
   if (!S || !path) return EULER_EINVAL;
   euler_stats st;
   int rc = euler_get_stats(S, &st);
+  if (!rc) rc = eu_precon_current(S);
   const bool slab = S->slab_on != 0;
   if (rc && !slab) return rc;
   const int nranks = slab ? S->cfg.slab_nranks : 1, rank = slab ? S->cfg.slab_rank : 0;
diff --git a/include/euler.h b/include/euler.h
--- a/include/euler.h
+++ b/include/euler.h
@@ -294,6 +294,7 @@
   EULER_OPT_TILE_STORE_Z = 21,
   EULER_OPT_ADVECT_RK2 = 22,
   EULER_OPT_ADVECT_MACCORMACK = 23,
+  EULER_OPT_SOLVE_PROLOGUE_SPLIT = 25,
   EULER_OPT__COUNT
 };
 int euler_set_option(euler_sim* sim, int32_t key, int64_t value);
```
